# edervishaj/GANMF

Measured on AMD Instinct MI355X. Metric: GANMF training steps/sec, higher is better.
Workload: dtype f32

## Files before the change

ganmf_amd/csrc/gemm_bf16s.hpp:

```cpp
#pragma once
#include "gemm_f32.hpp"

namespace ganmf {

template <int R, int BK, bool KM>
struct SplitStage {
  static constexpr int NW = R * BK / 8;
  static constexpr int NI = NW / 256;
  static constexpr int PLANE = R * BK / 2;
  static constexpr int CH = BK / 8;
  static constexpr int RQ = R / 4;
  static constexpr int KROW = R / 2;
  static_assert(R == 64 || R == 128, "K-major chunk swizzle is laid out for 64- and 128-row operand tiles");
  __device__ static inline int swzk(int k) { return R == 64 ? ((k & 3) >> 1) << 2 : (k & 3) << 2; }
  static_assert(NW % 256 == 0 && NI >= 1, "tile too small for 256 threads");
  static_assert(BK == 32 || BK == 64, "BK must be 32 or 64");

  __device__ static inline int swz(int row) { return BK == 32 ? (row >> 2) & 3 : (row >> 1) & 7; }

  const float* zp;
  const float* ptr[NI];
  int aux[NI];
  int dst[NI];
  int dst1[NI];

  __device__ inline void init(const float* __restrict__ base, int ld, int r0, int rlimit, int kbeg,
                              const float* zero, int tid) {
    zp = zero + (tid & 255) * 8;
#pragma unroll
    for (int j = 0; j < NI; ++j) {
      const int w = j * 256 + tid;
      if constexpr (!KM) {
        const int row = w / CH, c8 = w % CH;
        const bool ok = (r0 + row) < rlimit;
        ptr[j] = ok ? base + (size_t)(r0 + row) * ld + kbeg + 8 * c8 : zp;
        aux[j] = ok ? BK : 0;
        dst[j] = row * (BK / 2) + 4 * (c8 ^ swz(row));
      } else {
        const int kp = w / RQ, rq = w % RQ;
        const bool ok = (r0 + 4 * rq) < ld;
        ptr[j] = base + (size_t)(kbeg + 2 * kp) * ld + r0 + 4 * rq;
        aux[j] = ok ? 2 * kp : -1;
        dst[j] = (2 * kp) * KROW + 4 * ((rq >> 1) ^ swzk(2 * kp)) + 2 * (rq & 1);
        dst1[j] = (2 * kp + 1) * KROW + 4 * ((rq >> 1) ^ swzk(2 * kp + 1)) + 2 * (rq & 1);
      }
    }
  }

  __device__ inline void load(float4 (&v)[NI][2], int ld, int kleft) {
#pragma unroll
    for (int j = 0; j < NI; ++j) {
      if constexpr (!KM) {
        const float* s = ptr[j];
        v[j][0] = *reinterpret_cast<const float4*>(s);
        v[j][1] = *reinterpret_cast<const float4*>(s + 4);
        ptr[j] += aux[j];
      } else {
        const float* s0 = (aux[j] >= 0 && aux[j] < kleft) ? ptr[j] : zp;
        const float* s1 = (aux[j] >= 0 && aux[j] + 1 < kleft) ? ptr[j] + ld : zp;
        v[j][0] = *reinterpret_cast<const float4*>(s0);
        v[j][1] = *reinterpret_cast<const float4*>(s1);
        ptr[j] += (size_t)BK * ld;
      }
    }
  }

  bool diag_nosplit = false;
  template <int NPIECE, bool F16 = false>
  __device__ inline void store(unsigned* __restrict__ planes, const float4 (&v)[NI][2], float scale = 1.f) const {
#pragma unroll
    for (int j = 0; j < NI; ++j) {
      const float4 a = v[j][0], b = v[j][1];
      u32x4 pc[3];
      auto one = [&](float x0, float x1, auto qq) {
        constexpr int q = decltype(qq)::value;
        if constexpr (NPIECE == 3) {
          unsigned h, m, l;
#ifdef GANMF_PERSIST_DIAG_BUILD
          if (diag_nosplit) { h = cvt_pk_bf16(x0, x1); m = h; l = h; } else
#endif
          split_bf16x3(x0, x1, h, m, l);
          pc[0][q] = h; pc[1][q] = m; pc[2][q] = l;
        } else if constexpr (F16) {
          pc[0][q] = cvt_pk_f16(x0 * scale, x1 * scale);
        } else {
          pc[0][q] = cvt_pk_bf16(x0, x1);
        }
      };
      one(a.x, a.y, std::integral_constant<int, 0>{}); one(a.z, a.w, std::integral_constant<int, 1>{});
      one(b.x, b.y, std::integral_constant<int, 2>{}); one(b.z, b.w, std::integral_constant<int, 3>{});
#pragma unroll
      for (int q = 0; q < NPIECE; ++q) {
        if constexpr (KM) {
          typedef unsigned u32x2 __attribute__((ext_vector_type(2)));
          *reinterpret_cast<u32x2*>(planes + q * PLANE + dst[j]) = u32x2{pc[q][0], pc[q][1]};
          *reinterpret_cast<u32x2*>(planes + q * PLANE + dst1[j]) = u32x2{pc[q][2], pc[q][3]};
        } else {
          *reinterpret_cast<u32x4*>(planes + q * PLANE + dst[j]) = pc[q];
        }
      }
    }
  }

  __device__ static inline u32x4 frag(const unsigned* __restrict__ plane, int rb, int c, int i, int h) {
    if constexpr (!KM) {
      return *reinterpret_cast<const u32x4*>(plane + (rb + i) * (BK / 2) + 4 * ((2 * c + h) ^ swz(i)));
    } else {
      const int l16 = i & 15, gi = i >> 4, qq = l16 >> 2, pp = l16 & 3;
      const unsigned base = (unsigned)(size_t)(__attribute__((address_space(3))) const unsigned*)plane;
      const unsigned addr = base + (unsigned)((16 * c + 8 * h + qq) * (KROW * 4) + ((((rb >> 3) + 2 * gi + (pp >> 1)) ^ swzk(qq)) << 4) + ((pp & 1) << 3));
#if defined(__HIP_DEVICE_COMPILE__)
      typedef __attribute__((address_space(3))) s16x4* lds_s16x4_p;
      const s16x4 lo = __builtin_amdgcn_ds_read_tr16_b64_v4i16((lds_s16x4_p)addr);
      const s16x4 hi = __builtin_amdgcn_ds_read_tr16_b64_v4i16((lds_s16x4_p)(addr + 4 * (KROW * 4)));
      return __builtin_bit_cast(u32x4, __builtin_shufflevector(lo, hi, 0, 1, 2, 3, 4, 5, 6, 7));
#else
      (void)addr;
      return u32x4{0u, 0u, 0u, 0u};
#endif
    }
  }
};

typedef _Float16 f16x8 __attribute__((ext_vector_type(8)));

template <int BM, int BN, int BK, int NPIECE>
struct Bf16sLds {
  static constexpr int OPER = NPIECE * (BM * BK / 2 + BN * BK / 2);
  static constexpr int DW = OPER > BM * BN ? OPER : BM * BN;
};

template <int BM, int BN, int BK, bool AKM, bool BKM, int NPIECE, bool F16 = false, bool GRAM = false, bool ROWSQ = false>
__device__ __forceinline__ void gemm_bf16s_body(const GemmP& p, const int bid, const int nblk, float* __restrict__ smem) {
  static_assert(!F16 || NPIECE == 1, "fp16 pieces only in the single-piece (mixed precision) mode");
  const float sa = (F16 && p.a_scale != 0.f) ? p.a_scale : 1.f, sb = (F16 && p.b_scale != 0.f) ? p.b_scale : 1.f;
  using SA = SplitStage<BM, BK, AKM>;
  using SB = SplitStage<BN, BK, BKM>;
  constexpr int WM = BM / 2, WN = BN / 2;
  constexpr int TM = WM / 32, TN = WN / 32;
  constexpr int NC = BK / 16;
  static_assert(NPIECE == 1 || NPIECE == 3, "pieces per operand");
  static_assert(BM % 32 == 0 && BN % 32 == 0, "row XOR of the K-major layout needs 32-row blocks");
  static_assert(Bf16sLds<BM, BN, BK, NPIECE>::OPER == NPIECE * (SA::PLANE + SB::PLANE), "LDS budget");
  unsigned* const planes_a = reinterpret_cast<unsigned*>(smem);
  unsigned* const planes_b = planes_a + NPIECE * SA::PLANE;

  const int tid = threadIdx.x;
  const int lane = tid & 63;
  const int wave = __builtin_amdgcn_readfirstlane(tid >> 6);
  const int wr = wave >> 1, wc = wave & 1;
  const int li = lane & 31, lh = lane >> 5;

  int tm, tn, sp = 0, bz = 0;
  if constexpr (GRAM) gram_tile_coords(p, bid, nblk, tm, tn);
  else tile_coords(p, bid, nblk, tm, tn, sp, bz);
  const int m0 = tm * BM, n0 = tn * BN;
  const int kbeg = sp * p.k_per_split;
  const int kend = min(p.K, kbeg + p.k_per_split);
  const int nt = (kend - kbeg + BK - 1) / BK;
#ifdef GANMF_PERSIST_DIAG_BUILD
#define GANMF_S_STAMP(i) do { if (p.stamps && tid == 0) p.stamps[(size_t)bid * 64 + (i)] = __builtin_amdgcn_s_memrealtime(); } while (0)
#else
#define GANMF_S_STAMP(i) do { } while (0)
#endif
  GANMF_S_STAMP(0);

  f32x16 acc[TM][TN];
#pragma unroll
  for (int a = 0; a < TM; ++a)
#pragma unroll
    for (int b = 0; b < TN; ++b)
#pragma unroll
      for (int r = 0; r < 16; ++r) acc[a][b][r] = 0.f;

  SA la;
  SB lb;
  la.init(p.A + (size_t)bz * p.a_batch_stride, p.lda, m0, p.M, kbeg, p.zero_page, tid);
  lb.init(p.B, p.ldb, n0, p.N, kbeg, p.zero_page, tid);
#ifdef GANMF_PERSIST_DIAG_BUILD
  la.diag_nosplit = lb.diag_nosplit = (p.diag & 2) != 0;
#endif

  float4 ra[SA::NI][2], rb[SB::NI][2];
  int kleft = kend - kbeg;
  la.load(ra, p.lda, kleft);
  lb.load(rb, p.ldb, kleft);
  kleft -= BK;
  la.template store<NPIECE, F16>(planes_a, ra, sa);
  lb.template store<NPIECE, F16>(planes_b, rb, sb);
  __syncthreads();

  u32x4 pa[2][TM][NPIECE], pb[2][TN][NPIECE];
  auto load_frags = [&](int set, int c) {
#pragma unroll
    for (int a = 0; a < TM; ++a)
#pragma unroll
      for (int q = 0; q < NPIECE; ++q) pa[set][a][q] = SA::frag(planes_a + q * SA::PLANE, wr * WM + a * 32, c, li, lh);
#pragma unroll
    for (int b = 0; b < TN; ++b)
#pragma unroll
      for (int q = 0; q < NPIECE; ++q) pb[set][b][q] = SB::frag(planes_b + q * SB::PLANE, wc * WN + b * 32, c, li, lh);
  };
  f32x16 accl[NPIECE == 3 ? TM : 1][NPIECE == 3 ? TN : 1];
  if constexpr (NPIECE == 3) {
#pragma unroll
    for (int a = 0; a < TM; ++a)
#pragma unroll
      for (int b = 0; b < TN; ++b)
#pragma unroll
        for (int r = 0; r < 16; ++r) accl[a][b][r] = 0.f;
  }
  auto mfmas = [&](int set) {
    constexpr int NT = NPIECE == 3 ? 6 : 1;
    constexpr int ta[6] = {1, 0, 2, 1, 0, 0}, tb[6] = {1, 2, 0, 0, 1, 0};
#pragma unroll
    for (int t6 = 0; t6 < NT; ++t6)
#pragma unroll
      for (int a = 0; a < TM; ++a)
#pragma unroll
        for (int b = 0; b < TN; ++b) {
          const int ia = NT == 6 ? ta[t6] : 0, ib = NT == 6 ? tb[t6] : 0;
          if (NT == 6 && t6 < 5)
            accl[a][b] = __builtin_amdgcn_mfma_f32_32x32x16_bf16(__builtin_bit_cast(bf16x8, pa[set][a][ia]),
                                                                 __builtin_bit_cast(bf16x8, pb[set][b][ib]), accl[a][b], 0, 0, 0);
          else if constexpr (F16)
            acc[a][b] = __builtin_amdgcn_mfma_f32_32x32x16_f16(__builtin_bit_cast(f16x8, pa[set][a][ia]),
                                                               __builtin_bit_cast(f16x8, pb[set][b][ib]), acc[a][b], 0, 0, 0);
          else
            acc[a][b] = __builtin_amdgcn_mfma_f32_32x32x16_bf16(__builtin_bit_cast(bf16x8, pa[set][a][ia]),
                                                                __builtin_bit_cast(bf16x8, pb[set][b][ib]), acc[a][b], 0, 0, 0);
        }
  };

  for (int it = 0; it < nt; ++it) {
    const bool more = it + 1 < nt;
    if (more) {
#ifdef GANMF_PERSIST_DIAG_BUILD
      if (!(p.diag & 16))
#endif
      {
      la.load(ra, p.lda, kleft);
      lb.load(rb, p.ldb, kleft);
      }
      kleft -= BK;
    }
    if (it < 12) GANMF_S_STAMP(1 + 5 * it);
    load_frags(0, 0);
#pragma unroll
    for (int c = 0; c < NC; ++c) {
      if (c + 1 < NC) load_frags((c + 1) & 1, c + 1);
#ifdef GANMF_PERSIST_DIAG_BUILD
      if (p.diag & 4) { if (c == 0) mfmas(0); continue; }
#endif
      mfmas(c & 1);
    }
    if (it < 12) GANMF_S_STAMP(2 + 5 * it);
    __syncthreads();
    if (it < 12) GANMF_S_STAMP(3 + 5 * it);
    if (more) {
      la.template store<NPIECE, F16>(planes_a, ra, sa);
      lb.template store<NPIECE, F16>(planes_b, rb, sb);
      if (it < 12) GANMF_S_STAMP(4 + 5 * it);
      __syncthreads();
      if (it < 12) GANMF_S_STAMP(5 + 5 * it);
    }
  }
  GANMF_S_STAMP(62);
  if constexpr (NPIECE == 3) {
#pragma unroll
    for (int a = 0; a < TM; ++a)
#pragma unroll
      for (int b = 0; b < TN; ++b) acc[a][b] += accl[a][b];
  }
  if constexpr (F16) {
    if (sa != 1.f || sb != 1.f) {
      const float un = 1.f / (sa * sb);
#pragma unroll
      for (int a = 0; a < TM; ++a)
#pragma unroll
        for (int b = 0; b < TN; ++b) acc[a][b] *= un;
    }
  }
  if constexpr (GRAM) {
    static_assert(NPIECE == 3 && !F16 && !AKM && !BKM, "the symmetric product is an NT product in the exact three-way split");
    gram_epilogue<BM, BN, TM, TN>(p, acc, smem, TileCoord{tm, tn, sp, bz, m0, n0});
  } else if constexpr (ROWSQ) {
    static_assert(NPIECE == 3 && !F16, "the per-row residual sums are formed in the exact three-way split");
    rowsq_epilogue<BM, BN, TM, TN>(p, acc, smem, TileCoord{tm, tn, sp, bz, m0, n0});
  } else
  gemm_epilogue<BM, BN, TM, TN, 1, AKM && BKM>(p, acc, smem, TileCoord{tm, tn, sp, bz, m0, n0});
#ifdef GANMF_PERSIST_DIAG_BUILD
  if (p.stamps) { asm volatile("s_waitcnt vmcnt(0)" ::: "memory"); __syncthreads(); }
#endif
  GANMF_S_STAMP(63);
}

template <int BM, int BN, int BK, bool AKM, bool BKM, int NPIECE, bool F16 = false>
__global__ __launch_bounds__(256, 2) void gemm_bf16s_mfma(const GemmP p) {
  __shared__ __attribute__((aligned(16))) float smem[Bf16sLds<BM, BN, BK, NPIECE>::DW];
  gemm_bf16s_body<BM, BN, BK, AKM, BKM, NPIECE, F16>(p, (int)blockIdx.x, (int)gridDim.x, smem);
}

template <int BM, int BN, int BK, int NPIECE, bool F16 = false>
inline hipError_t gemm_bf16s_launch(hipStream_t st, const GemmP& p, bool akm, bool bkm) {
  const int grid = p.tiles_m * p.tiles_n * p.nsplit * p.nbatch;
  if (grid <= 0) return hipSuccess;
  if (!akm && !bkm) GANMF_LAUNCH((gemm_bf16s_mfma<BM, BN, BK, false, false, NPIECE, F16>), dim3(grid), dim3(256), 0, st, p);
  else if (!akm && bkm) GANMF_LAUNCH((gemm_bf16s_mfma<BM, BN, BK, false, true, NPIECE, F16>), dim3(grid), dim3(256), 0, st, p);
  else if (akm && bkm) GANMF_LAUNCH((gemm_bf16s_mfma<BM, BN, BK, true, true, NPIECE, F16>), dim3(grid), dim3(256), 0, st, p);
  else return hipErrorInvalidValue;
  return hipGetLastError();
}

template <int NPIECE, bool F16>
inline hipError_t gemm_bf16k_launch(hipStream_t st, const GemmP& p, bool akm, bool bkm);

inline hipError_t gemm_planes_launch(hipStream_t st, const GemmP& p, bool bkm);

inline hipError_t gemm_dispatch_staged(hipStream_t st, const GemmP& p, bool akm, bool bkm, const GemmPlan& pl) {
  if (pl.tile == 64 && pl.kg == 4) {
#ifdef GANMF_PERSIST_DIAG_BUILD
    if (pl.mode == MFMA_BF16X3 && p.a_planes && p.b_planes && !akm && !p.a_gather) return gemm_planes_launch(st, p, bkm);
#endif
    if (pl.mode == MFMA_BF16X3) return gemm_bf16k_launch<3, false>(st, p, akm, bkm);
    if (pl.mode == MFMA_F16) return gemm_bf16k_launch<1, true>(st, p, akm, bkm);
    if (pl.mode == MFMA_BF16) return gemm_bf16k_launch<1, false>(st, p, akm, bkm);
  }
  if (pl.mode == MFMA_F16)
    return pl.tile == 128 ? gemm_bf16s_launch<128, 128, 32, 1, true>(st, p, akm, bkm) : gemm_bf16s_launch<64, 64, 64, 1, true>(st, p, akm, bkm);
  if (pl.mode == MFMA_BF16X3 && pl.tile == 64 && pl.bk == 32) return gemm_bf16s_launch<64, 64, 32, 3>(st, p, akm, bkm);
  if (pl.mode == MFMA_BF16X3)
    return pl.tile == 128 ? gemm_bf16s_launch<128, 128, 32, 3>(st, p, akm, bkm) : gemm_bf16s_launch<64, 64, 64, 3>(st, p, akm, bkm);
  return pl.tile == 128 ? gemm_bf16s_launch<128, 128, 32, 1>(st, p, akm, bkm) : gemm_bf16s_launch<64, 64, 64, 1>(st, p, akm, bkm);
}

}
```

ganmf_amd/csrc/gemm_f32.hpp:

```cpp
#pragma once
#include <hip/hip_runtime.h>
#include <hip/hip_ext.h>

#include <algorithm>
#include <cstdio>
#include <cstdlib>
#include <vector>
#include <cmath>
#include <type_traits>

#include "adam_touch.hpp"

namespace ganmf {

struct LaunchProf { hipEvent_t start = nullptr, stop = nullptr; int count = 0; };
inline LaunchProf& launch_prof() { static thread_local LaunchProf lp; return lp; }
inline hipEvent_t& launch_stop_event() { static thread_local hipEvent_t ev = nullptr; return ev; }
inline long long& launch_count() { static thread_local long long n = 0; return n; }

template <class F, class... Args>
inline void launch_kernel(F kernel, const dim3& grid, const dim3& block, unsigned shmem, hipStream_t st, Args... args) {
  LaunchProf& lp = launch_prof();
  hipEvent_t& stop = launch_stop_event();
  ++launch_count();
  if (lp.start && lp.count++ == 0) hipExtLaunchKernelGGL(kernel, grid, block, shmem, st, lp.start, lp.stop, 0, args...);
  else if (stop) { hipExtLaunchKernelGGL(kernel, grid, block, shmem, st, nullptr, stop, 0, args...); stop = nullptr; }
  else hipLaunchKernelGGL(kernel, grid, block, shmem, st, args...);
}
#define GANMF_LAUNCH(...) ::ganmf::launch_kernel(__VA_ARGS__)

typedef float f32x16 __attribute__((ext_vector_type(16)));
typedef float f32x2 __attribute__((ext_vector_type(2)));
typedef unsigned u32x4 __attribute__((ext_vector_type(4)));
typedef __bf16 bf16x8 __attribute__((ext_vector_type(8)));

enum MfmaMode : int { MFMA_AUTO = -1, MFMA_F32 = 0, MFMA_BF16 = 1, MFMA_F16 = 2, MFMA_BF16X3 = 3 };

typedef __bf16 bf16x2 __attribute__((ext_vector_type(2)));

__device__ inline unsigned cvt_pk_bf16(float x0, float x1) {
  unsigned r;
  asm("v_cvt_pk_bf16_f32 %0, %1, %2" : "=v"(r) : "v"(x0), "v"(x1));
  return r;
}

__device__ inline unsigned cvt_pk_bf16_tok(float x0, float x1, int tok) {
  unsigned r;
  asm("v_cvt_pk_bf16_f32 %0, %1, %2 ; behind wait token %3" : "=v"(r) : "v"(x0), "v"(x1), "s"(tok));
  return r;
}
__device__ inline void split_bf16x3_tok(float x0, float x1, unsigned& hi, unsigned& mid, unsigned& lo, int tok) {
  hi = cvt_pk_bf16_tok(x0, x1, tok);
  float r0 = x0 - __uint_as_float(hi << 16), r1 = x1 - __uint_as_float(hi & 0xffff0000u);
  mid = cvt_pk_bf16(r0, r1);
  r0 -= __uint_as_float(mid << 16);
  r1 -= __uint_as_float(mid & 0xffff0000u);
  lo = cvt_pk_bf16(r0, r1);
}

__device__ inline unsigned cvt_pk_f16(float x0, float x1) {
  unsigned r;
  x0 = __builtin_amdgcn_fmed3f(x0, -65504.f, 65504.f);
  x1 = __builtin_amdgcn_fmed3f(x1, -65504.f, 65504.f);
  asm("v_cvt_pk_f16_f32 %0, %1, %2" : "=v"(r) : "v"(x0), "v"(x1));
  return r;
}

__device__ inline void split_bf16x3(float x0, float x1, unsigned& hi, unsigned& mid, unsigned& lo) {
  hi = cvt_pk_bf16(x0, x1);
  float r0 = x0 - __uint_as_float(hi << 16), r1 = x1 - __uint_as_float(hi & 0xffff0000u);
  mid = cvt_pk_bf16(r0, r1);
  r0 -= __uint_as_float(mid << 16);
  r1 -= __uint_as_float(mid & 0xffff0000u);
  lo = cvt_pk_bf16(r0, r1);
}

template <int I, int N, class F>
__device__ inline void static_for(F&& f) {
  if constexpr (I < N) {
    f(std::integral_constant<int, I>{});
    static_for<I + 1, N>(f);
  }
}

constexpr int LD_ALIGN = 64;

enum GemmEpi : int {
  EPI_STORE = 0,
  EPI_SUB_AUX_SQ = 1,
  EPI_SUB_SCALED_AUX = 2,
  EPI_ROWSCALE = 3,
  EPI_G_DE = 4,
  EPI_ACT = 5,
  EPI_MUL_ACTGRAD = 6,
  EPI_ADAM = 7,
  EPI_GRAM_STATS = 8,
};

constexpr float ADAM_B1 = 0.9f, ADAM_B2 = 0.999f, ADAM_EPS = 1e-8f;

enum ActKind : int { ACT_LINEAR = 0, ACT_TANH = 1, ACT_RELU = 2, ACT_SIGMOID = 3 };

__device__ inline float act_apply(int act, float z) {
  switch (act) {
    case ACT_TANH: return tanhf(z);
    case ACT_RELU: return fmaxf(z, 0.f);
    case ACT_SIGMOID: return 1.f / (1.f + expf(-z));
    default: return z;
  }
}
__device__ inline float act_grad_out(int act, float a) {
  switch (act) {
    case ACT_TANH: return 1.f - a * a;
    case ACT_RELU: return a > 0.f ? 1.f : 0.f;
    case ACT_SIGMOID: return a * (1.f - a);
    default: return 1.f;
  }
}

struct EpiD {
  int kind;
  const float* aux;
  int ldaux;
  long long aux_batch_stride;
  const float* rowscale;
  float c;
  const float* er;
  const float* ef;
  float cfm;
  float* sq_partials;
  int sq_stride;
  int sq_m_half;
  int act;
  const float* r1_u;
  const float* r1_w;
  int r1_ld;
  float* adam_theta;
  float* adam_theta_out;
  float* adam_m;
  float* adam_v;
  const float* adam_alpha;
  float adam_reg;
  const long long* csr_indptr;
  const int* csr_indices;
  const float* csr_data;
  const int* csr_rows;
  const float* sp_rows;
  int sp_ld, sp_bias_row, sp_bias_parts;
  unsigned short* planes;
  long long plane_stride;
  double* gram_partials;
};

__device__ inline float4 csr_quad(const EpiD& e, int m, int col) {
  const int r = e.csr_rows[m];
  long long lo = e.csr_indptr[r];
  const long long en = e.csr_indptr[r + 1];
  long long hi = en;
  while (lo < hi) {
    const long long mid = (lo + hi) >> 1;
    if (e.csr_indices[mid] < col) lo = mid + 1; else hi = mid;
  }
  float4 x = make_float4(0.f, 0.f, 0.f, 0.f);
  for (long long j = lo; j < en; ++j) {
    const int c = e.csr_indices[j] - col;
    if (c > 3) break;
    const float v = e.csr_data[j];
    if (c == 0) x.x = v; else if (c == 1) x.y = v; else if (c == 2) x.z = v; else x.w = v;
  }
  return x;
}

__device__ inline float4 sparse_rows_quad(const EpiD& e, int row, int col) {
  if (row > e.sp_bias_row) return make_float4(0.f, 0.f, 0.f, 0.f);
  float4 s = *reinterpret_cast<const float4*>(e.sp_rows + (size_t)row * e.sp_ld + col);
  if (row == e.sp_bias_row)
    for (int q = 1; q < e.sp_bias_parts; ++q) {
      const float4 d = *reinterpret_cast<const float4*>(e.sp_rows + (size_t)(row + q) * e.sp_ld + col);
      s.x += d.x; s.y += d.y; s.z += d.z; s.w += d.w;
    }
  return s;
}

__device__ __forceinline__ float adam_step(float x, float ma, float v) {
#ifdef GANMF_ADAM_IEEE
  return x - ma / (sqrtf(v) + ADAM_EPS);
#else
  return __builtin_fmaf(-ma, __builtin_amdgcn_rcpf(__builtin_amdgcn_sqrtf(v) + ADAM_EPS), x);
#endif
}

__device__ inline void adam_update(float g, float alpha, float reg, float& th, float& m, float& v, float& sq) {
  const float x = th;
  sq += x * x;
  const float gr = g + reg * x;
  m += (gr - m) * (1.f - ADAM_B1);
  v += (gr * gr - v) * (1.f - ADAM_B2);
  th = adam_step(x, m * alpha, v);
}

__device__ inline float epi_apply(const EpiD& e, float v, int row, int col, int ldc, const float* __restrict__ aux,
                                  float& sq) {
  switch (e.kind) {
    case EPI_SUB_AUX_SQ:
      if (aux) v -= aux[(size_t)row * e.ldaux + col];
      sq += v * v;
      break;
    case EPI_SUB_SCALED_AUX:
      v -= e.c * aux[(size_t)row * e.ldaux + col];
      break;
    case EPI_ROWSCALE:
      v *= e.rowscale[row];
      break;
    case EPI_G_DE: {
      const float d = e.ef[(size_t)row * ldc + col] - e.er[(size_t)row * ldc + col];
      v = e.c * v + e.cfm * d;
      sq += d * d;
      break;
    }
    case EPI_ACT:
      if (e.r1_u) v += e.r1_u[(size_t)row * e.r1_ld] * e.r1_w[col];
      v = act_apply(e.act, v);
      break;
    case EPI_MUL_ACTGRAD:
      v *= act_grad_out(e.act, aux[(size_t)row * e.ldaux + col]);
      break;
    default: break;
  }
  return v;
}

struct GemmP {
  const float* A;
  const float* B;
  float* C;
  int lda, ldb, ldc;
  int M, N, K;
  const float* zero_page;
  int nsplit;
  int k_per_split;
  long long c_split_stride;
  int nbatch;
  long long a_batch_stride, c_batch_stride;
  EpiD epi;
  int tiles_m, tiles_n;
  unsigned* counters;
  float* Cf;
  long long cf_batch_stride;
  int c_pad_writable;
  const int* a_gather;
  int a_gather_batch;
  float a_scale, b_scale;
  int xb_m, xb_n, xb_band;
  int diag;
  unsigned long long* stamps;
  const unsigned short* a_planes;
  const unsigned short* b_planes;
  long long a_pstride, b_pstride;
  int n_fastest;
  int adam_touch;
};

#define GANMF_WAIT_VMCNT(N) asm volatile("s_waitcnt vmcnt(%0)" ::"n"(N) : "memory")

template <int BM, int BN, int NTHR>
struct AdamTouchRegs {
  static constexpr int NR = (adam_touch_slots(BM, BN) + NTHR - 1) / NTHR;
  float v[NR];
};

template <int BM, int BN, int NTHR>
__device__ __forceinline__ void adam_touch_issue(const GemmP& p, int m0, int n0, int tid, AdamTouchRegs<BM, BN, NTHR>& k) {
#pragma unroll
  for (int j = 0; j < AdamTouchRegs<BM, BN, NTHR>::NR; ++j) {
    k.v[j] = 0.f;
    const AdamTouch t = adam_touch_slot(BM, BN, j * NTHR + tid, m0, n0, p.M, p.N, p.ldc);
    if (t.arr >= 0) {
      const float* __restrict__ b = t.arr == 0 ? p.epi.adam_theta : t.arr == 1 ? p.epi.adam_m : p.epi.adam_v;
      k.v[j] = b[t.off];
    }
  }
}

template <int BM, int BN, int NTHR>
__device__ __forceinline__ void adam_touch_keep(const AdamTouchRegs<BM, BN, NTHR>& k) {
#pragma unroll
  for (int j = 0; j < AdamTouchRegs<BM, BN, NTHR>::NR; ++j) asm volatile("" ::"v"(k.v[j]));
}

template <int R, int BK, bool KM, int NTHR = 256>
struct Stage {
  static constexpr int F4 = R * BK / 4;
  static constexpr int NP = F4 / NTHR;
  static constexpr int SZ = R * BK;
  static constexpr int S = BK / 4;
  static constexpr int RC4 = R / 4;
  static_assert(F4 % NTHR == 0 && NP >= 1, "tile too small for the workgroup");
  static_assert(BK == 32 || BK == 64, "BK must be 32 or 64");

  __device__ static inline int swz(int row) { return (row / (64 / BK)) & (S - 1); }

  const float* zp;
  const float* ptr[NP];
  int aux[NP];

  __device__ inline void init(const float* __restrict__ base, int ld, int r0, int rlimit, int kbeg,
                              const float* zero, int tid, const int* __restrict__ gather = nullptr) {
    zero += (tid & 255) * 4;
    zp = zero;
#pragma unroll
    for (int j = 0; j < NP; ++j) {
      const int pos = j * NTHR + tid;
      if constexpr (!KM) {
        const int row = pos / S, slot = pos % S;
        const int c4 = slot ^ swz(row);
        const bool ok = (r0 + row) < rlimit;
        const int src_row = (ok && gather) ? gather[r0 + row] : r0 + row;
        ptr[j] = ok ? base + (size_t)src_row * ld + kbeg + 4 * c4 : zero;
        aux[j] = ok ? BK : 0;
      } else {
        const int krow = pos / RC4, c4 = pos % RC4;
        const bool ok = (r0 + 4 * c4) < ld;
        ptr[j] = base + (size_t)(kbeg + krow) * ld + r0 + 4 * c4;
        aux[j] = ok ? krow : -1;
      }
    }
  }

  template <int J>
  __device__ inline void issue_piece(float* s, int ld, int kleft, int wave) {
    const float* src;
    if constexpr (!KM) {
      src = kleft > 0 ? ptr[J] : zp;
      ptr[J] += aux[J];
    } else {
      src = (aux[J] >= 0 && aux[J] < kleft) ? ptr[J] : zp;
      ptr[J] += (size_t)BK * ld;
    }
    __builtin_amdgcn_global_load_lds((const __attribute__((address_space(1))) void*)src,
                                     (__attribute__((address_space(3))) void*)(s + (J * NTHR + wave * 64) * 4),
                                     16, 0, 0);
  }
  template <int J>
  __device__ inline void issue_piece_asm(float* s, int ld, int kleft, int wave) {
    const float* src;
    if constexpr (!KM) {
      src = kleft > 0 ? ptr[J] : zp;
      ptr[J] += aux[J];
    } else {
      src = (aux[J] >= 0 && aux[J] < kleft) ? ptr[J] : zp;
      ptr[J] += (size_t)BK * ld;
    }
    const unsigned dst = __builtin_amdgcn_readfirstlane(
        (unsigned)(size_t)(__attribute__((address_space(3))) void*)(s + (J * NTHR + wave * 64) * 4));
    unsigned keep;
    asm volatile("s_mov_b32 %0, m0\n\ts_mov_b32 m0, %2\n\ts_nop 0\n\tglobal_load_lds_dwordx4 %1, off\n\ts_mov_b32 m0, %0"
                 : "=&s"(keep) : "v"(src), "s"(dst) : "memory");
  }
  template <int J0, int J1>
  __device__ inline void issue_range_asm(float* s, int ld, int kleft, int wave) {
    if constexpr (J0 < J1) {
      issue_piece_asm<J0>(s, ld, kleft, wave);
      issue_range_asm<J0 + 1, J1>(s, ld, kleft, wave);
    }
  }
  template <int J0, int J1>
  __device__ inline void issue_range(float* s, int ld, int kleft, int wave) {
    if constexpr (J0 < J1) {
      issue_piece<J0>(s, ld, kleft, wave);
      issue_range<J0 + 1, J1>(s, ld, kleft, wave);
    }
  }
  __device__ inline void issue(float* s, int ld, int kleft, int wave) {
    issue_range<0, NP>(s, ld, kleft, wave);
  }

  __device__ static inline float4 frag(const float* __restrict__ s, int rb, int c, int i, int h) {
    if constexpr (!KM) {
      return *reinterpret_cast<const float4*>(s + (rb + i) * BK + 4 * ((2 * c + h) ^ swz(i)));
    } else {
      const float* q = s + (c * 8 + 4 * h) * R + rb + i;
      return make_float4(q[0], q[R], q[2 * R], q[3 * R]);
    }
  }
};

__device__ inline void tile_coords(const GemmP& p, int bid, int nblk, int& tm, int& tn, int& sp, int& bz) {
  tile_order(TileGrid{p.tiles_m, p.tiles_n, p.nsplit, p.xb_m, p.xb_n, p.xb_band, p.n_fastest}, bid, nblk, tm, tn, sp, bz);
}

#ifndef GANMF_ADAM_HOIST
#define GANMF_ADAM_HOIST 1
#endif

struct TileCoord { int tm, tn, sp, bz, m0, n0; };

__device__ inline void gram_tile_coords(const GemmP& p, int bid, int nblk, int& tm, int& tn);
template <int BM, int BN, int TM, int TN>
__device__ inline void gram_epilogue(const GemmP& p, const f32x16 (&acc)[TM][TN], float* smem, const TileCoord& tc_);
template <int BM, int BN, int TM, int TN>
__device__ inline void rowsq_epilogue(const GemmP& p, const f32x16 (&acc)[TM][TN], float* smem, const TileCoord& tc_);

template <int BM, int BN, int TM, int TN, int KG = 1, bool ADAM_OK = true, int NIMG = KG, bool STAGED = false>
__device__ inline void gemm_epilogue(const GemmP& p, const f32x16 (&acc)[TM][TN], float* smem, const TileCoord& tc_) {
  constexpr int WM = BM / 2, WN = BN / 2;
  constexpr int NTHR = 256 * KG;
  const int tid = threadIdx.x, lane = tid & 63;
  const int wave = __builtin_amdgcn_readfirstlane(tid >> 6);
  const int kg = wave >> 2;
  const int wr = (wave >> 1) & 1, wc = wave & 1;
  const int li = lane & 31, lh = lane >> 5;
  const int tm = tc_.tm, tn = tc_.tn, sp = tc_.sp, bz = tc_.bz, m0 = tc_.m0, n0 = tc_.n0;
  float* __restrict__ ct = smem + kg * (BM * BN);
// ... 278 lines not shown
  la.init(p.A + (size_t)bz * p.a_batch_stride, p.lda, m0, p.M, kbeg, p.zero_page, tid,
          (AKM || !p.a_gather) ? nullptr : p.a_gather + (size_t)bz * p.a_gather_batch);
  lb.init(p.B, p.ldb, n0, p.N, kbeg, p.zero_page, tid);

  constexpr int NC = BK / 8 / KG;
  static_assert((BK / 8) % KG == 0 && NC >= 2 && NC % 2 == 0, "chunks per K group");
  float4 fa[2][TM], fb[2][TN];
  auto load_frags = [&](int set, const float* __restrict__ tile, int cl) {
    const int c = cl * KG + kg;
#pragma unroll
    for (int a = 0; a < TM; ++a) fa[set][a] = SA::frag(tile, wr * WM + a * 32, c, li, lh);
#pragma unroll
    for (int b = 0; b < TN; ++b) fb[set][b] = SB::frag(tile + SA::SZ, wc * WN + b * 32, c, li, lh);
  };
  auto mfmas = [&](int set) {
#pragma unroll
    for (int a = 0; a < TM; ++a)
#pragma unroll
      for (int b = 0; b < TN; ++b) {
        acc[a][b] = __builtin_amdgcn_mfma_f32_32x32x2f32(fa[set][a].x, fb[set][b].x, acc[a][b], 0, 0, 0);
        acc[a][b] = __builtin_amdgcn_mfma_f32_32x32x2f32(fa[set][a].y, fb[set][b].y, acc[a][b], 0, 0, 0);
        acc[a][b] = __builtin_amdgcn_mfma_f32_32x32x2f32(fa[set][a].z, fb[set][b].z, acc[a][b], 0, 0, 0);
        acc[a][b] = __builtin_amdgcn_mfma_f32_32x32x2f32(fa[set][a].w, fb[set][b].w, acc[a][b], 0, 0, 0);
      }
  };

  int kleft = kend - kbeg;
  constexpr bool TOUCH_OK = AKM && BKM && !GRAM;
  AdamTouchRegs<BM, BN, NTHR> touched{};
  const bool touch = TOUCH_OK && p.adam_touch && p.nsplit == 1 && p.epi.kind == EPI_ADAM;
  if constexpr (TOUCH_OK) {
    if (touch) adam_touch_issue<BM, BN, NTHR>(p, m0, n0, tid, touched);
  }
#pragma unroll
  for (int s = 0; s < NS; ++s) {
    if (kleft > 0) {
      la.issue(smem + s * BUF, p.lda, kleft, wave);
      lb.issue(smem + s * BUF + SA::SZ, p.ldb, kleft, wave);
    }
    kleft -= BK;
  }
  if (nt >= NS) GANMF_WAIT_VMCNT((NS - 1) * LOADS);
  else GANMF_WAIT_VMCNT(0);
  __builtin_amdgcn_s_barrier();
  GANMF_GEMM_STAMP(1);
  load_frags(0, smem, 0);

  constexpr int PPC = (LOADS + NC - 1) / NC;
  int slot = 0;
  int pend_slot = 0;
  int pend_kleft = 0;
  auto refill_chunk = [&](auto cc) {
    constexpr int c = decltype(cc)::value;
    if (pend_kleft > 0) {
      float* base = smem + pend_slot * BUF;
      constexpr int q0 = c * PPC < LOADS ? c * PPC : LOADS, q1 = (c + 1) * PPC < LOADS ? (c + 1) * PPC : LOADS;
      constexpr int a0 = q0 < SA::NP ? q0 : SA::NP, a1 = q1 < SA::NP ? q1 : SA::NP;
      constexpr int b0 = q0 > SA::NP ? q0 - SA::NP : 0, b1 = q1 > SA::NP ? q1 - SA::NP : 0;
      la.template issue_range<a0, a1>(base, p.lda, pend_kleft, wave);
      lb.template issue_range<b0, b1>(base + SA::SZ, p.ldb, pend_kleft, wave);
    }
  };
  auto tile = [&](auto tail_tag) {
    constexpr bool TAIL = decltype(tail_tag)::value;
    const float* __restrict__ cur = smem + slot * BUF;
    const int nslot = (slot + 1 == NS) ? 0 : slot + 1;
    static_for<0, NC>([&](auto cc) {
      constexpr int c = decltype(cc)::value;
      if constexpr (c + 1 < NC) {
        load_frags((c + 1) & 1, cur, c + 1);
        refill_chunk(cc);
        __builtin_amdgcn_sched_barrier(0);
      } else {
        refill_chunk(cc);
        asm volatile("s_waitcnt lgkmcnt(0)" ::: "memory");
        if constexpr (TAIL) GANMF_WAIT_VMCNT(0);
        else GANMF_WAIT_VMCNT((NS - 2) * LOADS);
        __builtin_amdgcn_s_barrier();
        pend_slot = slot;
        pend_kleft = kleft;
        kleft -= BK;
        load_frags(0, smem + nslot * BUF, 0);
        __builtin_amdgcn_sched_barrier(0);
      }
      mfmas(c & 1);
    });
    slot = nslot;
  };
  int it = 0;
  for (; it + NS - 1 < nt; ++it) tile(std::false_type{});
  for (; it < nt; ++it) tile(std::true_type{});
  GANMF_WAIT_VMCNT(0);
  asm volatile("s_waitcnt lgkmcnt(0)" ::: "memory");
  __builtin_amdgcn_s_barrier();
  if constexpr (TOUCH_OK) {
    if (touch) adam_touch_keep<BM, BN, NTHR>(touched);
  }

  GANMF_GEMM_STAMP(2);
  static_assert(KG * BM * BN <= NS * BUF, "the ring must hold the KG staged partial tiles");
  if constexpr (GRAM) {
    static_assert(KG == 1 && !AKM && !BKM, "the symmetric product is an NT product on one K group");
    gram_epilogue<BM, BN, TM, TN>(p, acc, smem, TileCoord{tm, tn, sp, bz, m0, n0});
  } else
  gemm_epilogue<BM, BN, TM, TN, KG, AKM && BKM>(p, acc, smem, TileCoord{tm, tn, sp, bz, m0, n0});
#ifdef GANMF_PERSIST_DIAG_BUILD
  if (p.stamps) { asm volatile("s_waitcnt vmcnt(0)" ::: "memory"); __builtin_amdgcn_s_barrier(); }
#endif
  GANMF_GEMM_STAMP(3);
}

template <int BM, int BN, int BK, int NS, bool AKM, bool BKM, int KG = 1>
__global__ __launch_bounds__(256 * KG) void gemm_f32_mfma(const GemmP p) {
  __shared__ __attribute__((aligned(16))) float smem[NS * (BM + BN) * BK];
  gemm_f32_body<BM, BN, BK, NS, AKM, BKM, KG>(p, (int)blockIdx.x, (int)gridDim.x, smem);
}

typedef unsigned short bf16raw;
typedef short s16x4 __attribute__((ext_vector_type(4)));
typedef short s16x8 __attribute__((ext_vector_type(8)));

struct PlaneRef {
  bf16raw* p;
  long long pstride;
};

__device__ inline void planes_store4(const PlaneRef& pl, size_t off, float x, float y, float z, float w) {
  unsigned h0, m0, l0, h1, m1, l1;
  split_bf16x3(x, y, h0, m0, l0);
  split_bf16x3(z, w, h1, m1, l1);
  *reinterpret_cast<uint2*>(pl.p + off) = make_uint2(h0, h1);
  *reinterpret_cast<uint2*>(pl.p + pl.pstride + off) = make_uint2(m0, m1);
  *reinterpret_cast<uint2*>(pl.p + 2 * pl.pstride + off) = make_uint2(l0, l1);
}
__device__ inline void planes_store1(const PlaneRef& pl, size_t off, float x) {
  unsigned h, m, l;
  split_bf16x3(x, 0.f, h, m, l);
  pl.p[off] = (bf16raw)(h & 0xffffu);
  pl.p[pl.pstride + off] = (bf16raw)(m & 0xffffu);
  pl.p[2 * pl.pstride + off] = (bf16raw)(l & 0xffffu);
}


struct RedP {
  const float* part;
  long long split_stride;
  int nsplit;
  float* out;
  int ld;
  int M, N;
  long long batch_stride;
  EpiD epi;
  int sc1 = 0;
};

__host__ __device__ inline int reduce_groups(long long total4, int nsplit) {
  return (nsplit >= 64 && total4 <= 8192) ? 16 : 1;
}

template <int NT = 256>
__device__ __forceinline__ void splitk_reduce_body(const RedP& p, const int bx, const int nbx, const int bz, float* __restrict__ red) {
  const int n4 = (p.N + 3) >> 2;
  const long long total = (long long)p.M * n4;
  const float* __restrict__ part = p.part + (size_t)bz * p.batch_stride;
  float* __restrict__ out = p.out + (size_t)bz * p.batch_stride;
  const EpiD& e = p.epi;
  const bool csr0 = e.csr_indptr != nullptr && bz == 0 && e.kind == EPI_SUB_AUX_SQ;
  const float* __restrict__ aux = (e.aux && !csr0) ? e.aux + (size_t)bz * e.aux_batch_stride : nullptr;
  float sq = 0.f;
  auto finish = [&](float4 s, int m, int c, size_t off) {
    if (csr0) {
      const float4 x = csr_quad(e, m, c);
      s.x -= x.x; s.y -= x.y; s.z -= x.z; s.w -= x.w;
    }
    float o[4] = {s.x, s.y, s.z, s.w};
    if (c + 3 < p.N) {
#pragma unroll
      for (int j = 0; j < 4; ++j) o[j] = epi_apply(e, o[j], m, c + j, p.ld, aux, sq);
      if (p.sc1) {
        typedef unsigned u32x4s __attribute__((ext_vector_type(4)));
        const __amdgpu_buffer_rsrc_t rs = __builtin_amdgcn_make_buffer_rsrc((void*)out, (short)0, 0x7fffffff, 0x00020000);
        u32x4s bits;
        bits[0] = __float_as_uint(o[0]); bits[1] = __float_as_uint(o[1]); bits[2] = __float_as_uint(o[2]); bits[3] = __float_as_uint(o[3]);
        __builtin_amdgcn_raw_buffer_store_b128(bits, rs, (int)(off * sizeof(float)), 0, 16 );
      } else
      *reinterpret_cast<float4*>(out + off) = make_float4(o[0], o[1], o[2], o[3]);
      if (e.planes) planes_store4(PlaneRef{e.planes, e.plane_stride}, off, o[0], o[1], o[2], o[3]);
    } else {
      for (int j = 0; j < 4 && c + j < p.N; ++j) {
        const float r = epi_apply(e, o[j], m, c + j, p.ld, aux, sq);
        if (p.sc1) {
          const __amdgpu_buffer_rsrc_t rs = __builtin_amdgcn_make_buffer_rsrc((void*)out, (short)0, 0x7fffffff, 0x00020000);
          __builtin_amdgcn_raw_buffer_store_b32(__float_as_uint(r), rs, (int)((off + j) * sizeof(float)), 0, 16);
        } else
        out[off + j] = r;
        if (e.planes) planes_store1(PlaneRef{e.planes, e.plane_stride}, off + j, r);
      }
    }
  };
  const int G = reduce_groups(total, p.nsplit);
  if (G > 1) {
    float4* const meet = reinterpret_cast<float4*>(red + 4);
    const int epb = NT / G, g = threadIdx.x / epb, el = threadIdx.x % epb;
    for (long long base = (long long)bx * epb; base < total; base += (long long)nbx * epb) {
      const long long idx = base + el;
      const bool live = idx < total;
      const int m = live ? (int)(idx / n4) : 0, c = live ? (int)(idx % n4) * 4 : 0;
      const size_t off = (size_t)m * p.ld + c;
      float4 s = make_float4(0.f, 0.f, 0.f, 0.f);
      if (live) {
#pragma unroll 8
        for (int k = g; k < p.nsplit; k += G) {
          const float4 q = *reinterpret_cast<const float4*>(part + (size_t)k * p.split_stride + off);
          s.x += q.x; s.y += q.y; s.z += q.z; s.w += q.w;
        }
      }
      meet[threadIdx.x] = s;
      __syncthreads();
      if (g == 0 && live) {
        for (int q = 1; q < G; ++q) {
          const float4 t = meet[q * epb + el];
          s.x += t.x; s.y += t.y; s.z += t.z; s.w += t.w;
        }
        finish(s, m, c, off);
      }
      __syncthreads();
    }
  } else {
    for (long long idx = (long long)bx * NT + threadIdx.x; idx < total; idx += (long long)nbx * NT) {
      const int m = (int)(idx / n4), c = (int)(idx % n4) * 4;
      const size_t off = (size_t)m * p.ld + c;
      float4 s = *reinterpret_cast<const float4*>(part + off);
#pragma unroll 8
      for (int k = 1; k < p.nsplit; ++k) {
        const float4 q = *reinterpret_cast<const float4*>(part + (size_t)k * p.split_stride + off);
        s.x += q.x; s.y += q.y; s.z += q.z; s.w += q.w;
      }
      finish(s, m, c, off);
    }
  }
  if (e.sq_partials) {
#pragma unroll
    for (int o = 32; o > 0; o >>= 1) sq += __shfl_xor(sq, o);
    if ((threadIdx.x & 63) == 0) red[threadIdx.x >> 6] = sq;
    __syncthreads();
    if (threadIdx.x == 0) {
      float t = (red[0] + red[1]) + (red[2] + red[3]);
#pragma unroll
      for (int w = 4; w < NT / 64; w += 4) t += (red[w] + red[w + 1]) + (red[w + 2] + red[w + 3]);
      e.sq_partials[(size_t)bz * e.sq_stride + bx] = t;
    }
  }
}

__global__ __launch_bounds__(256) void splitk_reduce_kernel(const RedP p) {
  __shared__ __attribute__((aligned(16))) float red[4 + 4 * 256];
  splitk_reduce_body(p, (int)blockIdx.x, (int)gridDim.x, (int)blockIdx.y, red);
}

constexpr int GEMM_K_ALIGN = 64;
constexpr int GEMM_CUS = 256;
constexpr int GEMM_RED_GRID = 512;

struct GemmPlan {
  int tile = 128, ring = 2, nsplit = 1, kps = 0;
  int mode = MFMA_F32;
  int tiles_m = 0, tiles_n = 0;
  int persist = 0;
  int bk = 0;
  int kg = 1;
  int sq_count = 0;
  int tile_order = 0;
  int skinny = 0;
  int skinny_n = 0;
  int wide32 = 0;
  double est_us = 0;
};

struct GemmTune {
  int tile = 0, ring = 0, nsplit = 0;
  int mode = MFMA_AUTO;
  int persist = -1;
  int bk = 0;
  int kg = 0;
  int tile_order = 0;
};

inline void split_plan(int K, int want, int& nsplit, int& kps) {
  int chunks = (K + GEMM_K_ALIGN - 1) / GEMM_K_ALIGN;
  if (want < 1) want = 1;
  if (want > chunks) want = chunks;
  int cps = (chunks + want - 1) / want;
  kps = cps * GEMM_K_ALIGN;
  nsplit = (chunks + cps - 1) / cps;
}

struct TileShape { int code, bm, bn, bk; double cyc_tile, fixed; };
constexpr TileShape kTileShapes[2] = {
    {128, 128, 128, 32, 4800.0, 9000.0},
    {64, 64, 64, 64, 2900.0, 6000.0},
};

inline GemmPlan gemm_plan(int M, int N, int K, int nbatch, bool wants_sq, const GemmTune& tune, bool no_split = false) {
  GemmPlan best;
  best.est_us = 1e30;
  const double gflop = 2.0 * M * (double)N * K * nbatch * 1e-9;
  for (const TileShape& ts : kTileShapes) {
    const int tile = ts.code;
    if (tune.tile && tune.tile != tile) continue;
    if (!tune.tile && tile == 128 && (M <= 64 || N <= 64)) continue;
    const int tm = (M + ts.bm - 1) / ts.bm, tn = (N + ts.bn - 1) / ts.bn;
    const long long T = (long long)tm * tn * nbatch;
    const int bk = ts.bk;
    const double cyc_tile = ts.cyc_tile;
    const int max_split = no_split ? 1 : std::max(1, (K + GEMM_K_ALIGN - 1) / GEMM_K_ALIGN);
    for (int want = 1; want <= max_split; want = want < 8 ? want + 1 : want + (want + 3) / 4) {
      if (tune.nsplit) want = std::min(tune.nsplit, max_split);
      int ns, kps;
      split_plan(K, want, ns, kps);
      const long long wgs = T * ns;
      const double k_tiles = std::ceil((double)std::min(kps, K) / bk);
      const double per_wg = ts.fixed + k_tiles * cyc_tile;
      const double rounds = std::ceil((double)wgs / GEMM_CUS);
      double us = rounds * per_wg / 2100.0;
      if (ns > 1) us += 1.5 + (double)(ns + 1) * M * N * nbatch * 4.0 / 3.0e6;
      if (us < best.est_us) {
        best.est_us = us; best.tile = tile; best.nsplit = ns; best.kps = kps; best.tiles_m = tm; best.tiles_n = tn;
      }
      if (tune.nsplit) break;
    }
  }
  const long long wgs = (long long)best.tiles_m * best.tiles_n * nbatch * best.nsplit;
  best.ring = tune.ring ? tune.ring : (wgs > GEMM_CUS ? 2 : 3);
  if (best.nsplit == 1) best.kps = ((K + GEMM_K_ALIGN - 1) / GEMM_K_ALIGN) * GEMM_K_ALIGN;
  const bool many = wgs >= 2 * GEMM_CUS || (best.tile == 128 && 2 * wgs >= 3 * GEMM_CUS);
  best.mode = tune.mode != MFMA_AUTO ? tune.mode : (many || gflop >= 6.0 ? MFMA_BF16X3 : MFMA_F32);
  best.bk = tune.bk;
  best.tile_order = tune.tile_order;
  best.kg = (best.tile == 64 && best.mode == MFMA_F32 && best.ring <= 3) ? (tune.kg ? tune.kg : (best.ring == 3 ? 4 : 1)) : 1;
  if (best.kg == 4 && best.ring != 3) best.kg = 2;
#ifndef GANMF_PERSIST_DIAG_BUILD
  if (best.tile == 64 && best.mode == MFMA_F32) {
    if (best.kg >= 2 && best.ring >= 3) { best.kg = 4; best.ring = 3; }
    else { best.kg = 1; best.ring = 2; }
  }
#endif
  best.sq_count = wants_sq ? best.tiles_m * best.tiles_n : 0;
  return best;
}

inline size_t gemm_slab_elems(const GemmPlan& pl, int M, int ldc, int nbatch) {
  return pl.nsplit > 1 ? (size_t)pl.nsplit * nbatch * M * ldc : 0;
}

template <int BM, int BN, int BK, int NS, int KG = 1>
inline hipError_t gemm_launch_t(hipStream_t st, const GemmP& p, bool akm, bool bkm) {
  const int grid = p.tiles_m * p.tiles_n * p.nsplit * p.nbatch;
  if (grid <= 0) return hipSuccess;
  if (!akm && !bkm) GANMF_LAUNCH((gemm_f32_mfma<BM, BN, BK, NS, false, false, KG>), dim3(grid), dim3(256 * KG), 0, st, p);
  else if (!akm && bkm) GANMF_LAUNCH((gemm_f32_mfma<BM, BN, BK, NS, false, true, KG>), dim3(grid), dim3(256 * KG), 0, st, p);
  else if (akm && bkm) GANMF_LAUNCH((gemm_f32_mfma<BM, BN, BK, NS, true, true, KG>), dim3(grid), dim3(256 * KG), 0, st, p);
  else return hipErrorInvalidValue;
  return hipGetLastError();
}

struct GemmPlan;
inline hipError_t gemm_dispatch(hipStream_t st, const GemmP& p, bool akm, bool bkm, const GemmPlan& pl);

inline hipError_t gemm_run(hipStream_t st, GemmP p, bool akm, bool bkm, const GemmPlan& pl, float* slab,
                           size_t slab_elems, unsigned* counters = nullptr, size_t n_counters = 0, int red_blocks = GEMM_RED_GRID) {
  if (p.nbatch < 1) p.nbatch = 1;
  if (!p.zero_page || (p.lda % LD_ALIGN) || (p.ldb % LD_ALIGN)) return hipErrorInvalidValue;
  p.tiles_m = pl.tiles_m; p.tiles_n = pl.tiles_n;
  p.nsplit = pl.nsplit; p.k_per_split = pl.kps;
  p.epi.sq_stride = pl.sq_count;
  p.counters = nullptr;
  const bool in_launch = pl.nsplit > 1 && counters && (size_t)pl.tiles_m * pl.tiles_n * p.nbatch <= n_counters;
  RedP r{};
  if (pl.nsplit > 1) {
    if (gemm_slab_elems(pl, p.M, p.ldc, p.nbatch) > slab_elems) return hipErrorOutOfMemory;
    r.part = slab; r.nsplit = pl.nsplit; r.out = p.C; r.ld = p.ldc; r.M = p.M; r.N = p.N;
    r.batch_stride = p.c_batch_stride; r.epi = p.epi;
    r.split_stride = (long long)p.nbatch * p.M * p.ldc;
    if (p.nbatch > 1 && p.c_batch_stride != (long long)p.M * p.ldc) return hipErrorInvalidValue;
    if (in_launch) { p.counters = counters; p.Cf = p.C; p.cf_batch_stride = p.c_batch_stride; }
    else if (p.epi.sq_partials) { p.epi.sq_stride = red_blocks; r.epi.sq_stride = red_blocks; }
    p.C = slab; p.c_split_stride = r.split_stride; p.c_batch_stride = (long long)p.M * p.ldc;
  }
  hipError_t e;
  e = gemm_dispatch(st, p, akm, bkm, pl);
  if (e != hipSuccess || pl.nsplit == 1 || in_launch) return e;
  GANMF_LAUNCH(splitk_reduce_kernel, dim3(red_blocks, p.nbatch), dim3(256), 0, st, r);
  return hipGetLastError();
}

inline hipError_t gemm_dispatch_staged(hipStream_t st, const GemmP& p, bool akm, bool bkm, const GemmPlan& pl);

inline hipError_t gemm_dispatch_persist(hipStream_t st, const GemmP& p, bool akm, bool bkm, const GemmPlan& pl);

inline void choose_tile_order(GemmP& p, const GemmPlan& pl) {
  p.xb_m = p.xb_n = p.xb_band = 0;
  if (pl.tile_order == 0 || pl.nsplit != 1 || p.nbatch != 1) return;
  const long long tiles = (long long)pl.tiles_m * pl.tiles_n;
  if (pl.tile_order == 1 && tiles < 3LL * GEMM_CUS) return;
  const double tile_bytes = 4.0 * pl.tile * std::max(p.K, 1);
  const int band = (int)std::max(1.0, std::min(1.5e6 / tile_bytes, 1e6));
  double best = 1e300;
  for (int xm = 1; xm <= 8; xm *= 2) {
    const int xn = 8 / xm;
    double fetch = 0;
// ... 85 lines not shown
```

ganmf_amd/csrc/gemm_multi.hpp:

```cpp
#pragma once
#include "gemm_bf16s.hpp"
#include "gemm_bf16k.hpp"
#ifdef GANMF_PERSIST_DIAG_BUILD
#include "gemm_planes.hpp"
#endif
#include "gemm_f32.hpp"
#include "kernels.hpp"
#include "gemm_skinny.hpp"
#include "gemm_bf16w.hpp"

namespace ganmf {

template <int KG, bool X3 = false>
__global__ __launch_bounds__(256 * KG) void front_kernel(const GemmP g, const DensP d) {
  __shared__ __attribute__((aligned(16))) float smem[3 * (64 + 64) * 64];
  static_assert(!X3 || KG == 4, "the split-bf16 form has four K groups");
  const int ng = g.tiles_m * g.tiles_n * g.nsplit * g.nbatch;
  if ((int)blockIdx.x < ng) {
    if constexpr (X3) gemm_bf16k_body<false, false>(g, (int)blockIdx.x, ng, smem);
    else gemm_f32_body<64, 64, 64, 3, false, false, KG>(g, (int)blockIdx.x, ng, smem);
  } else densify_row_body(d, (int)blockIdx.x - ng);
}
template <bool F16>
__global__ __launch_bounds__(1024) void front_lp_kernel(const GemmP g, const DensP d) {
  __shared__ __attribute__((aligned(16))) float smem[bf16k_smem_dw<1>()];
  const int ng = g.tiles_m * g.tiles_n * g.nsplit * g.nbatch;
  if ((int)blockIdx.x < ng) gemm_bf16k_body<false, false, 1, F16>(g, (int)blockIdx.x, ng, smem);
  else densify_row_body(d, (int)blockIdx.x - ng);
}

template <int KG, bool X3 = false>
__global__ __launch_bounds__(256 * KG) void de_dcoef_kernel(const GemmP g, const DCoefP d, const int nd) {
  __shared__ __attribute__((aligned(16))) float smem[3 * (64 + 64) * 64];
  static_assert(!X3 || KG == 4, "the split-bf16 form has four K groups");
  const int ng = g.tiles_m * g.tiles_n * g.nsplit * g.nbatch;
  if (nd == 0) {
    d_coef_body(d, (int)blockIdx.x, ng, smem);
    __syncthreads();
    if constexpr (X3) gemm_bf16k_body<false, false>(g, (int)blockIdx.x, ng, smem);
    else gemm_f32_body<64, 64, 64, 3, false, false, KG>(g, (int)blockIdx.x, ng, smem);
    return;
  }
  if ((int)blockIdx.x < ng) {
    if constexpr (X3) gemm_bf16k_body<false, false>(g, (int)blockIdx.x, ng, smem);
    else gemm_f32_body<64, 64, 64, 3, false, false, KG>(g, (int)blockIdx.x, ng, smem);
  } else d_coef_body(d, (int)blockIdx.x - ng, nd, smem);
}

template <int KG, int NS>
__global__ __launch_bounds__(256 * KG) __attribute__((amdgpu_num_sgpr(80))) void pair_kernel(const GemmP g0, const GemmP g1) {
  __shared__ __attribute__((aligned(16))) float smem[NS * (64 + 64) * 64];
  const int n0 = g0.tiles_m * g0.tiles_n * g0.nsplit * g0.nbatch;
  const int n1 = g1.tiles_m * g1.tiles_n * g1.nsplit * g1.nbatch;
  if ((int)blockIdx.x < n0) gemm_f32_body<64, 64, 64, NS, false, true, KG>(g0, (int)blockIdx.x, n0, smem);
  else gemm_f32_body<64, 64, 64, NS, true, true, KG>(g1, (int)blockIdx.x - n0, n1, smem);
}

template <bool F16>
__global__ __launch_bounds__(1024) __attribute__((amdgpu_num_sgpr(80))) void pair_lp_kernel(const GemmP g0, const GemmP g1) {
  __shared__ __attribute__((aligned(16))) float smem[bf16k_smem_dw<1>()];
  const int n0 = g0.tiles_m * g0.tiles_n * g0.nsplit * g0.nbatch;
  const int n1 = g1.tiles_m * g1.tiles_n * g1.nsplit * g1.nbatch;
  if ((int)blockIdx.x < n0) gemm_bf16k_body<false, true, 1, F16>(g0, (int)blockIdx.x, n0, smem);
  else gemm_bf16k_body<true, true, 1, F16>(g1, (int)blockIdx.x - n0, n1, smem);
}

__global__ __launch_bounds__(256, 2) void gemm_bf16s_red(const GemmP g, const RedP r, const int nred) {
  __shared__ __attribute__((aligned(16))) float smem[Bf16sLds<64, 64, 32, 3>::DW];
  const int ng = g.tiles_m * g.tiles_n * g.nsplit * g.nbatch;
  if ((int)blockIdx.x < ng) gemm_bf16s_body<64, 64, 32, true, true, 3>(g, (int)blockIdx.x, ng, smem);
  else splitk_reduce_body(r, (int)blockIdx.x - ng, nred, 0, smem);
}

template <int BK, int NPIECE, bool F16>
__global__ __launch_bounds__(256, 2) void gemm_bf16s_colsum(const GemmP g, const ColSumP q, const int ncs) {
  __shared__ __attribute__((aligned(16))) float smem[Bf16sLds<64, 64, BK, NPIECE>::DW];
  static_assert(Bf16sLds<64, 64, BK, NPIECE>::DW >= 2 * CS_GROUPS * CS_COLS, "the column sums' two LDS images");
  const int ng = g.tiles_m * g.tiles_n * g.nsplit * g.nbatch;
  if ((int)blockIdx.x < ng) gemm_bf16s_body<64, 64, BK, true, true, NPIECE, F16>(g, (int)blockIdx.x, ng, smem);
  else dis_colsum_body(q, (int)blockIdx.x - ng, smem);
}

__global__ __launch_bounds__(256, 2) void wgrad_pair_kernel(const GemmP g0, const GemmP g1) {
  __shared__ __attribute__((aligned(16))) float smem[Bf16sLds<64, 64, 32, 3>::DW];
  const int n0 = g0.tiles_m * g0.tiles_n * g0.nsplit * g0.nbatch;
  const int n1 = g1.tiles_m * g1.tiles_n * g1.nsplit * g1.nbatch;
  if ((int)blockIdx.x < n0) gemm_bf16s_body<64, 64, 32, true, true, 3>(g0, (int)blockIdx.x, n0, smem);
  else gemm_bf16s_body<64, 64, 32, true, true, 3>(g1, (int)blockIdx.x - n0, n1, smem);
}

__global__ __launch_bounds__(256, 2) void wgrad_seam_kernel(const GemmP g0, const GemmP g1, const RedP r, const int nred, unsigned long long* cnt,
                                                            const unsigned long long target) {
  __shared__ __attribute__((aligned(16))) float smem[Bf16sLds<64, 64, 32, 3>::DW];
  static_assert(Bf16sLds<64, 64, 32, 3>::DW >= 4 + 4 * 256, "splitk_reduce_body's LDS");
  const int n0 = g0.tiles_m * g0.tiles_n * g0.nsplit * g0.nbatch;
  const int n1 = g1.tiles_m * g1.tiles_n * g1.nsplit * g1.nbatch;
  const int b = (int)blockIdx.x;
  if (b < nred) {
    splitk_reduce_body(r, b, nred, 0, smem);
    asm volatile("s_waitcnt vmcnt(0)" ::: "memory");
    __syncthreads();
    if (threadIdx.x == 0) __hip_atomic_fetch_add(cnt, 1ull, __ATOMIC_RELAXED, __HIP_MEMORY_SCOPE_AGENT);
    return;
  }
  if (b < nred + n0) { gemm_bf16s_body<64, 64, 32, true, true, 3>(g0, b - nred, n0, smem); return; }
  if (threadIdx.x == 0) {
    unsigned spins = 0;
    while (__hip_atomic_load(cnt, __ATOMIC_RELAXED, __HIP_MEMORY_SCOPE_AGENT) < target) {
      __builtin_amdgcn_s_sleep(4);
      if (++spins > (1u << 22)) { __hip_atomic_store(cnt + 1, 1ull, __ATOMIC_RELAXED, __HIP_MEMORY_SCOPE_AGENT); break; }
    }
    __builtin_amdgcn_fence(__ATOMIC_ACQUIRE, "agent");
    asm volatile("s_waitcnt vmcnt(0)" ::: "memory");
  }
  __syncthreads();
  gemm_bf16s_body<64, 64, 32, true, true, 3>(g1, b - nred - n0, n1, smem);
}

inline bool plan_is_f32_64_kg(const GemmPlan& pl, int kg) {
  return pl.mode == MFMA_F32 && pl.tile == 64 && pl.ring == 3 && pl.kg == kg && !pl.persist;
}
inline bool plan_is_lp_64(const GemmPlan& pl) {
  return (pl.mode == MFMA_F16 || pl.mode == MFMA_BF16) && pl.tile == 64 && pl.ring == 3 && pl.bk != 32 && !pl.persist;
}

inline void fill_plan(GemmP& p, const GemmPlan& pl) {
  if (p.nbatch < 1) p.nbatch = 1;
  p.tiles_m = pl.tiles_m; p.tiles_n = pl.tiles_n;
  p.nsplit = pl.nsplit; p.k_per_split = pl.kps;
  p.epi.sq_stride = pl.sq_count;
  p.counters = nullptr;
}

}
```

ganmf_amd/csrc/kernels.hpp:

```cpp
#pragma once
#include <hip/hip_runtime.h>

#include "gemm_f32.hpp"

namespace ganmf {

enum Scal : int {
  S_B1P_D = 0, S_B2P_D = 1, S_B1P_G = 2, S_B2P_G = 3,
  S_ALPHA_D = 4, S_ALPHA_G = 5,
  S_ALPHA_D_ALT = 6,
  S_SUM_REAL = 8, S_SUM_FAKE = 9, S_SUM_FM = 10,
  S_B1P_G_SAVED = 12, S_B2P_G_SAVED = 13,
  S_COUNT = 16,
  S_TAB = 16
};


__device__ inline float wave_sum(float v) {
#pragma unroll
  for (int o = 32; o > 0; o >>= 1) v += __shfl_xor(v, o);
  return v;
}

__device__ inline float block_sum_256(float v, float* red4) {
  v = wave_sum(v);
  if ((threadIdx.x & 63) == 0) red4[threadIdx.x >> 6] = v;
  __syncthreads();
  return (red4[0] + red4[1]) + (red4[2] + red4[3]);
}

__device__ __forceinline__ void open_steps_body(float* __restrict__ scal, int which, int first_slot, int count, float lr);

struct DensP {
  const long long* indptr;
  const int* indices;
  const float* data;
  const int* rows;
  int nb, ncols;
  float* X;
  int ldx;
  const float* Uemb;
  int ldk;
  float* Ub;
  float* scal;
  int which, alpha_idx;
  float lr;
  int uid_col, row_offset;
  int nseg;
  int stage_b;
  int open_d_slot, open_d_count, open_g_slot, open_g_count;
  float lr_d, lr_g;
};

__device__ __forceinline__ void densify_row_body(const DensP& d, const int bid) {
  const int nseg = d.nseg > 1 ? d.nseg : 1;
  const int b = bid / nseg, seg = bid % nseg;
  const bool staged = d.stage_b > 0;
  if (staged && bid == 0 && threadIdx.x == 0) {
    if (d.open_d_count > 0) open_steps_body(d.scal, 0, d.open_d_slot, d.open_d_count, d.lr_d);
    if (d.open_g_count > 0) {
      d.scal[S_B1P_G_SAVED] = d.scal[S_B1P_G]; d.scal[S_B2P_G_SAVED] = d.scal[S_B2P_G];
      open_steps_body(d.scal, 1, d.open_g_slot, d.open_g_count, d.lr_g);
    }
  }
  if (!staged && d.alpha_idx >= 0 && bid == 0 && threadIdx.x == 0) {
    const int o = d.which ? S_B1P_G : S_B1P_D;
    const float b1p = d.scal[o], b2p = d.scal[o + 1];
    d.scal[d.alpha_idx] = d.lr * sqrtf(1.f - b2p) / (1.f - b1p);
    d.scal[o] = b1p * ADAM_B1;
    d.scal[o + 1] = b2p * ADAM_B2;
  }
  const int r = d.rows[b];
  const size_t xrow = staged ? (size_t)b + (size_t)(b / d.stage_b) * d.stage_b : (size_t)b;
  const size_t frow = staged ? xrow + d.stage_b : (size_t)d.nb + b;
  const int segw = ((d.ldx / 4 + nseg - 1) / nseg) * 4;
  const int c0 = seg * segw, c1 = min(d.ldx, c0 + segw);
  float* x = d.X + xrow * d.ldx;
  float4* xr = reinterpret_cast<float4*>(x + c0);
  for (int c = threadIdx.x; c < (c1 - c0) / 4; c += blockDim.x) xr[c] = make_float4(0.f, 0.f, 0.f, 0.f);
  if (seg == 0 && d.Ub) {
    const float4* us = reinterpret_cast<const float4*>(d.Uemb + (size_t)r * d.ldk);
    float4* ud = reinterpret_cast<float4*>(d.Ub + (size_t)b * d.ldk);
    for (int c = threadIdx.x; c < d.ldk / 4; c += blockDim.x) ud[c] = us[c];
  }
  __syncthreads();
  const long long s = d.indptr[r], e = d.indptr[r + 1];
  for (long long j = s + threadIdx.x; j < e; j += blockDim.x) {
    const int col = d.indices[j];
    if (col >= c0 && col < c1) x[col] = d.data[j];
  }
  if (threadIdx.x == 0) {
    if (d.ncols >= c0 && d.ncols < c1) x[d.ncols] = 1.0f;
    if (seg == 0) d.X[frow * d.ldx + d.ncols] = 1.0f;
    if (d.uid_col >= 0) {
      if (d.uid_col >= c0 && d.uid_col < c1) x[d.uid_col] = (float)(d.row_offset + r);
      if (seg == 0) d.X[frow * d.ldx + d.uid_col] = (float)(d.row_offset + r);
    }
  }
}

__global__ __launch_bounds__(256) void densify_rows_kernel(const DensP d) { densify_row_body(d, (int)blockIdx.x); }

__device__ __forceinline__ void csr_rowsum_body(const int* __restrict__ indices, const float* __restrict__ data, const long long s,
                                                const long long en, const float* __restrict__ We, const int lde, const int ncols,
                                                const int e, float* __restrict__ Erow, float4* __restrict__ part) {
  const int tid = threadIdx.x;
  const int c4n = (e + 3) / 4;
  const float* bias = We + (size_t)ncols * lde;
  for (int c0 = 0; c0 < c4n; c0 += 256) {
    const int width = min(256, c4n - c0);
    const int G = 256 / width, g = tid / width, c = c0 + tid % width;
    float4 acc = make_float4(0.f, 0.f, 0.f, 0.f);
    if (g < G) {
#pragma unroll 8
      for (long long j = s + g; j < en; j += G) {
        const float w = data[j];
        const float4 a = *reinterpret_cast<const float4*>(We + (size_t)indices[j] * lde + 4 * c);
        acc.x += w * a.x; acc.y += w * a.y; acc.z += w * a.z; acc.w += w * a.w;
      }
    }
    part[tid] = acc;
    __syncthreads();
    if (tid < width) {
      float4 t = *reinterpret_cast<const float4*>(bias + 4 * c);
      for (int q = 0; q < G; ++q) {
        const float4 a = part[q * width + tid];
        t.x += a.x; t.y += a.y; t.z += a.z; t.w += a.w;
      }
      float* dst = Erow + 4 * c;
      if (4 * c + 3 < e) *reinterpret_cast<float4*>(dst) = t;
      else {
        dst[0] = t.x;
        if (4 * c + 1 < e) dst[1] = t.y;
        if (4 * c + 2 < e) dst[2] = t.z;
      }
    }
    __syncthreads();
  }
}

__global__ __launch_bounds__(256) void sparse_front_kernel(const long long* __restrict__ indptr,
                                                           const int* __restrict__ indices,
                                                           const float* __restrict__ data,
                                                           const int* __restrict__ rows, int nb, int ncols,
                                                           float* __restrict__ XF, int ldx,
                                                           const float* __restrict__ Uemb, int ldk,
                                                           float* __restrict__ Ub, float* __restrict__ scal, int which,
                                                           int alpha_idx, float lr, const float* __restrict__ We, int lde,
                                                           int e, float* __restrict__ E) {
  __shared__ float4 part[256];
  const int b = blockIdx.x, tid = threadIdx.x;
  if (alpha_idx >= 0 && b == 0 && tid == 0) {
    const int o = which ? S_B1P_G : S_B1P_D;
    const float b1p = scal[o], b2p = scal[o + 1];
    scal[alpha_idx] = lr * sqrtf(1.f - b2p) / (1.f - b1p);
    scal[o] = b1p * ADAM_B1;
    scal[o + 1] = b2p * ADAM_B2;
  }
  const int r = rows[b];
  const float4* us = reinterpret_cast<const float4*>(Uemb + (size_t)r * ldk);
  if (Ub) {
    float4* ud = reinterpret_cast<float4*>(Ub + (size_t)b * ldk);
    for (int c = tid; c < ldk / 4; c += 256) ud[c] = us[c];
  }
  if (tid == 0) XF[(size_t)(nb + b) * ldx + ncols] = 1.0f;
  csr_rowsum_body(indices, data, indptr[r], indptr[r + 1], We, lde, ncols, e, E + (size_t)b * lde, part);
}

constexpr int CSC_BIAS_PARTS = 16;
__global__ __launch_bounds__(256) void csc_rows_kernel(const long long* __restrict__ colptr, const int* __restrict__ rowidx,
                                                       const float* __restrict__ val, const int* __restrict__ pos, int start,
                                                       int nb, int ncols, const float* __restrict__ dEr, int ld, int e,
                                                       float* __restrict__ S) {
  __shared__ float4 part[256];
  const int j = blockIdx.x, tid = threadIdx.x;
  const int c4n = (e + 3) / 4;
  const bool bias = j >= ncols;
  const long long a = bias ? 0 : colptr[j], z = bias ? 0 : colptr[j + 1];
  for (int c0 = 0; c0 < c4n; c0 += 256) {
    const int width = min(256, c4n - c0);
    const int G = 256 / width, g = tid / width, c = c0 + tid % width;
    float4 acc = make_float4(0.f, 0.f, 0.f, 0.f);
    if (g < G) {
      if (!bias) {
#pragma unroll 4
        for (long long i = a + g; i < z; i += G) {
          const int b = pos[rowidx[i]] - start;
          const bool in = b >= 0 && b < nb;
          const float w = in ? val[i] : 0.f;
          const float4 d = *reinterpret_cast<const float4*>(dEr + (size_t)(in ? b : 0) * ld + 4 * c);
          acc.x += w * d.x; acc.y += w * d.y; acc.z += w * d.z; acc.w += w * d.w;
        }
      } else {
#pragma unroll 4
        for (int b = (j - ncols) + g * CSC_BIAS_PARTS; b < nb; b += G * CSC_BIAS_PARTS) {
          const float4 d = *reinterpret_cast<const float4*>(dEr + (size_t)b * ld + 4 * c);
          acc.x += d.x; acc.y += d.y; acc.z += d.z; acc.w += d.w;
        }
      }
    }
    part[tid] = acc;
    __syncthreads();
    if (tid < width) {
      float4 t = part[tid];
      for (int q = 1; q < G; ++q) {
        const float4 u = part[q * width + tid];
        t.x += u.x; t.y += u.y; t.z += u.z; t.w += u.w;
      }
      *reinterpret_cast<float4*>(S + (size_t)j * ld + 4 * c) = t;
    }
    __syncthreads();
  }
}

__global__ void open_step_kernel(float* __restrict__ scal, int which, int alpha_idx, float lr) {
  if (blockIdx.x == 0 && threadIdx.x == 0) {
    const int o = which ? S_B1P_G : S_B1P_D;
    const float b1p = scal[o], b2p = scal[o + 1];
    scal[alpha_idx] = lr * sqrtf(1.f - b2p) / (1.f - b1p);
    scal[o] = b1p * ADAM_B1;
    scal[o + 1] = b2p * ADAM_B2;
  }
}

__device__ __forceinline__ void open_steps_body(float* __restrict__ scal, int which, int first_slot, int count, float lr) {
  const int o = which ? S_B1P_G : S_B1P_D;
  float b1p = scal[o], b2p = scal[o + 1];
  for (int i = 0; i < count; ++i) {
    scal[first_slot + i] = lr * sqrtf(1.f - b2p) / (1.f - b1p);
    b1p = b1p * ADAM_B1;
    b2p = b2p * ADAM_B2;
  }
  scal[o] = b1p;
  scal[o + 1] = b2p;
}
__global__ void restore_g_powers_kernel(float* __restrict__ scal) {
  if (blockIdx.x == 0 && threadIdx.x == 0) { scal[S_B1P_G] = scal[S_B1P_G_SAVED]; scal[S_B2P_G] = scal[S_B2P_G_SAVED]; }
}
__global__ void open_steps_kernel(float* __restrict__ scal, int which, int first_slot, int count, float lr) {
  if (blockIdx.x == 0 && threadIdx.x == 0) open_steps_body(scal, which, first_slot, count, lr);
}

__global__ __launch_bounds__(256) void gather_rows_kernel(const float* __restrict__ src, int ld,
                                                          const int* __restrict__ rows, int nrows,
                                                          float* __restrict__ dst) {
  const int c4 = ld / 4;
  const long long total = (long long)nrows * c4;
  for (long long i = (long long)blockIdx.x * blockDim.x + threadIdx.x; i < total;
       i += (long long)gridDim.x * blockDim.x) {
    const int b = (int)(i / c4), c = (int)(i % c4);
    reinterpret_cast<float4*>(dst + (size_t)b * ld)[c] =
        reinterpret_cast<const float4*>(src + (size_t)rows[b] * ld)[c];
  }
}

struct MultiRedEntry { const float* p; int n; int dst; int accumulate; };
constexpr int MULTIRED_MAX = 8;
struct MultiRed { MultiRedEntry e[MULTIRED_MAX]; int count; float* out; };

__global__ __launch_bounds__(256) void multi_reduce_kernel(const MultiRed mr) {
  __shared__ float red[4];
  for (int z = 0; z < mr.count; ++z) {
    const MultiRedEntry e = mr.e[z];
    if (e.dst != (int)blockIdx.x) continue;
    float s = 0.f;
    for (int i = threadIdx.x; i < e.n; i += 256) s += e.p[i];
    const float t = block_sum_256(s, red);
    if (threadIdx.x == 0) mr.out[e.dst] = e.accumulate ? mr.out[e.dst] + t : t;
    __syncthreads();
  }
}

__global__ __launch_bounds__(256) void finish_parts_kernel(const float* __restrict__ arena, int cap, int mode,
                                                           float* __restrict__ parts) {
  __shared__ float red[4];
  const float* a = arena + (size_t)blockIdx.x * 4 * cap;
  float tot[4];
  for (int sgm = 0; sgm < 4; ++sgm) {
    float s = 0.f;
    for (int i = threadIdx.x; i < cap; i += 256) s += a[(size_t)sgm * cap + i];
    tot[sgm] = block_sum_256(s, red);
    __syncthreads();
  }
  if (threadIdx.x == 0) {
    float* p = parts + (size_t)blockIdx.x * 4;
    if (mode == 0) p[2] = tot[2] + tot[3];
    else { p[0] = tot[0]; p[1] = tot[1]; p[2] = tot[2]; p[3] = tot[3]; }
  }
}

__global__ __launch_bounds__(256) void finish_dis_parts_kernel(const float* __restrict__ arena, long long stride, int cap,
                                                               int nseg, int mode, float* __restrict__ parts) {
  __shared__ float red[4];
  const float* a = arena + (size_t)blockIdx.x * stride;
  float out[4] = {0.f, 0.f, 0.f, 0.f};
  for (int sgm = 0; sgm < nseg; ++sgm) {
    if (mode == 0 && (sgm == 2 || sgm == 3)) continue;
    if (mode == 1 && sgm >= 4) break;
    float s = 0.f;
    for (int i = threadIdx.x; i < cap; i += 256) s += a[(size_t)sgm * cap + i];
    const float t = block_sum_256(s, red);
    __syncthreads();
    if (mode == 1 || sgm < 2) out[sgm] = t;
    else out[2] += t;
  }
  if (threadIdx.x == 0) {
    float* p = parts + (size_t)blockIdx.x * 4;
    p[0] = out[0]; p[1] = out[1]; p[2] = out[2];
    if (mode == 1) p[3] = out[3];
  }
}

__global__ void col_copy_kernel(float* __restrict__ parts, float* __restrict__ vec, long long n, int col, int to_vec) {
  for (long long i = (long long)blockIdx.x * blockDim.x + threadIdx.x; i < n; i += (long long)gridDim.x * blockDim.x) {
    if (to_vec) vec[i] = parts[4 * i + col];
    else parts[4 * i + col] = vec[i];
  }
}

struct DCoefP {
  float* scal;
  const float* partials;
  int np, pstride, presummed;
  float m;
  int b_local;
  float inv_bn;
  const float* E;
  float* Es;
  int lde;
  float* rs;
  float* loss_parts;
};

__device__ __forceinline__ void d_coef_body(const DCoefP& p, const int bx, const int nbx, float* __restrict__ red) {
  float* sums = red + 4;
  if (!p.presummed) {
    for (int z = 0; z < 2; ++z) {
      float s = 0.f;
      if (threadIdx.x < 256)
        for (int i = threadIdx.x; i < p.np; i += 256) s += p.partials[(size_t)z * p.pstride + i];
      s = wave_sum(s);
      if (threadIdx.x < 256 && (threadIdx.x & 63) == 0) red[threadIdx.x >> 6] = s;
      __syncthreads();
      if (threadIdx.x == 0) sums[z] = (red[0] + red[1]) + (red[2] + red[3]);
      __syncthreads();
    }
  } else {
    if (threadIdx.x == 0) { sums[0] = p.scal[S_SUM_REAL]; sums[1] = p.scal[S_SUM_FAKE]; }
    __syncthreads();
  }
  const float Lr = sums[0] * p.inv_bn, Lf = sums[1] * p.inv_bn;
  const float h = p.m * Lr - Lf;
  const bool on = h > 0.f;
  const float cr = (on ? 1.f + p.m : 1.f) * (2.f * p.inv_bn);
  const float cf = (on ? -1.f : 0.f) * (2.f * p.inv_bn);
  const int c4 = p.lde / 4;
  const long long total = (long long)2 * p.b_local * c4;
  for (long long i = (long long)bx * blockDim.x + threadIdx.x; i < total; i += (long long)nbx * blockDim.x) {
    const int r = (int)(i / c4);
    const float sc = r < p.b_local ? cr : cf;
    float4 v = reinterpret_cast<const float4*>(p.E)[i];
    v.x *= sc; v.y *= sc; v.z *= sc; v.w *= sc;
    reinterpret_cast<float4*>(p.Es)[i] = v;
  }
  if (bx == 0) {
    for (int r = threadIdx.x; r < 2 * p.b_local; r += blockDim.x) p.rs[r] = r < p.b_local ? cr : cf;
    if (threadIdx.x == 0) {
      p.loss_parts[0] = Lr + fmaxf(0.f, h);
      p.loss_parts[1] = on ? 1.f : 0.f;
    }
  }
}

__global__ __launch_bounds__(256) void d_coef_kernel(const DCoefP p) {
  __shared__ float red[6];
  d_coef_body(p, (int)blockIdx.x, (int)gridDim.x, red);
}

__global__ __launch_bounds__(256) void adam_dense_kernel(float* __restrict__ th, float* __restrict__ mo,
                                                         float* __restrict__ vo, const float* __restrict__ g,
                                                         long long n4, const float* __restrict__ scal,
                                                         int alpha_idx, float reg, float* __restrict__ sq_partials) {
  __shared__ float red[4];
  const float alpha = scal[alpha_idx];
  float sq = 0.f;
  for (long long i = (long long)blockIdx.x * blockDim.x + threadIdx.x; i < n4;
       i += (long long)gridDim.x * blockDim.x) {
    float4 t = reinterpret_cast<float4*>(th)[i];
    float4 m = reinterpret_cast<float4*>(mo)[i];
    float4 v = reinterpret_cast<float4*>(vo)[i];
    const float4 gg = reinterpret_cast<const float4*>(g)[i];
    float* tp = &t.x; float* mp = &m.x; float* vp = &v.x; const float* gp = &gg.x;
#pragma unroll
    for (int j = 0; j < 4; ++j) {
      const float x = tp[j];
      sq += x * x;
      const float gr = gp[j] + reg * x;
      mp[j] += (gr - mp[j]) * (1.f - ADAM_B1);
      vp[j] += (gr * gr - vp[j]) * (1.f - ADAM_B2);
      tp[j] = adam_step(x, mp[j] * alpha, vp[j]);
    }
    reinterpret_cast<float4*>(th)[i] = t;
    reinterpret_cast<float4*>(mo)[i] = m;
    reinterpret_cast<float4*>(vo)[i] = v;
  }
  if (sq_partials) {
    const float s = block_sum_256(sq, red);
    if (threadIdx.x == 0) sq_partials[blockIdx.x] = s;
  }
}

__device__ __forceinline__ void adam_row_elem(float g, float reg, float alpha, float& th, float& m, float& v, float& sq) {
  const float x = th;
  sq += x * x;
  const float gr = g + reg * x;
  m = m * ADAM_B1 + gr * (1.f - ADAM_B1);
  v = v * ADAM_B2 + (gr * gr) * (1.f - ADAM_B2);
  th = adam_step(x, alpha * m, v);
}

__global__ __launch_bounds__(256) void adam_rows_kernel(float* __restrict__ th, float* __restrict__ mo,
                                                        float* __restrict__ vo, const float* __restrict__ gb,
                                                        int gsplit, long long gstride,
                                                        const int* __restrict__ pos, int start, int nb,
                                                        int nrows, int ld, const float* __restrict__ scal,
                                                        int alpha_idx, float reg, float* __restrict__ sq_partials) {
  __shared__ float red[4];
  const float alpha = scal[alpha_idx];
  const int c4 = ld / 4;
  const long long total = (long long)nrows * c4;
  float sq = 0.f;
  for (long long i = (long long)blockIdx.x * blockDim.x + threadIdx.x; i < total;
       i += (long long)gridDim.x * blockDim.x) {
    const int r = (int)(i / c4), c = (int)(i % c4);
    const int slot = pos[r] - start;
    float4 gg = make_float4(0.f, 0.f, 0.f, 0.f);
    if (slot >= 0 && slot < nb) {
      const float* gp0 = gb + (size_t)slot * ld + 4 * c;
      gg = *reinterpret_cast<const float4*>(gp0);
#pragma unroll 8
      for (int sp = 1; sp < gsplit; ++sp) {
        const float4 q = *reinterpret_cast<const float4*>(gp0 + (size_t)sp * gstride);
        gg.x += q.x; gg.y += q.y; gg.z += q.z; gg.w += q.w;
      }
    }
    float4 t = reinterpret_cast<float4*>(th)[i];
    float4 m = reinterpret_cast<float4*>(mo)[i];
    float4 v = reinterpret_cast<float4*>(vo)[i];
    float* tp = &t.x; float* mp = &m.x; float* vp = &v.x; const float* gp = &gg.x;
#pragma unroll
    for (int j = 0; j < 4; ++j) adam_row_elem(gp[j], reg, alpha, tp[j], mp[j], vp[j], sq);
    reinterpret_cast<float4*>(th)[i] = t;
    reinterpret_cast<float4*>(mo)[i] = m;
    reinterpret_cast<float4*>(vo)[i] = v;
  }
  if (sq_partials) {
    const float s = block_sum_256(sq, red);
    if (threadIdx.x == 0) sq_partials[blockIdx.x] = s;
  }
}

struct LazyStep {
  const float* g;
  long long gstride;
  int nsplit, start, nb;
};

__global__ __launch_bounds__(256) void adam_rows_advance_kernel(const float* __restrict__ th, const float* __restrict__ mo,
                                                                const float* __restrict__ vo, const int* __restrict__ perm,
                                                                const int* __restrict__ pos_step, int n, int ld,
                                                                const float* __restrict__ scal, int tab, float reg,
                                                                float* __restrict__ out) {
  const int c4 = ld / 4;
  const long long total = (long long)n * c4;
  for (long long i = (long long)blockIdx.x * blockDim.x + threadIdx.x; i < total; i += (long long)gridDim.x * blockDim.x) {
    const int a = (int)(i / c4), c = (int)(i % c4);
    const size_t src = (size_t)perm[a] * c4 + c;
    const int s = pos_step[a];
    float4 t = reinterpret_cast<const float4*>(th)[src];
    float4 m = reinterpret_cast<const float4*>(mo)[src];
    float4 v = reinterpret_cast<const float4*>(vo)[src];
    float* tp = &t.x; float* mp = &m.x; float* vp = &v.x;
    float sq = 0.f;
    for (int tt = 0; tt < s; ++tt) {
      const float alpha = scal[tab + tt];
#pragma unroll
      for (int j = 0; j < 4; ++j) adam_row_elem(0.f, reg, alpha, tp[j], mp[j], vp[j], sq);
    }
    reinterpret_cast<float4*>(out)[i] = t;
  }
}

__global__ __launch_bounds__(256) void adam_rows_flush_kernel(float* __restrict__ th, float* __restrict__ mo, float* __restrict__ vo,
                                                              const int* __restrict__ pos, const int* __restrict__ pos_step,
                                                              const LazyStep* __restrict__ steps, int T, int nrows, int ld,
                                                              const float* __restrict__ scal, int tab, float reg) {
  const int c4 = ld / 4;
  const long long total = (long long)nrows * c4;
  for (long long i = (long long)blockIdx.x * blockDim.x + threadIdx.x; i < total; i += (long long)gridDim.x * blockDim.x) {
    const int r = (int)(i / c4), c = (int)(i % c4);
    const int a = pos[r];
    const int s = a >= 0 ? pos_step[a] : -1;
    float4 gg = make_float4(0.f, 0.f, 0.f, 0.f);
    if (s >= 0) {
      const LazyStep st = steps[s];
      const float* gp0 = st.g + (size_t)(a - st.start) * ld + 4 * c;
      gg = *reinterpret_cast<const float4*>(gp0);
#pragma unroll 8
      for (int sp = 1; sp < st.nsplit; ++sp) {
        const float4 q = *reinterpret_cast<const float4*>(gp0 + (size_t)sp * st.gstride);
        gg.x += q.x; gg.y += q.y; gg.z += q.z; gg.w += q.w;
      }
    }
    float4 t = reinterpret_cast<float4*>(th)[i];
    float4 m = reinterpret_cast<float4*>(mo)[i];
    float4 v = reinterpret_cast<float4*>(vo)[i];
    float* tp = &t.x; float* mp = &m.x; float* vp = &v.x; const float* gp = &gg.x;
    float sq = 0.f;
    for (int tt = 0; tt < T; ++tt) {
      const float alpha = scal[tab + tt];
      const bool mine = tt == s;
#pragma unroll
      for (int j = 0; j < 4; ++j) adam_row_elem(mine ? gp[j] : 0.f, reg, alpha, tp[j], mp[j], vp[j], sq);
    }
    reinterpret_cast<float4*>(th)[i] = t;
    reinterpret_cast<float4*>(mo)[i] = m;
    reinterpret_cast<float4*>(vo)[i] = v;
  }
// ... 646 lines not shown
```

ganmf_amd/csrc/lib/abi_core.inc:

```

int ganmf_abi_version(void) { return GANMF_ABI_VERSION; }
const char* ganmf_last_error(void) { return g_err.c_str(); }

static uint32_t g_crc_tab[8][256];
static std::once_flag g_crc_once;
static void crc_init() {
  for (uint32_t i = 0; i < 256; ++i) {
    uint32_t c = i;
    for (int k = 0; k < 8; ++k) c = (c & 1) ? (c >> 1) ^ 0x82F63B78u : c >> 1;
    g_crc_tab[0][i] = c;
  }
  for (uint32_t i = 0; i < 256; ++i)
    for (int t = 1; t < 8; ++t) g_crc_tab[t][i] = (g_crc_tab[t - 1][i] >> 8) ^ g_crc_tab[0][g_crc_tab[t - 1][i] & 0xff];
}
uint32_t ganmf_crc32c(uint32_t crc, const void* data, uint64_t n) {
  std::call_once(g_crc_once, crc_init);
  const uint8_t* p = static_cast<const uint8_t*>(data);
  uint32_t c = ~crc;
  while (n >= 8) {
    uint64_t w;
    memcpy(&w, p, 8);
    w ^= c;
    c = g_crc_tab[7][w & 0xff] ^ g_crc_tab[6][(w >> 8) & 0xff] ^ g_crc_tab[5][(w >> 16) & 0xff] ^
        g_crc_tab[4][(w >> 24) & 0xff] ^ g_crc_tab[3][(w >> 32) & 0xff] ^ g_crc_tab[2][(w >> 40) & 0xff] ^
        g_crc_tab[1][(w >> 48) & 0xff] ^ g_crc_tab[0][(w >> 56) & 0xff];
    p += 8; n -= 8;
  }
  while (n--) c = (c >> 8) ^ g_crc_tab[0][(c ^ *p++) & 0xff];
  return ~c;
}

int ganmf_device_count(void) {
  int n = 0;
  if (hipGetDeviceCount(&n) != hipSuccess) return 0;
  return n;
}

static int create_impl(const ganmf_cfg* cfg, ganmf_handle* h);

int ganmf_create(const ganmf_cfg* cfg, ganmf_handle** out) {
  if (!cfg || !out) return fail(-1, "ganmf_create: null argument");
  if (cfg->abi_version != GANMF_ABI_VERSION) return fail(-1, "ganmf_create: ABI version %d != %d", cfg->abi_version, GANMF_ABI_VERSION);
  if (cfg->model != GANMF_MODEL_GANMF && cfg->model != GANMF_MODEL_DISGANMF && cfg->model != GANMF_MODEL_MF && cfg->model != GANMF_MODEL_ITEMSIM) return fail(-1, "ganmf_create: unknown model %d", cfg->model);
  if (cfg->model == GANMF_MODEL_DISGANMF && (cfg->d_layers < 1 || cfg->d_layers > 16 || cfg->d_act < 0 || cfg->d_act > 3))
    return fail(-1, "ganmf_create: DisGANMF needs 1 <= d_layers <= 16 and a known activation");
  if (cfg->num_users < 1 || cfg->num_items < 1 || cfg->num_factors < 1 || cfg->emb_dim < 1 || cfg->batch_size < 1)
    return fail(-1, "ganmf_create: non-positive dimension");
  if (cfg->num_users > (1LL << 30) || cfg->num_items > (1LL << 30)) return fail(-1, "ganmf_create: dimension too large");
  int ndev = 0;
  HIP_TRY(hipGetDeviceCount(&ndev));
  if (ndev < 1) return fail(-2, "ganmf_create: no HIP device (the HIP path is the only path; there is no CPU fallback)");
  if (cfg->device < 0 || cfg->device >= ndev) return fail(-1, "ganmf_create: device %d out of range [0,%d)", cfg->device, ndev);
  HIP_TRY(hipSetDevice(cfg->device));
  ganmf_handle* h = new ganmf_handle();
  const int rc = create_impl(cfg, h);
  if (rc != 0) {
    const std::string msg = g_err;
    ganmf_destroy(h);
    (void)hipGetLastError();
    g_err = msg;
    *out = nullptr;
    return rc;
  }
  *out = h;
  return 0;
}

static int create_impl(const ganmf_cfg* cfg, ganmf_handle* h) {
  h->cfg = *cfg;
  h->dev = cfg->device;
  h->U = (int)cfg->num_users; h->N = (int)cfg->num_items; h->k = cfg->num_factors; h->e = cfg->emb_dim;
  h->B = (int)std::min<int64_t>(cfg->batch_size, cfg->num_users);
  h->ldN = round_up(h->N + 2, LD_ALIGN); h->ldk = round_up(h->k + 1, LD_ALIGN); h->lde = round_up(h->e + 1, LD_ALIGN);
  h->tune.tile = tune_env_int("tile", 0);
  if (h->tune.tile != 0 && h->tune.tile != 64 && h->tune.tile != 128) h->tune.tile = 0;
  h->tune.ring = tune_env_int("ring", 0);
  if (h->tune.ring != 0 && h->tune.ring != 2 && h->tune.ring != 3 && h->tune.ring != 4) h->tune.ring = 0;
  h->tune.nsplit = std::max(0, tune_env_int("nsplit", 0));
  h->tune.mode = env_mfma_mode((cfg->flags & GANMF_FLAG_MFMA_F16) ? MFMA_F16 : (cfg->flags & GANMF_FLAG_MFMA_BF16) ? MFMA_BF16 : (cfg->flags & GANMF_FLAG_MFMA_F32) ? MFMA_F32 : MFMA_DEFAULT);
  h->tune.persist = tune_env_int("persist", -1);
  if (h->tune.persist > 1) h->tune.persist = experiment_int("GANMF_PERSIST_WAVES", 1);
  h->tune.kg = tune_env_int("kg", 0);
  h->tune.tile_order = tune_env_int("tile_order", 0);
  h->pass_stage = tune_env_int("pass_stage", 1) != 0;
  h->skinny = tune_env_int("skinny", 1) != 0;
  h->skinny_n = h->skinny && tune_env_int("skinny_n", 1) != 0;
  h->lazy_rows = tune_env_int("lazy_rows", 1) != 0;
#ifdef GANMF_ASM_PREFETCH_UNTESTED
  constexpr int kAsmPrefetchDefault = 0;
#else
  constexpr int kAsmPrefetchDefault = 1;
#endif
  h->bf16w = tune_env_int("bf16w", kAsmPrefetchDefault);
  h->wgrad_xb = std::max(0, tune_env_int("wgrad_xb", 16));
  h->wd_lane = std::max(0, tune_env_int("wd_lane", 0));
  h->g_rows_staged = std::max(0, std::min(2, tune_env_int("g_rows_staged", 1)));
  h->pair_kg = tune_env_int("pair_kg", 4) == 1 ? 1 : 4;
  h->wgrad_seam = tune_env_int("wgrad_seam", 0);
  h->adam_touch = tune_env_int("adam_touch", 1) != 0 ? 1 : 0;
  h->gram_arith = tune_env_int("gram", 1) == 0 ? 0 : 1;
  HIP_TRY(hipMalloc((void**)&h->seam_cnt, 2 * sizeof(unsigned long long)));
  HIP_TRY(hipMemset(h->seam_cnt, 0, 2 * sizeof(unsigned long long)));
  if (h->tune.kg != 0 && h->tune.kg != 1 && h->tune.kg != 2 && h->tune.kg != 4) h->tune.kg = 0;
  h->debug_plan = env_int("GANMF_DEBUG_PLAN", 0) != 0;
  h->fused_mode = experiment_int("GANMF_FUSED_X3", 1) ? MFMA_BF16X3 : MFMA_F32;
  h->fused_tile = experiment_int("GANMF_FUSED_TILE", 64) == 128 ? 128 : 64;
  h->fused_bk = experiment_int("GANMF_FUSED_BK", 32);
  HIP_TRY(hipStreamCreateWithFlags(&h->st, hipStreamNonBlocking));
  HIP_TRY(hipStreamCreateWithFlags(&h->st2, hipStreamNonBlocking));
  const bool lane_fence = env_int("GANMF_LANE_EVENT_FENCE", cfg->world_size > 1 ? 1 : 0) != 0;
  const unsigned lane_flags = lane_fence ? hipEventDisableTiming : (hipEventDisableTiming | hipEventDisableSystemFence);
  HIP_TRY(hipEventCreateWithFlags(&h->ev_fork, lane_flags));
  HIP_TRY(hipEventCreateWithFlags(&h->ev_join, lane_flags));
  HIP_TRY(hipEventCreateWithFlags(&h->ev_mid, lane_flags));
  HIP_TRY(hipEventCreateWithFlags(&h->ev_we, lane_flags));
  HIP_TRY(hipEventCreateWithFlags(&h->ev_wd, lane_flags));
  h->fuse_adam = experiment_int("GANMF_FUSE_ADAM", 1) != 0;
  const int multi_env = env_int("GANMF_MULTI", 127);
  h->multi = multi_env & 31;
  h->defer_gub = (multi_env & 32) != 0;
  h->dis_fuse_hidden = (multi_env & 64) != 0;
  h->x3kg = env_int("GANMF_X3KG", kAsmPrefetchDefault ? 7 : 0);
  h->dcoef_spread = experiment_int("GANMF_DCOEF_SPREAD", 1) != 0;
  h->pair_ring = experiment_int("GANMF_PAIR_RING", 2) == 3 ? 3 : 2;
  h->inkernel_reduce = experiment_int("GANMF_INKERNEL_REDUCE", 0) != 0;
  h->inlaunch_max = experiment_int("GANMF_INLAUNCH_MAX", 4);
  h->inlaunch_tags = experiment_int("GANMF_INLAUNCH_TAGS", 0);
  h->force_coll = env_int("GANMF_FORCE_COLLECTIVES", 0) != 0;
  h->score_presplit = env_int("GANMF_SCORE_PRESPLIT", 1) != 0;
  h->fork_attach = experiment_int("GANMF_FORK_ATTACH", 1) != 0;
  h->adam_nfast = experiment_int("GANMF_ADAM_NFAST", 3);
  h->red_elems = experiment_int("GANMF_RED_ELEMS", 0);
  h->merge_decode = experiment_int("GANMF_MERGE_DECODE", 1) != 0;
  TRY(dalloc((float**)&h->counters, COUNTER_CAP));
  TRY(dalloc((float**)&h->counters2, COUNTER_CAP));
  const int U = h->U, N = h->N, k = h->k, e = h->e, B = h->B;
  const bool dis = cfg->model == GANMF_MODEL_DISGANMF;
  const bool sim = cfg->model == GANMF_MODEL_ITEMSIM;
  const bool mf = cfg->model == GANMF_MODEL_MF || sim;
  const int world = std::max(1, (int)cfg->world_size);
  if (!sim) {
    TRY(alloc_tensor(h->Ue, U, k, false, 1));
    TRY(alloc_tensor(h->V, N, k, true, world));
    TRY(dalloc(&h->V_alt, h->V.cap));
  }
  if (mf) {
  } else if (!dis) {
    TRY(alloc_tensor(h->We, N + 1, e, false, world));
    TRY(alloc_tensor(h->Wd, e + 1, N, false, world, h->ldN));
    h->gD_elems = h->We.cap + h->Wd.cap;
    TRY(dalloc(&h->gD, h->gD_elems));
    h->We.g = h->gD;
    h->Wd.g = h->We.g + h->We.cap;
  } else {
    h->L = cfg->d_layers; h->act = cfg->d_act;
    h->Wl.resize(h->L);
    h->dis_fused.assign(h->L, 0);
    h->dis_regn.assign(h->L, ADAM_GRID);
    h->gD_elems = 0;
    for (int l = 0; l < h->L; ++l) {
      TRY(alloc_tensor(h->Wl[l], l == 0 ? N + 2 : e + 1, e, false, world));
      h->gD_elems += h->Wl[l].cap;
    }
    TRY(alloc_tensor(h->Wo, 1, e + 1, false, world));
    h->gD_elems += h->Wo.cap;
    TRY(dalloc(&h->gD, h->gD_elems));
    float* gp = h->gD;
    for (int l = 0; l < h->L; ++l) { h->Wl[l].g = gp; gp += h->Wl[l].cap; }
    h->Wo.g = gp;
  }
  TRY(dalloc(&h->zero_page, 2048 + 64));
  TRY(dalloc((float**)&h->perm, (size_t)3 * U));
  h->pos = h->perm + U;
  h->pos_step = h->perm + 2 * (size_t)U;
  if (!mf) {
    TRY(dalloc(&h->XF, (size_t)2 * B * h->ldN));
    h->XF_own = h->XF;
    TRY(dalloc(&h->Ub, (size_t)B * h->ldk));
    h->Ub_own = h->Ub;
    TRY(dalloc(&h->dF, (size_t)B * h->ldN));
    TRY(dalloc(&h->gUb, (size_t)B * h->ldk));
    h->gUb_own = h->gUb;
    std::vector<float> ones((size_t)2 * B, 1.0f);
    HIP_TRY(hipMemcpy2D(h->XF + N, (size_t)h->ldN * 4, ones.data(), 4, 4, (size_t)2 * B, hipMemcpyHostToDevice));
    if (!dis) {
      TRY(dalloc(&h->E, (size_t)2 * B * h->lde));
      TRY(dalloc(&h->Es, (size_t)2 * B * h->lde));
      TRY(dalloc(&h->Dl, (size_t)2 * B * h->ldN));
      TRY(dalloc(&h->dE, (size_t)2 * B * h->lde));
      HIP_TRY(hipMemcpy2D(h->E + e, (size_t)h->lde * 4, ones.data(), 4, 4, (size_t)2 * B, hipMemcpyHostToDevice));
#ifdef GANMF_PERSIST_DIAG_BUILD
      h->wgrad_stream = env_int("GANMF_WGRAD_STREAM", 0) != 0;
#endif
      if (h->wgrad_stream) {
        h->ps_N = (long long)2 * B * h->ldN; h->ps_e = (long long)2 * B * h->lde;
        TRY(dalloc((float**)&h->pl_XF, (size_t)(3 * h->ps_N + 1) / 2));
        TRY(dalloc((float**)&h->pl_Dl, (size_t)(3 * h->ps_N + 1) / 2));
        TRY(dalloc((float**)&h->pl_Es, (size_t)(3 * h->ps_e + 1) / 2));
        TRY(dalloc((float**)&h->pl_dE, (size_t)(3 * h->ps_e + 1) / 2));
        TRY(dalloc(&h->wgs_dump, 2048 + 64));
      }
    } else {
      h->Al.resize(h->L, nullptr);
      for (int l = 0; l < h->L; ++l) {
        TRY(dalloc(&h->Al[l], (size_t)2 * B * h->lde));
        HIP_TRY(hipMemcpy2D(h->Al[l] + e, (size_t)h->lde * 4, ones.data(), 4, 4, (size_t)2 * B, hipMemcpyHostToDevice));
      }
      TRY(dalloc(&h->dz0, (size_t)2 * B * h->lde));
      TRY(dalloc(&h->dz1, (size_t)2 * B * h->lde));
      TRY(dalloc(&h->dlogit, (size_t)2 * B));
    }
  }
  TRY(dalloc(&h->rs, (size_t)2 * B));
  h->tab_cap = (int)(U / std::max(B, 1)) + 2;
  TRY(dalloc(&h->scal, (size_t)S_TAB + 4 * (size_t)h->tab_cap));
  TRY(dalloc(&h->sqp, (size_t)2 * std::max(GEMM_RED_GRID, ((B + 63) / 64) * ((N + 63) / 64)) + 16));
  {
    auto t64 = [](int a, int b) { return ((a + 63) / 64) * ((b + 63) / 64); };
    h->reg_cap = std::max({ADAM_GRID, (int)GEMM_RED_GRID, t64(N + 2, e), t64(e + 1, N), t64(N, k), t64(B, N), t64(B, e)});
    h->reg_cap = round_up(h->reg_cap + (e + 63) / 64, 64);
    h->dis_cap = round_up(std::max({h->reg_cap, B, dis_dz_top_blocks(e) + 1}), 64);
  }
  const float pw[4] = {ADAM_B1, ADAM_B2, ADAM_B1, ADAM_B2};
  HIP_TRY(hipMemcpy(h->scal, pw, sizeof pw, hipMemcpyHostToDevice));
  HIP_TRY(hipDeviceSynchronize());
  return 0;
}

int ganmf_destroy(ganmf_handle* h) {
  if (!h) return 0;
  hipSetDevice(h->dev);
  if (h->st) hipStreamSynchronize(h->st);
  if (h->has_comm && !h->local && !h->comm_aborted) ncclCommDestroy(h->comm);
  if (h->local) {
    std::lock_guard<std::mutex> lk(h->local->mu);
    h->local->failed = true;
    h->local->cv.notify_all();
  }
  free_tensor(h->We, false); free_tensor(h->Wd, false); hipFree(h->zero_page); hipFree(h->Es); hipFree(h->seam_cnt);
  for (auto& t : h->Wl) free_tensor(t, false);
  free_tensor(h->Wo, false);
  for (float* a : h->Al) hipFree(a);
  hipFree(h->dz0); hipFree(h->dz1); hipFree(h->dlogit);
  free_tensor(h->Ue, false); free_tensor(h->V, true); hipFree(h->V_alt);
  hipFree(h->gD); hipFree(h->indptr); hipFree(h->indices); hipFree(h->data); hipFree(h->perm);
  hipFree(h->csc_colptr); hipFree(h->csc_rowidx); hipFree(h->csc_val); hipFree(h->sp_rows);
  if (h->stage_i) hipHostFree(h->stage_i);
  if (h->stage_f) hipHostFree(h->stage_f);
  hipFree(h->test_indptr); hipFree(h->test_indices); hipFree(h->test_gain); hipFree(h->eval_buf);
  hipFree(h->cand_indptr); hipFree(h->cand_indices);
  hipFree(h->test_rating); hipFree(h->eval_w); hipFree(h->eval_rmse); hipFree(h->eval_counts); hipFree(h->eval_grp);
  hipFree(h->XF_own); hipFree(h->XF_pass); hipFree(h->Ub_pass); hipFree(h->Ub_own); hipFree(h->Ub_sched); hipFree(h->lazy_tab);
  for (auto& ch : h->lazy_chunks) hipFree(ch.first);
  if (h->lazy_stage) hipHostFree(h->lazy_stage);
  h->lazy_chunks.clear();
  hipFree(h->E); hipFree(h->Dl); hipFree(h->dE); hipFree(h->dF); hipFree(h->gUb_own);
  hipFree(h->slab); hipFree(h->rs); hipFree(h->scal); hipFree(h->sqp);
  hipFree(h->seen_indptr); hipFree(h->seen_indices); hipFree(h->item_mask); hipFree(h->topk_items); hipFree(h->topk_vals); hipFree(h->sc_ids);
  hipFree(h->colbuf); hipFree(h->parts_all); hipFree(h->sc_rows); hipFree(h->sc_out); hipFree(h->sc_pa); hipFree(h->sc_pb);
  hipFree(h->sim_mat); hipFree(h->sim_pool); hipFree(h->sim_part); hipFree(h->sim_zero);
  hipFree(h->rank_mask); hipFree(h->div_mat);
  for (AlsSide& s : h->als) { hipFree(s.indptr); hipFree(s.indices); hipFree(s.conf); }
  hipFree(h->als_G); hipFree(h->als_bad);
  hipFree(h->knn_indptr); hipFree(h->knn_nbr); hipFree(h->knn_val); hipFree(h->knn_dense);
  hipFree(h->svd_P[0]); hipFree(h->svd_P[1]); hipFree(h->svd_G); hipFree(h->svd_X); hipFree(h->svd_Wl);
  hipFree(h->svd_lam); hipFree(h->svd_flag);
  hipFree(h->dr_ids); hipFree(h->dr_X); hipFree(h->dr_Ub); hipFree(h->dr_E); hipFree(h->dr_A); hipFree(h->dr_part); hipFree(h->dr_val);
  for (auto& r : h->recs) { hipEventDestroy(r.a); hipEventDestroy(r.b); }
  if (h->st2) hipStreamSynchronize(h->st2);
  if (h->ev_fork) hipEventDestroy(h->ev_fork);
  if (h->ev_join) hipEventDestroy(h->ev_join);
  if (h->ev_mid) hipEventDestroy(h->ev_mid);
  if (h->ev_t0) hipEventDestroy(h->ev_t0);
  if (h->ev_t1) hipEventDestroy(h->ev_t1);
  if (h->ev_we) hipEventDestroy(h->ev_we);
  if (h->ev_wd) hipEventDestroy(h->ev_wd);
  if (h->st2) hipStreamDestroy(h->st2);
  if (h->st) hipStreamDestroy(h->st);
  hipFree(h->slab2); hipFree(h->counters); hipFree(h->counters2);
  hipFree(h->pl_XF); hipFree(h->pl_Dl); hipFree(h->pl_Es); hipFree(h->pl_dE); hipFree(h->wgs_dump); hipFree(h->wgs_table);
  delete h;
  return 0;
}

int ganmf_comm_unique_id(uint8_t out128[128]) {
  static_assert(sizeof(ncclUniqueId) == 128, "ncclUniqueId is expected to be 128 bytes");
  ncclUniqueId id;
  NCCL_TRY(ncclGetUniqueId(&id));
  memcpy(out128, &id, 128);
  return 0;
}

int ganmf_comm_init_local(ganmf_handle* h, int32_t group_id) {
  if (!h) return fail(-1, "null handle");
  if (h->has_comm) return fail(-1, "ganmf_comm_init_local: handle already has a communicator");
  const int world = h->cfg.world_size, rank = h->cfg.rank;
  if (world < 1 || world > LOCAL_MAX_WORLD || rank < 0 || rank >= world)
    return fail(-1, "ganmf_comm_init_local: world_size %d / rank %d out of range (max %d)", world, rank, LOCAL_MAX_WORLD);
  std::lock_guard<std::mutex> lk(g_local_mu);
  std::shared_ptr<LocalGroup>& slot = g_local_groups[group_id];
  if (!slot || slot->joined == slot->world || slot->failed) {
    slot = std::make_shared<LocalGroup>();
    slot->world = world; slot->dev = h->dev;
  }
  if (slot->world != world || slot->dev != h->dev)
    return fail(-1, "ganmf_comm_init_local: group %d is for world_size %d on device %d", group_id, slot->world, slot->dev);
  ++slot->joined;
  h->local = slot;
  h->has_comm = true;
  return 0;
}

int ganmf_comm_init(ganmf_handle* h, const uint8_t id128[128]) {
  if (!h) return fail(-1, "null handle");
  HIP_TRY(hipSetDevice(h->dev));
  ncclUniqueId id;
  memcpy(&id, id128, 128);
  NCCL_TRY(ncclCommInitRank(&h->comm, h->cfg.world_size, id, h->cfg.rank));
  h->has_comm = true;
  return 0;
}

int ganmf_comm_info(ganmf_handle* h, int32_t* world_size, int32_t* rank) {
  if (!h || !world_size || !rank) return fail(-1, "ganmf_comm_info: null argument");
  *world_size = 0; *rank = -1;
  if (!h->has_comm) return 0;
  if (h->local) { *world_size = h->local->world; *rank = h->cfg.rank; return 0; }
  int n = 0, r = -1;
  std::lock_guard<std::mutex> comm_lk(h->comm_mu);
  if (h->comm_aborted.load(std::memory_order_acquire)) return fail(-3, "ganmf_comm_info: communicator aborted (ganmf_comm_abort)");
  NCCL_TRY(ncclCommCount(h->comm, &n));
  NCCL_TRY(ncclCommUserRank(h->comm, &r));
  *world_size = n; *rank = r;
  return 0;
}

int ganmf_comm_abort(ganmf_handle* h) {
  if (!h) return fail(-1, "ganmf_comm_abort: null handle");
  if (!h->has_comm) return 0;
  if (h->local) {
    std::lock_guard<std::mutex> lk(h->local->mu);
    h->local->failed = true;
    h->local->cv.notify_all();
    return 0;
  }
  if (!h->comm_aborted.exchange(true, std::memory_order_acq_rel)) {
    std::lock_guard<std::mutex> comm_lk(h->comm_mu);
    NCCL_TRY(ncclCommAbort(h->comm));
  }
  return 0;
}

int ganmf_set_urm_csr(ganmf_handle* h, const int64_t* indptr, const int32_t* indices, const float* data,
                      int64_t n_rows, int64_t n_cols) {
  if (!h || !indptr || ((!indices || !data) && indptr[n_rows] > 0)) return fail(-1, "ganmf_set_urm_csr: null argument");
  if (n_rows != h->U || n_cols != h->N) return fail(-1, "ganmf_set_urm_csr: shape %lldx%lld != handle %dx%d", (long long)n_rows, (long long)n_cols, h->U, h->N);
  int64_t nnz = indptr[n_rows];
  if (indptr[0] != 0 || nnz < 0) return fail(-1, "ganmf_set_urm_csr: bad indptr");
  for (int64_t r = 0; r < n_rows; ++r)
    if (indptr[r + 1] < indptr[r]) return fail(-1, "ganmf_set_urm_csr: indptr not monotone at row %lld", (long long)r);
  for (int64_t j = 0; j < nnz; ++j)
    if (indices[j] < 0 || indices[j] >= n_cols) return fail(-1, "ganmf_set_urm_csr: column index %d out of range at %lld", indices[j], (long long)j);
  std::vector<int64_t> c_indptr;
  std::vector<int> c_indices;
  std::vector<float> c_data;
  bool canonical = true;
  for (int64_t r = 0; r < n_rows && canonical; ++r)
    for (int64_t j = indptr[r] + 1; j < indptr[r + 1]; ++j)
      if (indices[j] <= indices[j - 1]) { canonical = false; break; }
  if (!canonical) {
    c_indptr.assign((size_t)n_rows + 1, 0);
    c_indices.reserve((size_t)nnz);
    c_data.reserve((size_t)nnz);
    std::vector<int64_t> order;
    for (int64_t r = 0; r < n_rows; ++r) {
      order.resize((size_t)(indptr[r + 1] - indptr[r]));
      for (size_t i = 0; i < order.size(); ++i) order[i] = indptr[r] + (int64_t)i;
      std::stable_sort(order.begin(), order.end(), [&](int64_t a, int64_t b) { return indices[a] < indices[b]; });
      for (size_t i = 0; i < order.size(); ++i) {
        const int64_t j = order[i];
        if (i > 0 && indices[j] == c_indices.back()) c_data.back() += data[j];
        else { c_indices.push_back(indices[j]); c_data.push_back(data[j]); }
      }
      c_indptr[(size_t)r + 1] = (int64_t)c_indices.size();
    }
    indptr = c_indptr.data();
    indices = c_indices.data();
    data = c_data.data();
    nnz = (int64_t)c_indices.size();
  }
  HIP_TRY(hipSetDevice(h->dev));
  if (h->indptr) { hipFree(h->indptr); hipFree(h->indices); hipFree(h->data); h->indptr = nullptr; }
  HIP_TRY(hipMalloc((void**)&h->indptr, (n_rows + 1) * sizeof(long long)));
  HIP_TRY(hipMalloc((void**)&h->indices, std::max<int64_t>(nnz, 1) * sizeof(int)));
  HIP_TRY(hipMalloc((void**)&h->data, std::max<int64_t>(nnz, 1) * sizeof(float)));
  HIP_TRY(hipMemcpy(h->indptr, indptr, (n_rows + 1) * sizeof(long long), hipMemcpyHostToDevice));
  if (nnz) {
    HIP_TRY(hipMemcpy(h->indices, indices, nnz * sizeof(int), hipMemcpyHostToDevice));
    HIP_TRY(hipMemcpy(h->data, data, nnz * sizeof(float), hipMemcpyHostToDevice));
  }
  h->nnz = nnz;
  h->has_urm = true;
  const double density = (double)nnz / ((double)n_rows * (double)n_cols);
  const int force = env_int("GANMF_SPARSE", -1);
  h->sparse_g = h->cfg.model == GANMF_MODEL_GANMF && (force >= 0 ? force != 0 : density < 0.005);
  const int force_d = env_int("GANMF_SPARSE_D", -1);
  const double flops_saved = 4.0 * (double)h->B * (double)h->N * (double)h->e;
  h->sparse_d = h->cfg.model == GANMF_MODEL_GANMF && force != 0 &&
                (force_d >= 0 ? force_d != 0 : (density < 0.005 && flops_saved >= 2.0e9));
  if (h->debug_plan)
    fprintf(stderr, "[ganmf urm] set_urm_csr %lldx%lld nnz=%lld%s density %.5f -> sparse_g %d sparse_d %d\n", (long long)n_rows,
            (long long)n_cols, (long long)nnz, canonical ? "" : " (made canonical)", density, (int)h->sparse_g, (int)h->sparse_d);
  hipFree(h->csc_colptr); hipFree(h->csc_rowidx); hipFree(h->csc_val);
  h->csc_colptr = nullptr; h->csc_rowidx = nullptr; h->csc_val = nullptr;
  if (h->sparse_d) {
    std::vector<long long> colptr((size_t)n_cols + 1, 0);
    for (int64_t j = 0; j < nnz; ++j) ++colptr[(size_t)indices[j] + 1];
    for (int64_t c = 0; c < n_cols; ++c) colptr[c + 1] += colptr[c];
    std::vector<long long> fill(colptr.begin(), colptr.end() - 1);
    std::vector<int> rowidx((size_t)std::max<int64_t>(nnz, 1));
    std::vector<float> val((size_t)std::max<int64_t>(nnz, 1));
    for (int64_t r = 0; r < n_rows; ++r)
      for (int64_t j = indptr[r]; j < indptr[r + 1]; ++j) {
        const long long at = fill[indices[j]]++;
        rowidx[at] = (int)r; val[at] = data[j];
      }
    HIP_TRY(hipMalloc((void**)&h->csc_colptr, (size_t)(n_cols + 1) * sizeof(long long)));
    HIP_TRY(hipMalloc((void**)&h->csc_rowidx, rowidx.size() * sizeof(int)));
    HIP_TRY(hipMalloc((void**)&h->csc_val, val.size() * sizeof(float)));
    HIP_TRY(hipMemcpy(h->csc_colptr, colptr.data(), (size_t)(n_cols + 1) * sizeof(long long), hipMemcpyHostToDevice));
    HIP_TRY(hipMemcpy(h->csc_rowidx, rowidx.data(), rowidx.size() * sizeof(int), hipMemcpyHostToDevice));
    HIP_TRY(hipMemcpy(h->csc_val, val.data(), val.size() * sizeof(float), hipMemcpyHostToDevice));
    if (!h->sp_rows) TRY(dalloc(&h->sp_rows, (size_t)(h->N + CSC_BIAS_PARTS) * h->lde));
  }
  return 0;
}

int ganmf_tensor_shape(ganmf_handle* h, int tensor_id, int64_t* rows, int64_t* cols) {
  View v;
  if (h) TRY(needs_tensors(h, "ganmf_tensor_shape"));
  if (!h || !find_view(h, tensor_id, &v)) return fail(-1, "unknown tensor id %d", tensor_id);
  if (rows) *rows = v.rows;
  if (cols) *cols = v.cols;
  return 0;
}

static int copy_view(ganmf_handle* h, int tensor_id, int slot, float* host, int64_t n, bool to_device, const char* who) {
  View v;
  if (h) TRY(needs_tensors(h, who));
  if (!h || !host || !find_view(h, tensor_id, &v)) return fail(-1, "%s: unknown tensor id %d", who, tensor_id);
  if (n != (int64_t)v.rows * v.cols) return fail(-1, "%s: tensor %d has %lld elements, got %lld", who, tensor_id, (long long)v.rows * v.cols, (long long)n);
  if ((slot == GANMF_SLOT_ADAM_M || slot == GANMF_SLOT_ADAM_V) && h->has_comm && h->cfg.world_size > 1 && tensor_id != GANMF_T_USER_EMB)
    return fail(-1, "%s: the Adam moments of replicated tensor %d are sharded over the %d ranks of a data-parallel run "
                    "(each rank holds its slice only); only user_embeddings' moments are whole on their rank", who, tensor_id, h->cfg.world_size);
  HIP_TRY(hipSetDevice(h->dev));
  HIP_TRY(hipStreamSynchronize(h->st));
  for (int i = 0; i < v.nseg; ++i) {
    const Seg& sg = v.seg[i];
    float* d = slot_ptr(sg.t, slot);
    if (!d) return fail(-1, "%s: bad slot %d", who, slot);
    d += (size_t)sg.row0 * sg.t->ld + sg.col0;
    float* hp = host + (size_t)sg.host_row0 * v.cols;
    const size_t hpitch = (size_t)sg.cols * 4, dpitch = (size_t)sg.t->ld * 4;
    if (to_device) HIP_TRY(hipMemcpy2D(d, dpitch, hp, hpitch, (size_t)sg.cols * 4, sg.rows, hipMemcpyHostToDevice));
    else HIP_TRY(hipMemcpy2D(hp, hpitch, d, dpitch, (size_t)sg.cols * 4, sg.rows, hipMemcpyDeviceToHost));
  }
  return 0;
}

int ganmf_set_tensor(ganmf_handle* h, int tensor_id, int slot, const float* host, int64_t n) {
  if (h) ++h->param_version;
  return copy_view(h, tensor_id, slot, const_cast<float*>(host), n, true, "ganmf_set_tensor");
}

int ganmf_get_tensor(ganmf_handle* h, int tensor_id, int slot, float* host, int64_t n) {
  return copy_view(h, tensor_id, slot, host, n, false, "ganmf_get_tensor");
}

int ganmf_get_adam_powers(ganmf_handle* h, float out4[4]) {
  if (!h) return fail(-1, "null handle");
  HIP_TRY(hipSetDevice(h->dev));
  HIP_TRY(hipStreamSynchronize(h->st));
  HIP_TRY(hipMemcpy(out4, h->scal, 4 * sizeof(float), hipMemcpyDeviceToHost));
  return 0;
}

int ganmf_set_adam_powers(ganmf_handle* h, const float in4[4]) {
  if (!h) return fail(-1, "null handle");
  HIP_TRY(hipSetDevice(h->dev));
  HIP_TRY(hipStreamSynchronize(h->st));
  HIP_TRY(hipMemcpy(h->scal, in4, 4 * sizeof(float), hipMemcpyHostToDevice));
  return 0;
}
```

ganmf_amd/csrc/lib/handle.inc:

```

constexpr int LOCAL_MAX_WORLD = 8;
struct LocalPtrs { float* p[LOCAL_MAX_WORLD]; };
enum LocalOp : int { LOCAL_ALLREDUCE = 0, LOCAL_REDUCE_SCATTER = 1, LOCAL_ALLGATHER = 2 };
__global__ void local_collective_kernel(LocalPtrs b, int world, size_t count, int op) {
  const size_t slice = count / (size_t)world;
  for (size_t i = (size_t)blockIdx.x * blockDim.x + threadIdx.x; i < count; i += (size_t)gridDim.x * blockDim.x) {
    if (op == LOCAL_ALLGATHER) {
      const float v = b.p[i / slice][i];
      for (int r = 0; r < world; ++r) b.p[r][i] = v;
      continue;
    }
    float s = b.p[0][i];
    for (int r = 1; r < world; ++r) s += b.p[r][i];
    if (op == LOCAL_ALLREDUCE) { for (int r = 0; r < world; ++r) b.p[r][i] = s; }
    else b.p[i / slice][i] = s;
  }
}
struct LocalGroup {
  std::mutex mu;
  std::condition_variable cv;
  int world = 0, dev = -1, arrived = 0, joined = 0;
  long long generation = 0;
  size_t count = 0;
  int op = 0;
// ... 45 lines not shown
  size_t stage_i_cap = 0, stage_f_cap = 0;
  float *XF = nullptr, *Ub = nullptr, *E = nullptr, *Es = nullptr, *Dl = nullptr, *dE = nullptr, *dF = nullptr, *gUb = nullptr;
  float* XF_own = nullptr;
  float* XF_pass = nullptr;
  size_t XF_pass_elems = 0;
  float* Ub_pass = nullptr;
  size_t Ub_pass_elems = 0;
  bool skinny = true;
  int bf16w = 1;
  bool skinny_n = true;
  bool pass_stage = true;
  bool pass_buffers_tried = false;
  bool x_staged = false;
  bool front_staged = false;
  int tab_cap = 0;
  bool lazy_rows = true;
  bool lazy_pass = false;
  int g_alpha = S_ALPHA_G;
  float* Ub_own = nullptr;
  float* gUb_own = nullptr;
  float* Ub_sched = nullptr;
  size_t Ub_sched_elems = 0;
  int* pos_step = nullptr;
  std::vector<std::pair<float*, size_t>> lazy_chunks;
  size_t lazy_chunk = 0, lazy_used = 0;
  std::vector<LazyStep> lazy_steps;
  int lazy_step = 0;
  LazyStep* lazy_stage = nullptr;
  size_t lazy_stage_cap = 0;
  LazyStep* lazy_tab = nullptr;
  size_t lazy_tab_cap = 0;
  float* zero_page = nullptr;
  float* slab = nullptr;
  size_t slab_elems = 0;
  float* slab2 = nullptr;
  size_t slab2_elems = 0;
  unsigned *counters = nullptr, *counters2 = nullptr;
  int x3kg = 7;
  bool inkernel_reduce = true;
  int inlaunch_tags = 0;
  int inlaunch_max = 4;
  float* rs = nullptr;
  float* scal = nullptr;
  float *sqp = nullptr;
  int sqp_stride = 0;
  int reg_cap = 0;
  int pair_ring = 2;
  bool dis_colsum_pending = false;
  ColSumP dis_colsum{};
  bool dis_uid_done = false;
  int dis_cap = 0;
  float* dis_slot = nullptr;
  std::vector<char> dis_fused;
  std::vector<int> dis_regn;
  bool defer_gub = true;
  int multi = 31;
  float* V_alt = nullptr;
  bool fuse_adam = true;
  bool dis_fuse_hidden = true;
  bool dcoef_spread = true;
  float* parts_all = nullptr;
  float *d_parts = nullptr, *g_parts = nullptr;
  float* colbuf = nullptr;
  float *d_arena = nullptr, *g_arena = nullptr;
  int64_t parts_cap = 0;
  long long* seen_indptr = nullptr;
  int* seen_indices = nullptr;
  int64_t seen_rows = 0, seen_cols = 0;
  unsigned char* item_mask = nullptr;
  size_t item_mask_cap = 0;
  int64_t item_mask_w = 0;
  bool mask_cold = false;
  std::vector<unsigned char> filter_host, ignore_host;
  int64_t ignore_w = 0;
  unsigned char* rank_mask = nullptr;
  size_t rank_mask_cap = 0;
  int* topk_items = nullptr;
  float* topk_vals = nullptr;
  size_t topk_cap = 0;
  float* div_mat = nullptr;
  int64_t div_w = 0;
  long long* test_indptr = nullptr;
  int* test_indices = nullptr;
  double* test_gain = nullptr;
  int64_t test_rows = 0, test_cols = 0;
  double* eval_buf = nullptr;
  size_t eval_cap = 0;
  int64_t test_nnz = 0;
  float* test_rating = nullptr;
  bool test_rating_ok = false;
  double* eval_w = nullptr;
  int64_t eval_w_width = 0;
  float* eval_rmse = nullptr;
  size_t eval_rmse_cap = 0;
  unsigned* eval_counts = nullptr;
  size_t eval_counts_cap = 0;
  int* eval_grp = nullptr;
  size_t eval_grp_cap = 0;
  long long* cand_indptr = nullptr;
  int* cand_indices = nullptr;
  std::vector<long long> cand_indptr_host;
  int64_t cand_rows = 0, cand_cols = 0;
  int* sc_ids = nullptr;
  size_t sc_ids_cap = 0;
  float *sc_rows = nullptr, *sc_out = nullptr;
  size_t sc_rows_cap = 0, sc_out_cap = 0;
  unsigned *sc_pa = nullptr, *sc_pb = nullptr;
  size_t sc_pa_cap = 0, sc_pb_cap = 0;
  const float* sc_pb_src = nullptr;
  long long sc_pb_version = -1, param_version = 0;
  int sc_pb_rows = 0;
  float *sim_mat = nullptr, *sim_pool = nullptr;
  double* sim_part = nullptr;
  int* sim_zero = nullptr;
  size_t sim_mat_cap = 0, sim_pool_cap = 0, sim_part_cap = 0, sim_zero_cap = 0;
  int* dr_ids = nullptr;
  float *dr_X = nullptr, *dr_Ub = nullptr, *dr_E = nullptr, *dr_A = nullptr;
  double *dr_part = nullptr, *dr_val = nullptr;
  size_t dr_ids_cap = 0, dr_X_cap = 0, dr_Ub_cap = 0, dr_E_cap = 0, dr_A_cap = 0, dr_part_cap = 0, dr_val_cap = 0;
  int64_t disc_block = 0;
  AlsSide als[2];
  float* als_G = nullptr;
  int* als_bad = nullptr;
  long long* knn_indptr = nullptr;
  int* knn_nbr = nullptr;
  float* knn_val = nullptr;
  int64_t knn_nnz = -1;
  float* knn_dense = nullptr;
  size_t knn_dense_cap = 0;
  float* svd_P[2] = {nullptr, nullptr};
  float *svd_G = nullptr, *svd_X = nullptr, *svd_Wl = nullptr, *svd_lam = nullptr;
  int* svd_flag = nullptr;
  int svd_ldl = 0;
  int gram_arith = 1;
  bool score_presplit = true;
  ncclComm_t comm = nullptr;
  bool has_comm = false;
  std::atomic<bool> comm_aborted{false};
  std::mutex comm_mu;
  std::shared_ptr<LocalGroup> local;
  int d_alpha = S_ALPHA_D;
  int side_pending = 0;
  bool merge_decode = true;
  int red_elems = 0;
  bf16raw *pl_XF = nullptr, *pl_Dl = nullptr, *pl_Es = nullptr, *pl_dE = nullptr;
  long long ps_N = 0, ps_e = 0;
  float* wgs_dump = nullptr;
  int* wgs_table = nullptr;
  int wgs_key[5] = {0, 0, 0, 0, 0}, wgs_rounds = 0;
  size_t wgs_table_cap = 0;
  bool wgrad_stream = false;
  int adam_nfast = 3;
  int wgrad_xb = 16;
  int wgrad_seam = 0;
  int adam_touch = 1;
  unsigned long long* seam_cnt = nullptr;
  unsigned long long seam_target = 0;
  int pair_kg = 4;
  bool gub_x3 = false;
  int g_rows_staged = 1;
  int wd_lane = 0;
  long long fork_armed_at = 0;
  bool fork_attach = true;
  bool force_coll = false;
  GemmTune tune;
  bool debug_plan = false;
  int fused_bk = 0;
  int fused_tile = 64;
  int fused_mode = MFMA_BF16X3;
  std::vector<long long> seen_plans;
  bool prof = false;
  std::vector<ProfRec> recs;
};
```

ganmf_amd/csrc/lib/step_ganmf.inc:

```
GemmPlan generator_plan(ganmf_handle* h, int nb, bool* front) {
  const int N = h->N, k = h->k;
  GemmP g{};
  g.A = h->Ub; g.lda = h->ldk; g.B = h->V.p; g.ldb = h->ldk;
  g.C = h->XF + (size_t)nb * h->ldN; g.ldc = h->ldN;
  g.M = nb; g.N = N; g.K = k; g.epi.kind = EPI_STORE; g.nbatch = 1;
  g.zero_page = h->zero_page;
  GemmPlan pl = gemm_plan(g.M, g.N, g.K, 1, false, h->tune, (h->multi & 1) != 0 && k <= 256);
  pl.persist = gemm_persist_eligible(g, false, false, pl, h->tune.persist) ? 1 : 0;
  *front = (h->multi & 1) && plan_is_f32_64_kg(pl, 4) && pl.nsplit == 1;
  if (!*front && (h->multi & 1) && (h->x3kg & 4) && low_precision(h) && plan_is_lp_64(pl) && pl.nsplit == 1) { pl.kg = 4; *front = true; }
  if (*front) return pl;
  return plan_gemm(h, T_GEMM_GEN, g, false, false, nullptr);
}

inline int lazy_tab_slot(const ganmf_handle* h, int p);
bool stage_pass_plan(ganmf_handle* h, int64_t nfull, GemmPlan* pl, bool* front) {
  if (!h->pass_stage || nfull < 4 || h->sparse_d || nfull > h->tab_cap) return false;
  *pl = generator_plan(h, h->B, front);
  if (!*front && (pl->persist || pl->nsplit != 1)) return false;
  const size_t need = (size_t)nfull * 2 * h->B * h->ldN;
  if (need > h->XF_pass_elems) {
    size_t free_b = 0, total_b = 0;
    if (hipMemGetInfo(&free_b, &total_b) != hipSuccess) return false;
    if ((need - h->XF_pass_elems) * sizeof(float) > free_b / 4) return false;
// ... 101 lines not shown
    fill_plan(g, pl);
    Scope s(h, T_GEMM_GEN, nfull * gemm_flops(g.M, g.N, g.K), gemm_bytes((double)nfull * g.M, g.N, g.K));
    HIP_TRY(gemm_dispatch(h->st, g, false, false, pl));
    return 0;
  }
  g.A = h->Ub_pass; g.a_batch_stride = (long long)B * h->ldk;
  return run_gemm(h, T_GEMM_GEN, T_RED_GEN, g, false, false, nullptr, 0, 0, nullptr, nullptr, nullptr, nullptr, &pl0);
}

int rows_and_generator(ganmf_handle* h, const int* rows_dev, int nb, int which, int aslot, int uid_col, int row_offset) {
  if (which == 0 && h->front_staged) return 0;
  const bool xs = which == 1 && h->x_staged && h->lazy_pass;
  const int N = h->N, k = h->k;
  const bool lazy = which == 1 && h->lazy_pass;
  DensP d{h->indptr, h->indices, h->data, rows_dev, nb, N, h->XF, h->ldN, h->Ue.p, h->ldk, lazy ? nullptr : h->Ub, h->scal, which,
          lazy ? -1 : aslot, which ? h->cfg.g_lr : h->cfg.d_lr, uid_col, row_offset};
  GemmP g{};
  g.A = h->Ub; g.lda = h->ldk; g.B = h->V.p; g.ldb = h->ldk;
  g.C = h->XF + (size_t)nb * h->ldN; g.ldc = h->ldN;
  g.M = nb; g.N = N; g.K = k; g.epi.kind = EPI_STORE; g.nbatch = 1;
  g.zero_page = h->zero_page;
  bool is_front = false;
  GemmPlan pl = generator_plan(h, nb, &is_front);
  if (is_front) {
    if (h->debug_plan) {
      const long long key = ((long long)T_GEMM_GEN << 48) ^ ((long long)g.M << 32) ^ ((long long)g.N << 16) ^ g.K;
      if (std::find(h->seen_plans.begin(), h->seen_plans.end(), key) == h->seen_plans.end()) {
        h->seen_plans.push_back(key);
        fprintf(stderr, "[ganmf plan] %-28s M=%d N=%d K=%d batch=1 -> tile 64 ring 3 kg 4 nsplit 1 (kps %d) mfma %s wgs %d est %.1f us (one launch with the %d CSR rows)\n",
                kTagName[T_GEMM_GEN], g.M, g.N, g.K, pl.kps, pl.mode == MFMA_F16 ? "f16" : pl.mode == MFMA_BF16 ? "bf16" : combined_x3(h) ? "bf16x3" : "f32",
                pl.tiles_m * pl.tiles_n, pl.est_us, nb);
      }
    }
    Scope s(h, T_FRONT, gemm_flops(g.M, g.N, g.K), gemm_bytes(g.M, g.N, g.K) + 4.0 * nb * (N + 2 * k));
    if (!lazy) { g.A = h->Ue.p; g.a_gather = rows_dev; }
    fill_plan(g, pl);
    const int nrow_blocks = xs ? 0 : nb;
    if (pl.mode == MFMA_F16) GANMF_LAUNCH(front_lp_kernel<true>, dim3(pl.tiles_m * pl.tiles_n + nrow_blocks), dim3(1024), 0, h->st, g, d);
    else if (pl.mode == MFMA_BF16) GANMF_LAUNCH(front_lp_kernel<false>, dim3(pl.tiles_m * pl.tiles_n + nrow_blocks), dim3(1024), 0, h->st, g, d);
    else if (combined_x3(h)) GANMF_LAUNCH((front_kernel<4, true>), dim3(pl.tiles_m * pl.tiles_n + nrow_blocks), dim3(1024), 0, h->st, g, d);
    else GANMF_LAUNCH(front_kernel<4>, dim3(pl.tiles_m * pl.tiles_n + nrow_blocks), dim3(1024), 0, h->st, g, d);
    HIP_TRY(hipGetLastError());
    return 0;
  }
  if (!xs) {
    Scope s(h, T_DENSIFY, 0, 4.0 * nb * (N + 2 * k));
    d.nseg = std::max(1, std::min(16, (h->ldN + 8191) / 8192));
    GANMF_LAUNCH(densify_rows_kernel, dim3(nb * d.nseg), dim3(256), 0, h->st, d);
    HIP_TRY(hipGetLastError());
  }
  return run_gemm(h, T_GEMM_GEN, T_RED_GEN, g, false, false);
}

int step_front(ganmf_handle* h, const int* rows_dev, int nb, int which) {
  const int N = h->N, k = h->k, e = h->e;
  const int aslot = which ? h->g_alpha : h->d_alpha;
  const bool lazy = which == 1 && h->lazy_pass;
  if ((which == 1 && h->sparse_g) || (which == 0 && h->sparse_d)) {
    TRY(dp_join(h, PEND_WE));
    {
      Scope s(h, T_DENSIFY, 0, 4.0 * nb * (2 * k + e) + 4.0 * (double)h->nnz / std::max(h->U, 1) * nb * e);
      GANMF_LAUNCH(sparse_front_kernel, dim3(nb), dim3(256), 0, h->st, h->indptr, h->indices, h->data, rows_dev, nb, N,
                         h->XF, h->ldN, h->Ue.p, h->ldk, lazy ? nullptr : h->Ub, h->scal, which, lazy ? -1 : aslot, which ? h->cfg.g_lr : h->cfg.d_lr, h->We.p, h->lde, e, h->E);
      HIP_TRY(hipGetLastError());
    }
    {
      GemmP g{};
      g.A = h->Ub; g.lda = h->ldk; g.B = h->V.p; g.ldb = h->ldk;
      g.C = h->XF + (size_t)nb * h->ldN; g.ldc = h->ldN;
      g.M = nb; g.N = N; g.K = k; g.epi.kind = EPI_STORE;
      TRY(run_gemm(h, T_GEMM_GEN, T_RED_GEN, g, false, false));
    }
    {
      TRY(dp_join(h, PEND_WE));
      GemmP g{};
      g.A = h->XF + (size_t)nb * h->ldN; g.lda = h->ldN; g.B = h->We.p; g.ldb = h->lde;
      g.C = h->E + (size_t)nb * h->lde; g.ldc = h->lde; g.M = nb; g.N = e; g.K = N + 1; g.epi.kind = EPI_STORE;
      TRY(run_gemm(h, T_GEMM_ENC, T_RED_ENC, g, false, true));
    }
    return 0;
  }
  TRY(rows_and_generator(h, rows_dev, nb, which, aslot, -1, 0));
  {
    TRY(dp_join(h, PEND_WE));
    GemmP g{};
    g.A = h->XF; g.lda = h->ldN; g.B = h->We.p; g.ldb = h->lde;
    g.C = h->E; g.ldc = h->lde; g.M = 2 * nb; g.N = e; g.K = N + 1; g.epi.kind = EPI_STORE;
    TRY(run_gemm(h, T_GEMM_ENC, T_RED_ENC, g, false, true));
  }
  return 0;
}

int d_step(ganmf_handle* h, const int* rows_dev, int nb, int b_global, float* parts, float* arena) {
  float* regWe = arena + 2 * (size_t)h->reg_cap;
  float* regWd = arena + 3 * (size_t)h->reg_cap;
  const int N = h->N, e = h->e;
  const bool dist = h->has_comm;
  if ((dist || h->wd_lane) && !h->front_staged) h->d_alpha = h->d_alpha == S_ALPHA_D ? S_ALPHA_D_ALT : S_ALPHA_D;
  const int aslot = h->d_alpha;
  const float inv_bn = 1.0f / ((float)b_global * (float)N);
  int sqn = 0;
  bool fused = false;
  int regn[2] = {ADAM_GRID, ADAM_GRID};
  if (nb > 0) {
    TRY(step_front(h, rows_dev, nb, 0));
    TRY(dp_join(h, PEND_WD));
    {
      GemmP g{};
      g.A = h->E; g.lda = h->lde; g.B = h->Wd.p; g.ldb = h->ldN;
      g.C = h->Dl; g.ldc = h->ldN; g.M = nb; g.N = N; g.K = e + 1;
      g.nbatch = 2; g.a_batch_stride = (long long)nb * h->lde; g.c_batch_stride = (long long)nb * h->ldN;
      g.epi.kind = EPI_SUB_AUX_SQ; g.epi.aux = h->XF; g.epi.ldaux = h->ldN;
      g.epi.aux_batch_stride = (long long)nb * h->ldN; g.epi.sq_partials = h->sqp;
      if (h->sparse_d) {
        g.epi.csr_indptr = h->indptr; g.epi.csr_indices = h->indices; g.epi.csr_data = h->data; g.epi.csr_rows = rows_dev;
      }
      bool merged = false;
      if (!h->sparse_d && nb % 64 == 0 && h->merge_decode) {
        const GemmPlan p1 = gemm_plan(2 * nb, g.N, g.K, 1, true, h->tune), p2 = gemm_plan(g.M, g.N, g.K, 2, true, h->tune);
        if (p1.tile == 64 && p2.tile == 64 && p1.nsplit == 1 && p2.nsplit == 1 && p1.mode == p2.mode && p1.kg == p2.kg && p1.ring == p2.ring) {
          GemmP q = g;
          q.M = 2 * nb; q.nbatch = 1; q.a_batch_stride = 0; q.c_batch_stride = 0; q.epi.aux_batch_stride = 0;
          q.epi.sq_m_half = nb / 64;
          int cnt = 0;
          TRY(run_gemm(h, T_GEMM_DEC, T_RED_DEC, q, false, true, &cnt, 4.0 * 2 * nb * N));
          sqn = p2.sq_count;
          merged = true;
        }
      }
      if (!merged)
      TRY(run_gemm(h, T_GEMM_DEC, T_RED_DEC, g, false, true, &sqn, 4.0 * 2 * nb * N));
    }
  } else {
    GANMF_LAUNCH(open_step_kernel, dim3(1), dim3(64), 0, h->st, h->scal, 0, aslot, h->cfg.d_lr);
    HIP_TRY(hipGetLastError());
  }
  if (dist) {
    MultiRed mr{};
    mr.count = 2; mr.out = h->scal;
    mr.e[0] = {h->sqp, sqn, S_SUM_REAL, 0};
    mr.e[1] = {h->sqp + sqn, sqn, S_SUM_FAKE, 0};
    {
      Scope s(h, T_MULTIRED, 0, 0);
      GANMF_LAUNCH(multi_reduce_kernel, dim3(S_SUM_FAKE + 1), dim3(256), 0, h->st, mr);
      HIP_TRY(hipGetLastError());
    }
    TRY(allreduce(h, h->scal + S_SUM_REAL, 2));
  }
  const DCoefP dc{h->scal, h->sqp, sqn, sqn, dist ? 1 : 0, h->cfg.m, nb, inv_bn, h->E, h->Es, h->lde, h->rs, parts};
  const long long dc_total = (long long)2 * nb * (h->lde / 4);
  bool dcoef_done = false;
  GemmP gde{};
  GemmPlan pde;
  if (nb > 0 && (h->multi & 4) && (h->multi & 8)) {
    gde.A = h->Dl; gde.lda = h->ldN; gde.B = h->Wd.p; gde.ldb = h->ldN;
    gde.C = h->dE; gde.ldc = h->lde; gde.M = 2 * nb; gde.N = e; gde.K = N; gde.nbatch = 1;
    gde.epi.kind = EPI_ROWSCALE; gde.epi.rowscale = h->rs; gde.zero_page = h->zero_page;
    pde = gemm_plan(gde.M, gde.N, gde.K, 1, false, h->tune);
    pde.persist = 0;
    GemmPlan pskn = pde;
    const bool de_stream = h->skinny_n && plan_skinny_n(pskn, gde, false);
    if (!de_stream && plan_is_f32_64_kg(pde, 4) && pde.nsplit > 1 && !(h->inkernel_reduce && pde.nsplit <= h->inlaunch_max)) {
      TRY(ensure_slab(h, gemm_slab_elems(pde, gde.M, gde.ldc, 1), 0));
      Scope s(h, T_DE_DCOEF, gemm_flops(gde.M, gde.N, gde.K), gemm_bytes(gde.M, gde.N, gde.K) + 8.0 * 2 * nb * e);
      GemmP q = gde;
      fill_plan(q, pde);
      q.C = h->slab; q.c_split_stride = (long long)gde.M * gde.ldc; q.c_batch_stride = (long long)gde.M * gde.ldc;
      const int ng = pde.tiles_m * pde.tiles_n * pde.nsplit;
      const int nd = h->dcoef_spread ? 0 : (int)std::max<long long>(1, std::min<long long>(32, (dc_total + 4095) / 4096));
      if (combined_x3(h)) GANMF_LAUNCH((de_dcoef_kernel<4, true>), dim3(ng + nd), dim3(1024), 0, h->st, q, dc, nd);
      else GANMF_LAUNCH(de_dcoef_kernel<4>, dim3(ng + nd), dim3(1024), 0, h->st, q, dc, nd);
      HIP_TRY(hipGetLastError());
      dcoef_done = true;
    }
  }
  if (!dcoef_done) {
    Scope s(h, T_DCOEF, 0, 8.0 * 2 * nb * e);
    const int grid = (int)std::max<long long>(1, std::min<long long>(128, (dc_total + 1023) / 1024));
    GANMF_LAUNCH(d_coef_kernel, dim3(grid), dim3(256), 0, h->st, dc);
    HIP_TRY(hipGetLastError());
  }
  if (nb > 0) {
    const bool regD = h->cfg.d_reg != 0.f;
    fused = h->fuse_adam && !dist;
    GemmTune ft;
    ft.tile = h->fused_tile; ft.ring = 2; ft.nsplit = 1;
    ft.mode = h->tune.mode != MFMA_AUTO ? h->tune.mode : h->fused_mode;
    ft.bk = h->fused_bk;
    const GemmTune* wg_tune = &ft;
    const int start = (int)(rows_dev - h->perm);
    auto sparse_gWe = [&](GemmP& g) {
      if (!h->sparse_d) return;
      g.A = h->XF + (size_t)nb * h->ldN; g.B = h->dE + (size_t)nb * h->lde; g.K = nb;
      g.epi.sp_rows = h->sp_rows; g.epi.sp_ld = h->lde; g.epi.sp_bias_row = N; g.epi.sp_bias_parts = CSC_BIAS_PARTS;
    };
    auto sparse_rows = [&]() -> int {
      if (!h->sparse_d) return 0;
      Scope s(h, T_DENSIFY, 0, 4.0 * ((double)h->nnz / std::max(h->U, 1) * nb * e + 2.0 * (N + CSC_BIAS_PARTS) * e));
      GANMF_LAUNCH(csc_rows_kernel, dim3(N + CSC_BIAS_PARTS), dim3(256), 0, h->st, h->csc_colptr, h->csc_rowidx, h->csc_val,
                   h->pos, start, nb, N, h->dE, h->lde, e, h->sp_rows);
      HIP_TRY(hipGetLastError());
      return 0;
    };
    RedP dE_red{};
    auto gemm_gWd = [&]() -> int {
      GemmP g{};
      g.A = h->Es; g.lda = h->lde; g.B = h->Dl; g.ldb = h->ldN;
      g.C = h->Wd.g; g.ldc = h->ldN; g.M = e + 1; g.N = N; g.K = 2 * nb; g.epi.kind = EPI_STORE;
      g.a_scale = grad_scale(h, b_global);
      if (fused) {
        g.epi.kind = EPI_ADAM; g.epi.adam_theta = h->Wd.p; g.epi.adam_m = h->Wd.m; g.epi.adam_v = h->Wd.v;
        g.epi.adam_alpha = h->scal + aslot; g.epi.adam_reg = h->cfg.d_reg;
        g.epi.sq_partials = regD ? regWd : nullptr;
      }
      return run_gemm(h, T_GEMM_GWD, T_RED_GWD, g, true, true, &regn[1], fused ? 24.0 * h->Wd.count() : 0, 0, wg_tune, nullptr,
                      nullptr, dE_red.part ? &dE_red : nullptr);
    };
    if (dcoef_done) {
      dE_red = RedP{};
      dE_red.part = h->slab; dE_red.nsplit = pde.nsplit; dE_red.out = gde.C; dE_red.ld = gde.ldc; dE_red.M = gde.M; dE_red.N = gde.N;
      dE_red.batch_stride = 0; dE_red.epi = gde.epi; dE_red.epi.sq_stride = GEMM_RED_GRID;
      dE_red.split_stride = (long long)gde.M * gde.ldc;
    } else {
      GemmP g{};
      g.A = h->Dl; g.lda = h->ldN; g.B = h->Wd.p; g.ldb = h->ldN;
      g.C = h->dE; g.ldc = h->lde; g.M = 2 * nb; g.N = e; g.K = N;
      g.epi.kind = EPI_ROWSCALE; g.epi.rowscale = h->rs;
      TRY(run_gemm(h, T_GEMM_DE, T_RED_DE, g, false, false, nullptr, 0, 0, nullptr, nullptr,
                   (!dist && (h->multi & 4)) ? &dE_red : nullptr));
    }
    bool wpair = false;
#ifdef GANMF_PERSIST_DIAG_BUILD
    if (!dist && fused && h->wgrad_stream && h->pl_XF && ft.mode == MFMA_BF16X3) {
      const int K2 = 2 * nb;
      PlaneJobs js{};
      auto job = [&](const float* src, bf16raw* dst, long long ps, int rows, int ld) {
        js.j[js.count++] = PlaneJob{src, PlaneRef{dst, ps}, (long long)rows * ld / 4};
      };
      if (h->sparse_d) job(h->XF + (size_t)nb * h->ldN, h->pl_XF + (size_t)nb * h->ldN, h->ps_N, nb, h->ldN);
      else job(h->XF, h->pl_XF, h->ps_N, K2, h->ldN);
      job(h->Dl, h->pl_Dl, h->ps_N, K2, h->ldN);
      job(h->Es, h->pl_Es, h->ps_e, K2, h->lde);
      RedPlanes rp{};
      RedP rr{};
      int nred = 0;
      long long n4 = 0;
      if (dE_red.part) {
        rr = dE_red; rp.pl = PlaneRef{h->pl_dE, h->ps_e}; rp.on = 1;
        nred = h->red_elems > 0 ? red_grid(h, dE_red.M, dE_red.N, dE_red.nsplit) : GEMM_RED_GRID;
        rr.epi.sq_stride = nred;
      } else job(h->dE, h->pl_dE, h->ps_e, K2, h->lde);
      for (int i = 0; i < js.count; ++i) n4 += js.j[i].n4;
      const int nsp = (int)std::max<long long>(1, std::min<long long>(1024, (n4 + 1023) / 1024));
      {
        Scope s(h, T_RED_DE, 0, (dE_red.part ? 4.0 * (dE_red.nsplit + 1) * dE_red.M * dE_red.N : 0.0) + 10.0 * 4.0 * (double)n4);
        GANMF_LAUNCH(presplit_red_kernel, dim3(nred + nsp), dim3(256), 0, h->st, rr, rp, nred, js);
        HIP_TRY(hipGetLastError());
      }
      TRY(sparse_rows());
      WgsP w{};
      w.zero_page = h->zero_page;
      w.dump = h->wgs_dump;
      WgsProd& w0 = w.g[0];
      w0.a_pl = h->pl_Es; w0.a_ps = h->ps_e; w0.lda = h->lde; w0.b_pl = h->pl_Dl; w0.b_ps = h->ps_N; w0.ldb = h->ldN; w0.ldc = h->ldN;
      w0.M = e + 1; w0.N = N; w0.K = K2;
      w0.epi.kind = EPI_ADAM; w0.epi.adam_theta = h->Wd.p; w0.epi.adam_m = h->Wd.m; w0.epi.adam_v = h->Wd.v;
      w0.epi.adam_alpha = h->scal + aslot; w0.epi.adam_reg = h->cfg.d_reg; w0.epi.sq_partials = regD ? regWd : nullptr;
      WgsProd& w1 = w.g[1];
      const size_t r1 = h->sparse_d ? (size_t)nb : 0;
      w1.a_pl = h->pl_XF + r1 * h->ldN; w1.a_ps = h->ps_N; w1.lda = h->ldN; w1.b_pl = h->pl_dE + r1 * h->lde; w1.b_ps = h->ps_e; w1.ldb = h->lde;
      w1.ldc = h->lde; w1.M = N + 1; w1.N = e; w1.K = h->sparse_d ? nb : K2;
      w1.epi.kind = EPI_ADAM; w1.epi.adam_theta = h->We.p; w1.epi.adam_m = h->We.m; w1.epi.adam_v = h->We.v;
      w1.epi.adam_alpha = h->scal + aslot; w1.epi.adam_reg = h->cfg.d_reg; w1.epi.sq_partials = regD ? regWe : nullptr;
      if (h->sparse_d) { w1.epi.sp_rows = h->sp_rows; w1.epi.sp_ld = h->lde; w1.epi.sp_bias_row = N; w1.epi.sp_bias_parts = CSC_BIAS_PARTS; }
      for (int i = 0; i < 2; ++i) { w.g[i].tiles_m = (w.g[i].M + WGS_BM - 1) / WGS_BM; w.g[i].tiles_n = (w.g[i].N + WGS_BN - 1) / WGS_BN; }
      w.tiles0 = w0.tiles_m * w0.tiles_n;
      w.tiles_total = w.tiles0 + w1.tiles_m * w1.tiles_n;
      regn[1] = w.tiles0; regn[0] = w.tiles_total - w.tiles0;
      const int grid = std::min(GEMM_CUS, round_up(w.tiles_total, 8));
      {
        const int key[5] = {w0.tiles_m, w0.tiles_n, w1.tiles_m, w1.tiles_n, grid};
        if (memcmp(key, h->wgs_key, sizeof key) != 0) {
          const int tms[2] = {w0.tiles_m, w1.tiles_m}, tns[2] = {w0.tiles_n, w1.tiles_n};
          std::vector<int> tab;
          const int rounds = wgs_build_schedule(tms, tns, 2, grid, tab);
          HIP_TRY(hipStreamSynchronize(h->st));
          if (tab.size() > h->wgs_table_cap) {
            hipFree(h->wgs_table); h->wgs_table = nullptr;
            HIP_TRY(hipMalloc((void**)&h->wgs_table, tab.size() * sizeof(int)));
            h->wgs_table_cap = tab.size();
          }
          HIP_TRY(hipMemcpy(h->wgs_table, tab.data(), tab.size() * sizeof(int), hipMemcpyHostToDevice));
          memcpy(h->wgs_key, key, sizeof key);
          h->wgs_rounds = rounds;
        }
        w.table = h->wgs_table; w.rounds = h->wgs_rounds;
      }
      w.diag = env_int("GANMF_WGS_DIAG", 0);
      static unsigned long long* wst = nullptr;
      static int wst_n = 0;
      const bool stamping = env_int("GANMF_WGS_STAMPS", 0) != 0 && wst_n < 40;
      if (stamping) {
        if (!wst) HIP_TRY(hipMalloc((void**)&wst, (size_t)GEMM_CUS * 64 * 8));
        HIP_TRY(hipMemsetAsync(wst, 0, (size_t)GEMM_CUS * 64 * 8, h->st));
        w.stamps = wst;
      }
      {
        Scope s(h, T_WPAIR, gemm_flops(w0.M, w0.N, w0.K) + gemm_flops(w1.M, w1.N, w1.K),
                6.0 * ((double)w0.K * (w0.M + w0.N) + (double)w1.K * (w1.M + w1.N)) + 24.0 * ((double)w0.M * w0.N + (double)w1.M * w1.N));
        GANMF_LAUNCH(wgrad_stream_kernel, dim3(grid), dim3(1024), 0, h->st, w);
        HIP_TRY(hipGetLastError());
      }
      if (stamping && ++wst_n == 40) {
        HIP_TRY(hipStreamSynchronize(h->st));
        std::vector<unsigned long long> hs((size_t)grid * 64);
        HIP_TRY(hipMemcpy(hs.data(), wst, hs.size() * 8, hipMemcpyDeviceToHost));
        unsigned long long t0 = ~0ull;
        for (int b = 0; b < grid; ++b) if (hs[(size_t)b * 64]) t0 = std::min(t0, hs[(size_t)b * 64]);
        auto med = [&](int role, int i) {
          std::vector<double> v;
          for (int b = 0; b < grid; ++b) { const unsigned long long x = hs[((size_t)b * 2 + role) * 32 + i]; if (x) v.push_back((double)(x - t0) * 0.01); }
          if (v.empty()) return -1.0;
          std::sort(v.begin(), v.end());
          return v[v.size() / 2];
        };
        fprintf(stderr, "[wgs stamps] diag %d, %d workgroups, medians in us after the first GEMM-wave entry\n", w.diag, grid);
        for (int role = 0; role < 2; ++role) {
          fprintf(stderr, "  %s: start %.2f |", role ? "Adam" : "GEMM", med(role, 0));
          for (int r = 0; r < 6; ++r) fprintf(stderr, " r%d: work done %.2f, past Y %.2f, past X %.2f |", r, med(role, 1 + 3 * r), med(role, 2 + 3 * r), med(role, 3 + 3 * r));
          fprintf(stderr, "\n   detail:");
          for (int i = 19; i < 32; ++i) fprintf(stderr, " %.2f", med(role, i));
          fprintf(stderr, "\n");
        }
      }
      wpair = true;
    }
#endif
    if (!wpair && !dist && fused && (h->multi & 16) && dE_red.part) {
      GemmP g0{}, g1{};
      g0.A = h->Es; g0.lda = h->lde; g0.B = h->Dl; g0.ldb = h->ldN;
      g0.C = h->Wd.g; g0.ldc = h->ldN; g0.M = e + 1; g0.N = N; g0.K = 2 * nb; g0.nbatch = 1; g0.zero_page = h->zero_page;
      g0.a_scale = grad_scale(h, b_global);
      g0.epi.kind = EPI_ADAM; g0.epi.adam_theta = h->Wd.p; g0.epi.adam_m = h->Wd.m; g0.epi.adam_v = h->Wd.v;
      g0.epi.adam_alpha = h->scal + aslot; g0.epi.adam_reg = h->cfg.d_reg; g0.epi.sq_partials = regD ? regWd : nullptr;
      g1.A = h->XF; g1.lda = h->ldN; g1.B = h->dE; g1.ldb = h->lde;
      g1.C = h->We.g; g1.ldc = h->lde; g1.M = N + 1; g1.N = e; g1.K = 2 * nb; g1.nbatch = 1; g1.zero_page = h->zero_page;
      g1.b_scale = grad_scale(h, b_global);
      g1.epi.kind = EPI_ADAM; g1.epi.adam_theta = h->We.p; g1.epi.adam_m = h->We.m; g1.epi.adam_v = h->We.v;
      g1.epi.adam_alpha = h->scal + aslot; g1.epi.adam_reg = h->cfg.d_reg; g1.epi.sq_partials = regD ? regWe : nullptr;
      sparse_gWe(g1);
      GemmPlan p0 = gemm_plan(g0.M, g0.N, g0.K, 1, regD, ft, true), p1 = gemm_plan(g1.M, g1.N, g1.K, 1, regD, ft, true);
      auto staged = [](const GemmPlan& pl) { return pl.mode == MFMA_BF16X3 && pl.tile == 64 && pl.bk == 32 && pl.nsplit == 1; };
      const bool seam = h->wgrad_seam && !h->wd_lane && !h->sparse_d;
      if (staged(p0) && staged(p1)) {
        if (!seam) {
          Scope s(h, T_RED_DE, 0, 4.0 * (dE_red.nsplit + 1) * dE_red.M * dE_red.N);
          GANMF_LAUNCH(splitk_reduce_kernel, dim3(h->red_elems > 0 ? red_grid(h, dE_red.M, dE_red.N, dE_red.nsplit) : GEMM_RED_GRID, 1), dim3(256), 0, h->st, dE_red);
          HIP_TRY(hipGetLastError());
        }
        TRY(sparse_rows());
        fill_plan(g0, p0);
        fill_plan(g1, p1);
        g0.n_fastest = g1.n_fastest = (h->adam_nfast & 1);
        if (h->wgrad_xb > 0) { g0.n_fastest = 0; g0.xb_m = 1; g0.xb_n = 8; g0.xb_band = h->wgrad_xb; }
#ifdef GANMF_PERSIST_DIAG_BUILD
        if (env_int("GANMF_WGRAD_DIAG", 0) & 1) { g0.K = 0; g1.K = 0; g0.k_per_split = g1.k_per_split = 0; }
        g0.diag = g1.diag = env_int("GANMF_WGRAD_DIAG", 0);
#endif
        regn[1] = p0.sq_count; regn[0] = p1.sq_count;
        const int n0 = p0.tiles_m * p0.tiles_n, n1 = p1.tiles_m * p1.tiles_n;
#ifdef GANMF_PERSIST_DIAG_BUILD
        static unsigned long long* wst = nullptr;
        static int wst_printed = 0;
        const bool stamping = env_int("GANMF_WGRAD_STAMPS", 0) != 0 && wst_printed < 3;
        if (stamping) {
          if (!wst) HIP_TRY(hipMalloc((void**)&wst, (size_t)(n0 + n1) * 64 * 8));
          HIP_TRY(hipMemsetAsync(wst, 0, (size_t)(n0 + n1) * 64 * 8, h->st));
          g0.stamps = wst; g1.stamps = wst + (size_t)n0 * 64;
        }
#endif
        if (h->wd_lane) {
          GemmP none{};
          const bool armed = h->wd_lane == 1 && fork_arm(h);
          if (h->wd_lane != 1) TRY(lane_fork(h));
          {
            Scope s1(h, T_GEMM_GWE, gemm_flops(g1.M, g1.N, g1.K), 4.0 * (double)g1.K * (g1.M + g1.N) + 24.0 * (double)g1.M * g1.N);
            GANMF_LAUNCH(wgrad_pair_kernel, dim3(n1), dim3(256), 0, h->st, none, g1);
            HIP_TRY(hipGetLastError());
          }
          if (h->wd_lane == 1) TRY(fork_wait(h, armed));
          {
            Scope s0(h, T_GEMM_GWD, gemm_flops(g0.M, g0.N, g0.K), 4.0 * (double)g0.K * (g0.M + g0.N) + 24.0 * (double)g0.M * g0.N, h->st2);
            GANMF_LAUNCH(wgrad_pair_kernel, dim3(n0), dim3(256), 0, h->st2, g0, none);
            HIP_TRY(hipGetLastError());
          }
          TRY(dp_mark(h, PEND_WD));
        } else if (seam) {
          const int nred = h->red_elems > 0 ? red_grid(h, dE_red.M, dE_red.N, dE_red.nsplit) : GEMM_RED_GRID;
          RedP rr = dE_red;
          rr.sc1 = 1;
          h->seam_target += (unsigned long long)nred;
          Scope s(h, T_WPAIR, gemm_flops(g0.M, g0.N, g0.K) + gemm_flops(g1.M, g1.N, g1.K),
                  4.0 * ((double)g0.K * (g0.M + g0.N) + (double)g1.K * (g1.M + g1.N)) + 24.0 * ((double)g0.M * g0.N + (double)g1.M * g1.N) +
                      4.0 * (dE_red.nsplit + 1) * dE_red.M * dE_red.N);
          GANMF_LAUNCH(wgrad_seam_kernel, dim3(nred + n0 + n1), dim3(256), 0, h->st, g0, g1, rr, nred, h->seam_cnt, h->seam_target);
          HIP_TRY(hipGetLastError());
        } else {
          Scope s(h, T_WPAIR, gemm_flops(g0.M, g0.N, g0.K) + gemm_flops(g1.M, g1.N, g1.K),
                  4.0 * ((double)g0.K * (g0.M + g0.N) + (double)g1.K * (g1.M + g1.N)) + 24.0 * ((double)g0.M * g0.N + (double)g1.M * g1.N));
          GANMF_LAUNCH(wgrad_pair_kernel, dim3(n0 + n1), dim3(256), 0, h->st, g0, g1);
          HIP_TRY(hipGetLastError());
        }
#ifdef GANMF_PERSIST_DIAG_BUILD
        if (stamping && ++wst_printed >= 2) {
          HIP_TRY(hipStreamSynchronize(h->st));
          const int nw = n0 + n1;
          std::vector<unsigned long long> hs((size_t)nw * 64);
          HIP_TRY(hipMemcpy(hs.data(), wst, hs.size() * 8, hipMemcpyDeviceToHost));
          unsigned long long t0 = ~0ull, t1 = 0;
          for (int b = 0; b < nw; ++b) { t0 = std::min(t0, hs[(size_t)b * 64]); t1 = std::max(t1, hs[(size_t)b * 64 + 63]); }
          auto med = [&](auto f) { std::vector<double> v(nw); for (int b = 0; b < nw; ++b) v[b] = f(b) * 0.01; std::sort(v.begin(), v.end()); return std::make_pair(v[nw / 2], v[(size_t)(nw * 0.9)]); };
          auto pr = [&](const char* name, std::pair<double, double> m) { fprintf(stderr, "  %-44s median %6.2f  p90 %6.2f us\n", name, m.first, m.second); };
          fprintf(stderr, "[wgrad stamps] %d + %d workgroups, first entry -> last exit %.2f us\n", n0, n1, (t1 - t0) * 0.01);
          pr("entry after the first entry", med([&](int b) { return (double)(hs[(size_t)b * 64] - t0); }));
          pr("entry -> first K-tile's loads issued", med([&](int b) { return (double)(hs[(size_t)b * 64 + 1] - hs[(size_t)b * 64]); }));
          pr("K loop (8 K-tiles)", med([&](int b) { return (double)(hs[(size_t)b * 64 + 62] - hs[(size_t)b * 64 + 1]); }));
          pr("epilogue (Adam streams) + store drain", med([&](int b) { return (double)(hs[(size_t)b * 64 + 63] - hs[(size_t)b * 64 + 62]); }));
          for (int it = 0; it < 8; ++it) {
            const int o = 1 + 5 * it;
            fprintf(stderr, "  K-tile %d:", it);
            auto m1 = med([&](int b) { return (double)(hs[(size_t)b * 64 + o + 1] - hs[(size_t)b * 64 + o]); });
            auto m2 = med([&](int b) { return (double)(hs[(size_t)b * 64 + o + 2] - hs[(size_t)b * 64 + o + 1]); });
            fprintf(stderr, " fragments + MFMA issue %5.2f (p90 %5.2f)  barrier %5.2f (%5.2f)", m1.first, m1.second, m2.first, m2.second);
            if (it < 7) {
              auto m3 = med([&](int b) { return (double)(hs[(size_t)b * 64 + o + 3] - hs[(size_t)b * 64 + o + 2]); });
              auto m4 = med([&](int b) { return (double)(hs[(size_t)b * 64 + o + 4] - hs[(size_t)b * 64 + o + 3]); });
              auto m5 = med([&](int b) { return (double)(hs[(size_t)b * 64 + o + 5] - hs[(size_t)b * 64 + o + 4]); });
              fprintf(stderr, "  wait for loads + split + plane stores %5.2f (%5.2f)  barrier %5.2f (%5.2f)  next loads issued %5.2f", m3.first, m3.second, m4.first, m4.second, m5.first);
            }
            fprintf(stderr, " us\n");
          }
        }
#endif
        wpair = true;
      }
    }
    if (dist && dE_red.part) {
      Scope s(h, T_RED_DE, 0, 4.0 * (dE_red.nsplit + 1) * dE_red.M * dE_red.N);
      GANMF_LAUNCH(splitk_reduce_kernel, dim3(h->red_elems > 0 ? red_grid(h, dE_red.M, dE_red.N, dE_red.nsplit) : GEMM_RED_GRID, 1), dim3(256), 0, h->st, dE_red);
      HIP_TRY(hipGetLastError());
      dE_red.part = nullptr;
    }
    if (!dist && !wpair) TRY(gemm_gWd());
    if (!wpair) {
      TRY(sparse_rows());
      GemmP g{};
      g.A = h->XF; g.lda = h->ldN; g.B = h->dE; g.ldb = h->lde;
      g.C = h->We.g; g.ldc = h->lde; g.M = N + 1; g.N = e; g.K = 2 * nb; g.epi.kind = EPI_STORE;
      g.b_scale = grad_scale(h, b_global);
      if (fused) {
        g.epi.kind = EPI_ADAM; g.epi.adam_theta = h->We.p; g.epi.adam_m = h->We.m; g.epi.adam_v = h->We.v;
        g.epi.adam_alpha = h->scal + aslot; g.epi.adam_reg = h->cfg.d_reg;
        g.epi.sq_partials = regD ? regWe : nullptr;
      }
      sparse_gWe(g);
      const bool armed = dist && fork_arm(h);
      TRY(run_gemm(h, T_GEMM_GWE, T_RED_GWE, g, true, true, &regn[0], fused ? 24.0 * h->We.count() : 0, 0, wg_tune));
      if (dist) TRY(fork_wait(h, armed));
    }
    if (dist) {
      TRY(dp_update(h, T_ADAM_D, h->We, aslot, h->cfg.d_reg, regD ? regWe : nullptr, 1));
      TRY(dp_mark(h, PEND_WE));
      const bool armed = fork_arm(h);
      TRY(gemm_gWd());
      TRY(fork_wait(h, armed));
      TRY(dp_update(h, T_ADAM_D, h->Wd, aslot, h->cfg.d_reg, regD ? regWd : nullptr, 1));
      TRY(dp_mark(h, PEND_WD));
      (void)regn; (void)parts;
      return 0;
    }
  } else {
    TRY(dp_join(h));
    HIP_TRY(hipMemsetAsync(h->gD, 0, h->gD_elems * sizeof(float), h->st));
    if (dist) {
      const bool regD = h->cfg.d_reg != 0.f;
      TRY(lane_fork(h));
      TRY(dp_update(h, T_ADAM_D, h->We, aslot, h->cfg.d_reg, regD ? regWe : nullptr, 1));
      TRY(dp_mark(h, PEND_WE));
      TRY(dp_update(h, T_ADAM_D, h->Wd, aslot, h->cfg.d_reg, regD ? regWd : nullptr, 1));
      TRY(dp_mark(h, PEND_WD));
    }
  }
  const bool reg = h->cfg.d_reg != 0.f;
  if (!dist && !fused) {
    TRY(adam_dense(h, T_ADAM_D, h->We, h->We.g, aslot, h->cfg.d_reg, reg ? regWe : nullptr));
    TRY(adam_dense(h, T_ADAM_D, h->Wd, h->Wd.g, aslot, h->cfg.d_reg, reg ? regWd : nullptr));
  }
  (void)regn; (void)parts;
  return 0;
}

inline int lazy_tab_slot(const ganmf_handle* h, int p) { return S_TAB + (2 + (p & 1)) * h->tab_cap; }
bool lazy_pass_ok(const ganmf_handle* h, int64_t per_pass, int64_t n) {
  if (!(h->lazy_rows && h->cfg.g_reg == 0.f && per_pass >= 4 && per_pass <= h->tab_cap && n > 0)) return false;
  const GemmPlan pl = gemm_plan(h->B, h->k, h->N, 1, false, h->tune);
  const size_t per_step = (size_t)(std::max(pl.nsplit, 1) + 1) * h->B * h->ldk + 128;
  size_t have = 0;
  for (const auto& ch : h->lazy_chunks) have += ch.second;
  const size_t need = (size_t)per_pass * per_step;
  if (need <= have) return true;
  size_t free_b = 0, total_b = 0;
  if (hipMemGetInfo(&free_b, &total_b) != hipSuccess) return false;
  return (need - have) * sizeof(float) <= free_b / 4;
}
int lazy_block(ganmf_handle* h, size_t elems, float** out) {
  elems = (elems + 63) / 64 * 64;
  while (h->lazy_chunk < h->lazy_chunks.size() && h->lazy_used + elems > h->lazy_chunks[h->lazy_chunk].second) { ++h->lazy_chunk; h->lazy_used = 0; }
  if (h->lazy_chunk == h->lazy_chunks.size()) {
    const size_t want = std::max<size_t>(elems, (size_t)16 << 20);
    if (!lazy_chunk_alloc(h, want)) HIP_TRY(hipErrorOutOfMemory);
    h->lazy_used = 0;
  }
  *out = h->lazy_chunks[h->lazy_chunk].first + h->lazy_used;
  h->lazy_used += elems;
  return 0;
}
void lazy_pass_abort(ganmf_handle* h) {
  h->lazy_pass = false; h->Ub = h->Ub_own; h->gUb = h->gUb_own; h->g_alpha = S_ALPHA_G;
}
int lazy_pass_begin(ganmf_handle* h, int p, int64_t per_pass, int64_t n, bool opened) {
  const size_t need = (size_t)n * h->ldk;
  if (need > h->Ub_sched_elems) {
    HIP_TRY(hipStreamSynchronize(h->st));
    HIP_TRY(hipStreamSynchronize(h->st2));
    hipFree(h->Ub_sched); h->Ub_sched = nullptr; h->Ub_sched_elems = 0;
    TRY(dalloc(&h->Ub_sched, need));
    h->Ub_sched_elems = need;
  }
  const int tab = lazy_tab_slot(h, p);
  if (!opened) {
    GANMF_LAUNCH(open_steps_kernel, dim3(1), dim3(64), 0, h->st, h->scal, 1, tab, (int)per_pass, h->cfg.g_lr);
    HIP_TRY(hipGetLastError());
  }
  {
    Scope s(h, T_ADAM_U, 0, 16.0 * n * h->ldk);
    const long long total = (long long)n * (h->ldk / 4);
    const int grid = (int)std::max<long long>(1, std::min<long long>(8192, (total + 255) / 256));
    GANMF_LAUNCH(adam_rows_advance_kernel, dim3(grid), dim3(256), 0, h->st, h->Ue.p, h->Ue.m, h->Ue.v, h->perm, h->pos_step, (int)n,
                 h->ldk, h->scal, tab, h->cfg.g_reg, h->Ub_sched);
    HIP_TRY(hipGetLastError());
  }
  h->lazy_steps.assign((size_t)per_pass, LazyStep{nullptr, 0, 1, 0, 0});
  h->lazy_chunk = 0; h->lazy_used = 0;
  h->lazy_pass = true;
  return 0;
}
int lazy_pass_end(ganmf_handle* h, int p, int64_t per_pass) {
  const size_t T = (size_t)per_pass;
  if (2 * T > h->lazy_stage_cap) {
    HIP_TRY(hipStreamSynchronize(h->st));
    if (h->lazy_stage) hipHostFree(h->lazy_stage);
    h->lazy_stage = nullptr; h->lazy_stage_cap = 0;
    HIP_TRY(hipHostMalloc((void**)&h->lazy_stage, 2 * (T + 16) * sizeof(LazyStep), hipHostMallocDefault));
    h->lazy_stage_cap = 2 * (T + 16);
  }
  if (2 * T > h->lazy_tab_cap) {
    HIP_TRY(hipStreamSynchronize(h->st));
    hipFree(h->lazy_tab); h->lazy_tab = nullptr; h->lazy_tab_cap = 0;
    HIP_TRY(hipMalloc((void**)&h->lazy_tab, 2 * (T + 16) * sizeof(LazyStep)));
    h->lazy_tab_cap = 2 * (T + 16);
  }
  if (p >= 2) HIP_TRY(hipStreamSynchronize(h->st));
  LazyStep* const host = h->lazy_stage + (size_t)(p & 1) * (h->lazy_stage_cap / 2);
  LazyStep* const dev = h->lazy_tab + (size_t)(p & 1) * (h->lazy_tab_cap / 2);
  std::copy(h->lazy_steps.begin(), h->lazy_steps.end(), host);
  HIP_TRY(hipMemcpyAsync(dev, host, T * sizeof(LazyStep), hipMemcpyHostToDevice, h->st));
  {
    Scope s(h, T_ADAM_U, 0, 24.0 * h->Ue.count());
    const long long total = (long long)h->U * (h->ldk / 4);
    const int grid = (int)std::max<long long>(1, std::min<long long>(8192, (total + 255) / 256));
    GANMF_LAUNCH(adam_rows_flush_kernel, dim3(grid), dim3(256), 0, h->st, h->Ue.p, h->Ue.m, h->Ue.v, h->pos, h->pos_step, dev,
                 (int)per_pass, h->U, h->ldk, h->scal, lazy_tab_slot(h, p), h->cfg.g_reg);
    HIP_TRY(hipGetLastError());
  }
  lazy_pass_abort(h);
  return 0;
}

int gen_update(ganmf_handle* h, int nb, int start, int b_global, int* regn_v, float* reg_u, float* reg_v) {
  const int N = h->N, k = h->k;
  const bool reg = h->cfg.g_reg != 0.f;
  const bool dist = h->has_comm;
  const bool fused = h->fuse_adam && !dist && nb > 0;
  *regn_v = ADAM_GRID;
  const bool lazy = h->lazy_pass;
  h->gub_x3 = (long long)((N + 63) / 64) * ((k + 63) / 64) >= 2 * GEMM_CUS && experiment_int("GANMF_GV_STAGED", 1) != 0;
  SlabRef gub{h->gUb, 1, 0};
  auto gemm_gUb = [&]() -> int {
    GemmP g{};
// ... 210 lines not shown
```

Before: 9488.

## Fold d_coef into dE split-K reduce and add one-piece bf16 A path

Moves the discriminator coefficient computation (loss sums, hinge scalars, scaling of E into Es) out of the dE GEMM launch and into the split-K reduce kernel. The reduced dE output is scaled directly by the per-row coefficients, which removes the extra d_coef blocks and part of a pass over memory. It also adds an optional mode for the weight-gradient GEMM: when the sparse input values are exactly representable in bf16, A is stored as a single bf16 piece for the leading K-tiles, skipping the low-piece MFMAs. That mode is off by default (x_onepiece=0), so the fused-reduce path is the main active change; it adds restructuring and some extra synchronisation inside the reduce.

```diff
diff --git a/ganmf_amd/csrc/d_coef.hpp b/ganmf_amd/csrc/d_coef.hpp
--- /dev/null
+++ b/ganmf_amd/csrc/d_coef.hpp
@@ -0,0 +1,95 @@
+#pragma once
+#include <hip/hip_runtime.h>
+
+namespace ganmf {
+
+enum Scal : int {
+  S_B1P_D = 0, S_B2P_D = 1, S_B1P_G = 2, S_B2P_G = 3,
+  S_ALPHA_D = 4, S_ALPHA_G = 5,
+  S_ALPHA_D_ALT = 6,
+  S_SUM_REAL = 8, S_SUM_FAKE = 9, S_SUM_FM = 10,
+  S_B1P_G_SAVED = 12, S_B2P_G_SAVED = 13,
+  S_COUNT = 16,
+  S_TAB = 16
+};
+
+__device__ inline float wave_sum(float v) {
+#pragma unroll
+  for (int o = 32; o > 0; o >>= 1) v += __shfl_xor(v, o);
+  return v;
+}
+
+struct DCoefP {
+  float* scal;
+  const float* partials;
+  int np, pstride, presummed;
+  float m;
+  int b_local;
+  float inv_bn;
+  const float* E;
+  float* Es;
+  int lde;
+  float* rs;
+  float* loss_parts;
+};
+
+struct DCoefS { float cr, cf, Lr, h; };
+
+__device__ __forceinline__ void d_coef_loads(const DCoefP& p, float& q0, float& q1) {
+  q0 = 0.f; q1 = 0.f;
+  if (p.presummed) { q0 = p.scal[S_SUM_REAL]; q1 = p.scal[S_SUM_FAKE]; }
+  else if (threadIdx.x < 256 && (int)threadIdx.x < p.np) { q0 = p.partials[threadIdx.x]; q1 = p.partials[(size_t)p.pstride + threadIdx.x]; }
+}
+
+__device__ __forceinline__ DCoefS d_coef_scalars(const DCoefP& p, const float q0, const float q1, float* __restrict__ red) {
+  float sum0 = q0, sum1 = q1;
+  if (!p.presummed) {
+    float s0 = 0.f, s1 = 0.f;
+    s0 += q0; s1 += q1;
+    if (threadIdx.x < 256)
+      for (int i = threadIdx.x + 256; i < p.np; i += 256) { s0 += p.partials[i]; s1 += p.partials[(size_t)p.pstride + i]; }
+    s0 = wave_sum(s0);
+    s1 = wave_sum(s1);
+    if (threadIdx.x < 256 && (threadIdx.x & 63) == 0) { red[threadIdx.x >> 6] = s0; red[4 + (threadIdx.x >> 6)] = s1; }
+    __syncthreads();
+    sum0 = (red[0] + red[1]) + (red[2] + red[3]);
+    sum1 = (red[4] + red[5]) + (red[6] + red[7]);
+  }
+  DCoefS s;
+  s.Lr = sum0 * p.inv_bn;
+  const float Lf = sum1 * p.inv_bn;
+  s.h = p.m * s.Lr - Lf;
+  const bool on = s.h > 0.f;
+  s.cr = (on ? 1.f + p.m : 1.f) * (2.f * p.inv_bn);
+  s.cf = (on ? -1.f : 0.f) * (2.f * p.inv_bn);
+  return s;
+}
+
+__device__ __forceinline__ void d_coef_scale(const DCoefP& p, const DCoefS& s, const int bx, const int nbx, const float4* first = nullptr) {
+  const int c4 = p.lde / 4;
+  const long long total = (long long)2 * p.b_local * c4;
+  const long long i0 = (long long)bx * blockDim.x + threadIdx.x;
+  for (long long i = i0; i < total; i += (long long)nbx * blockDim.x) {
+    const int r = (int)(i / c4);
+    const float sc = r < p.b_local ? s.cr : s.cf;
+    float4 v = (first && i == i0) ? *first : reinterpret_cast<const float4*>(p.E)[i];
+    v.x *= sc; v.y *= sc; v.z *= sc; v.w *= sc;
+    reinterpret_cast<float4*>(p.Es)[i] = v;
+  }
+  if (bx == 0) {
+    for (int r = threadIdx.x; r < 2 * p.b_local; r += blockDim.x) p.rs[r] = r < p.b_local ? s.cr : s.cf;
+    if (threadIdx.x == 0) {
+      p.loss_parts[0] = s.Lr + fmaxf(0.f, s.h);
+      p.loss_parts[1] = s.h > 0.f ? 1.f : 0.f;
+    }
+  }
+}
+
+__device__ __forceinline__ void d_coef_body(const DCoefP& p, const int bx, const int nbx, float* __restrict__ red) {
+  float q0, q1;
+  d_coef_loads(p, q0, q1);
+  const DCoefS s = d_coef_scalars(p, q0, q1, red);
+  d_coef_scale(p, s, bx, nbx);
+}
+
+}
diff --git a/ganmf_amd/csrc/gemm_bf16s.hpp b/ganmf_amd/csrc/gemm_bf16s.hpp
--- a/ganmf_amd/csrc/gemm_bf16s.hpp
+++ b/ganmf_amd/csrc/gemm_bf16s.hpp
@@ -130,7 +130,7 @@
   static constexpr int DW = OPER > BM * BN ? OPER : BM * BN;
 };
 
-template <int BM, int BN, int BK, bool AKM, bool BKM, int NPIECE, bool F16 = false, bool GRAM = false, bool ROWSQ = false>
+template <int BM, int BN, int BK, bool AKM, bool BKM, int NPIECE, bool F16 = false, bool GRAM = false, bool ROWSQ = false, bool A1 = false>
 __device__ __forceinline__ void gemm_bf16s_body(const GemmP& p, const int bid, const int nblk, float* __restrict__ smem) {
   static_assert(!F16 || NPIECE == 1, "fp16 pieces only in the single-piece (mixed precision) mode");
   const float sa = (F16 && p.a_scale != 0.f) ? p.a_scale : 1.f, sb = (F16 && p.b_scale != 0.f) ? p.b_scale : 1.f;
@@ -186,16 +186,22 @@
   la.load(ra, p.lda, kleft);
   lb.load(rb, p.ldb, kleft);
   kleft -= BK;
-  la.template store<NPIECE, F16>(planes_a, ra, sa);
-  lb.template store<NPIECE, F16>(planes_b, rb, sb);
-  __syncthreads();
+  static_assert(!A1 || (AKM && BKM && NPIECE == 3 && !F16 && !GRAM && !ROWSQ), "one-piece A: the TN three-way split form");
+  int ne = 0;
+  if constexpr (A1) ne = min(nt, max(p.a_exact_k - kbeg, 0) / BK);
+  if constexpr (!A1) {
+    la.template store<NPIECE, F16>(planes_a, ra, sa);
+    lb.template store<NPIECE, F16>(planes_b, rb, sb);
+    __syncthreads();
+  }
 
   u32x4 pa[2][TM][NPIECE], pb[2][TN][NPIECE];
-  auto load_frags = [&](int set, int c) {
+  auto load_frags = [&](int set, int c, auto a1) {
+    constexpr int NPA = decltype(a1)::value ? 1 : NPIECE;
 #pragma unroll
     for (int a = 0; a < TM; ++a)
 #pragma unroll
-      for (int q = 0; q < NPIECE; ++q) pa[set][a][q] = SA::frag(planes_a + q * SA::PLANE, wr * WM + a * 32, c, li, lh);
+      for (int q = 0; q < NPA; ++q) pa[set][a][q] = SA::frag(planes_a + q * SA::PLANE, wr * WM + a * 32, c, li, lh);
 #pragma unroll
     for (int b = 0; b < TN; ++b)
 #pragma unroll
@@ -210,7 +216,7 @@
 #pragma unroll
         for (int r = 0; r < 16; ++r) accl[a][b][r] = 0.f;
   }
-  auto mfmas = [&](int set) {
+  auto mfmas = [&](int set, auto a1) {
     constexpr int NT = NPIECE == 3 ? 6 : 1;
     constexpr int ta[6] = {1, 0, 2, 1, 0, 0}, tb[6] = {1, 2, 0, 0, 1, 0};
 #pragma unroll
@@ -220,6 +226,7 @@
 #pragma unroll
         for (int b = 0; b < TN; ++b) {
           const int ia = NT == 6 ? ta[t6] : 0, ib = NT == 6 ? tb[t6] : 0;
+          if (decltype(a1)::value && ia != 0) continue;
           if (NT == 6 && t6 < 5)
             accl[a][b] = __builtin_amdgcn_mfma_f32_32x32x16_bf16(__builtin_bit_cast(bf16x8, pa[set][a][ia]),
                                                                  __builtin_bit_cast(bf16x8, pb[set][b][ib]), accl[a][b], 0, 0, 0);
@@ -232,6 +239,7 @@
         }
   };
 
+  if constexpr (!A1)
   for (int it = 0; it < nt; ++it) {
     const bool more = it + 1 < nt;
     if (more) {
@@ -245,14 +253,14 @@
       kleft -= BK;
     }
     if (it < 12) GANMF_S_STAMP(1 + 5 * it);
-    load_frags(0, 0);
+    load_frags(0, 0, std::false_type{});
 #pragma unroll
     for (int c = 0; c < NC; ++c) {
-      if (c + 1 < NC) load_frags((c + 1) & 1, c + 1);
-#ifdef GANMF_PERSIST_DIAG_BUILD
-      if (p.diag & 4) { if (c == 0) mfmas(0); continue; }
-#endif
-      mfmas(c & 1);
+      if (c + 1 < NC) load_frags((c + 1) & 1, c + 1, std::false_type{});
+#ifdef GANMF_PERSIST_DIAG_BUILD
+      if (p.diag & 4) { if (c == 0) mfmas(0, std::false_type{}); continue; }
+#endif
+      mfmas(c & 1, std::false_type{});
     }
     if (it < 12) GANMF_S_STAMP(2 + 5 * it);
     __syncthreads();
@@ -265,6 +273,42 @@
       if (it < 12) GANMF_S_STAMP(5 + 5 * it);
     }
   }
+  auto ktile_a1 = [&](const int it, auto a1) {
+    if constexpr (decltype(a1)::value) la.template store<1, false>(planes_a, ra);
+    else la.template store<NPIECE, F16>(planes_a, ra, sa);
+    lb.template store<NPIECE, F16>(planes_b, rb, sb);
+    if (it > 0 && it <= 12) GANMF_S_STAMP(4 + 5 * (it - 1));
+    __syncthreads();
+    if (it > 0 && it <= 12) GANMF_S_STAMP(5 + 5 * (it - 1));
+    if (it + 1 < nt) {
+#ifdef GANMF_PERSIST_DIAG_BUILD
+      if (!(p.diag & 16))
+#endif
+      {
+      la.load(ra, p.lda, kleft);
+      lb.load(rb, p.ldb, kleft);
+      }
+      kleft -= BK;
+    }
+    if (it < 12) GANMF_S_STAMP(1 + 5 * it);
+    load_frags(0, 0, a1);
+#pragma unroll
+    for (int c = 0; c < NC; ++c) {
+      if (c + 1 < NC) load_frags((c + 1) & 1, c + 1, a1);
+#ifdef GANMF_PERSIST_DIAG_BUILD
+      if (p.diag & 4) { if (c == 0) mfmas(0, a1); continue; }
+#endif
+      mfmas(c & 1, a1);
+    }
+    if (it < 12) GANMF_S_STAMP(2 + 5 * it);
+    __syncthreads();
+    if (it < 12) GANMF_S_STAMP(3 + 5 * it);
+  };
+  if constexpr (A1) {
+    int it = 0;
+    for (; it < ne; ++it) ktile_a1(it, std::true_type{});
+    for (; it < nt; ++it) ktile_a1(it, std::false_type{});
+  }
   GANMF_S_STAMP(62);
   if constexpr (NPIECE == 3) {
 #pragma unroll
diff --git a/ganmf_amd/csrc/gemm_f32.hpp b/ganmf_amd/csrc/gemm_f32.hpp
--- a/ganmf_amd/csrc/gemm_f32.hpp
+++ b/ganmf_amd/csrc/gemm_f32.hpp
@@ -10,6 +10,7 @@
 #include <type_traits>
 
 #include "adam_touch.hpp"
+#include "d_coef.hpp"
 
 namespace ganmf {
 
@@ -259,6 +260,7 @@
   long long a_pstride, b_pstride;
   int n_fastest;
   int adam_touch;
+  int a_exact_k;
 };
 
 #define GANMF_WAIT_VMCNT(N) asm volatile("s_waitcnt vmcnt(%0)" ::"n"(N) : "memory")
@@ -843,13 +845,14 @@
   long long batch_stride;
   EpiD epi;
   int sc1 = 0;
+  DCoefP dc;
 };
 
 __host__ __device__ inline int reduce_groups(long long total4, int nsplit) {
   return (nsplit >= 64 && total4 <= 8192) ? 16 : 1;
 }
 
-template <int NT = 256>
+template <int NT = 256, bool DC = false>
 __device__ __forceinline__ void splitk_reduce_body(const RedP& p, const int bx, const int nbx, const int bz, float* __restrict__ red) {
   const int n4 = (p.N + 3) >> 2;
   const long long total = (long long)p.M * n4;
@@ -859,6 +862,15 @@
   const bool csr0 = e.csr_indptr != nullptr && bz == 0 && e.kind == EPI_SUB_AUX_SQ;
   const float* __restrict__ aux = (e.aux && !csr0) ? e.aux + (size_t)bz * e.aux_batch_stride : nullptr;
   float sq = 0.f;
+  constexpr bool dcon = DC;
+  DCoefS ds{};
+  float dq0 = 0.f, dq1 = 0.f;
+  float4 de0 = make_float4(0.f, 0.f, 0.f, 0.f);
+  if (dcon) {
+    d_coef_loads(p.dc, dq0, dq1);
+    const long long ei = (long long)bx * blockDim.x + threadIdx.x;
+    if (ei < (long long)2 * p.dc.b_local * (p.dc.lde / 4)) de0 = reinterpret_cast<const float4*>(p.dc.E)[ei];
+  }
   auto finish = [&](float4 s, int m, int c, size_t off) {
     if (csr0) {
       const float4 x = csr_quad(e, m, c);
@@ -867,7 +879,7 @@
     float o[4] = {s.x, s.y, s.z, s.w};
     if (c + 3 < p.N) {
 #pragma unroll
-      for (int j = 0; j < 4; ++j) o[j] = epi_apply(e, o[j], m, c + j, p.ld, aux, sq);
+      for (int j = 0; j < 4; ++j) o[j] = dcon ? o[j] * (m < p.dc.b_local ? ds.cr : ds.cf) : epi_apply(e, o[j], m, c + j, p.ld, aux, sq);
       if (p.sc1) {
         typedef unsigned u32x4s __attribute__((ext_vector_type(4)));
         const __amdgpu_buffer_rsrc_t rs = __builtin_amdgcn_make_buffer_rsrc((void*)out, (short)0, 0x7fffffff, 0x00020000);
@@ -879,7 +891,7 @@
       if (e.planes) planes_store4(PlaneRef{e.planes, e.plane_stride}, off, o[0], o[1], o[2], o[3]);
     } else {
       for (int j = 0; j < 4 && c + j < p.N; ++j) {
-        const float r = epi_apply(e, o[j], m, c + j, p.ld, aux, sq);
+        const float r = dcon ? o[j] * (m < p.dc.b_local ? ds.cr : ds.cf) : epi_apply(e, o[j], m, c + j, p.ld, aux, sq);
         if (p.sc1) {
           const __amdgpu_buffer_rsrc_t rs = __builtin_amdgcn_make_buffer_rsrc((void*)out, (short)0, 0x7fffffff, 0x00020000);
           __builtin_amdgcn_raw_buffer_store_b32(__float_as_uint(r), rs, (int)((off + j) * sizeof(float)), 0, 16);
@@ -891,6 +903,7 @@
   };
   const int G = reduce_groups(total, p.nsplit);
   if (G > 1) {
+    if (dcon) { ds = d_coef_scalars(p.dc, dq0, dq1, red); __syncthreads(); }
     float4* const meet = reinterpret_cast<float4*>(red + 4);
     const int epb = NT / G, g = threadIdx.x / epb, el = threadIdx.x % epb;
     for (long long base = (long long)bx * epb; base < total; base += (long long)nbx * epb) {
@@ -918,18 +931,34 @@
       __syncthreads();
     }
   } else {
-    for (long long idx = (long long)bx * NT + threadIdx.x; idx < total; idx += (long long)nbx * NT) {
-      const int m = (int)(idx / n4), c = (int)(idx % n4) * 4;
-      const size_t off = (size_t)m * p.ld + c;
+    auto slab_sum = [&](size_t off) {
       float4 s = *reinterpret_cast<const float4*>(part + off);
 #pragma unroll 8
       for (int k = 1; k < p.nsplit; ++k) {
         const float4 q = *reinterpret_cast<const float4*>(part + (size_t)k * p.split_stride + off);
         s.x += q.x; s.y += q.y; s.z += q.z; s.w += q.w;
       }
-      finish(s, m, c, off);
-    }
-  }
+      return s;
+    };
+    long long idx = (long long)bx * NT + threadIdx.x;
+    if (dcon) {
+      const bool live = idx < total;
+      const int m = live ? (int)(idx / n4) : 0, c = live ? (int)(idx % n4) * 4 : 0;
+      const size_t off = (size_t)m * p.ld + c;
+      float4 s = make_float4(0.f, 0.f, 0.f, 0.f);
+      if (live) s = slab_sum(off);
+      ds = d_coef_scalars(p.dc, dq0, dq1, red);
+      if (e.sq_partials) __syncthreads();
+      if (live) finish(s, m, c, off);
+      idx += (long long)nbx * NT;
+    }
+    for (; idx < total; idx += (long long)nbx * NT) {
+      const int m = (int)(idx / n4), c = (int)(idx % n4) * 4;
+      const size_t off = (size_t)m * p.ld + c;
+      finish(slab_sum(off), m, c, off);
+    }
+  }
+  if (dcon) d_coef_scale(p.dc, ds, bx, nbx, &de0);
   if (e.sq_partials) {
 #pragma unroll
     for (int o = 32; o > 0; o >>= 1) sq += __shfl_xor(sq, o);
@@ -947,6 +976,10 @@
 __global__ __launch_bounds__(256) void splitk_reduce_kernel(const RedP p) {
   __shared__ __attribute__((aligned(16))) float red[4 + 4 * 256];
   splitk_reduce_body(p, (int)blockIdx.x, (int)gridDim.x, (int)blockIdx.y, red);
+}
+__global__ __launch_bounds__(256) void splitk_reduce_dcoef_kernel(const RedP p) {
+  __shared__ __attribute__((aligned(16))) float red[4 + 4 * 256];
+  splitk_reduce_body<256, true>(p, (int)blockIdx.x, (int)gridDim.x, 0, red);
 }
 
 constexpr int GEMM_K_ALIGN = 64;
diff --git a/ganmf_amd/csrc/gemm_multi.hpp b/ganmf_amd/csrc/gemm_multi.hpp
--- a/ganmf_amd/csrc/gemm_multi.hpp
+++ b/ganmf_amd/csrc/gemm_multi.hpp
@@ -37,14 +37,12 @@
   if (nd == 0) {
     d_coef_body(d, (int)blockIdx.x, ng, smem);
     __syncthreads();
-    if constexpr (X3) gemm_bf16k_body<false, false>(g, (int)blockIdx.x, ng, smem);
-    else gemm_f32_body<64, 64, 64, 3, false, false, KG>(g, (int)blockIdx.x, ng, smem);
+  } else if (nd > 0 && (int)blockIdx.x >= ng) {
+    d_coef_body(d, (int)blockIdx.x - ng, nd, smem);
     return;
   }
-  if ((int)blockIdx.x < ng) {
-    if constexpr (X3) gemm_bf16k_body<false, false>(g, (int)blockIdx.x, ng, smem);
-    else gemm_f32_body<64, 64, 64, 3, false, false, KG>(g, (int)blockIdx.x, ng, smem);
-  } else d_coef_body(d, (int)blockIdx.x - ng, nd, smem);
+  if constexpr (X3) gemm_bf16k_body<false, false>(g, (int)blockIdx.x, ng, smem);
+  else gemm_f32_body<64, 64, 64, 3, false, false, KG>(g, (int)blockIdx.x, ng, smem);
 }
 
 template <int KG, int NS>
@@ -85,8 +83,8 @@
   __shared__ __attribute__((aligned(16))) float smem[Bf16sLds<64, 64, 32, 3>::DW];
   const int n0 = g0.tiles_m * g0.tiles_n * g0.nsplit * g0.nbatch;
   const int n1 = g1.tiles_m * g1.tiles_n * g1.nsplit * g1.nbatch;
-  if ((int)blockIdx.x < n0) gemm_bf16s_body<64, 64, 32, true, true, 3>(g0, (int)blockIdx.x, n0, smem);
-  else gemm_bf16s_body<64, 64, 32, true, true, 3>(g1, (int)blockIdx.x - n0, n1, smem);
+  if ((int)blockIdx.x < n0) gemm_bf16s_body<64, 64, 32, true, true, 3, false, false, false, true>(g0, (int)blockIdx.x, n0, smem);
+  else gemm_bf16s_body<64, 64, 32, true, true, 3, false, false, false, true>(g1, (int)blockIdx.x - n0, n1, smem);
 }
 
 __global__ __launch_bounds__(256, 2) void wgrad_seam_kernel(const GemmP g0, const GemmP g1, const RedP r, const int nred, unsigned long long* cnt,
diff --git a/ganmf_amd/csrc/kernels.hpp b/ganmf_amd/csrc/kernels.hpp
--- a/ganmf_amd/csrc/kernels.hpp
+++ b/ganmf_amd/csrc/kernels.hpp
@@ -4,23 +4,6 @@
 #include "gemm_f32.hpp"
 
 namespace ganmf {
-
-enum Scal : int {
-  S_B1P_D = 0, S_B2P_D = 1, S_B1P_G = 2, S_B2P_G = 3,
-  S_ALPHA_D = 4, S_ALPHA_G = 5,
-  S_ALPHA_D_ALT = 6,
-  S_SUM_REAL = 8, S_SUM_FAKE = 9, S_SUM_FM = 10,
-  S_B1P_G_SAVED = 12, S_B2P_G_SAVED = 13,
-  S_COUNT = 16,
-  S_TAB = 16
-};
-
-
-__device__ inline float wave_sum(float v) {
-#pragma unroll
-  for (int o = 32; o > 0; o >>= 1) v += __shfl_xor(v, o);
-  return v;
-}
 
 __device__ inline float block_sum_256(float v, float* red4) {
   v = wave_sum(v);
@@ -318,62 +301,8 @@
   }
 }
 
-struct DCoefP {
-  float* scal;
-  const float* partials;
-  int np, pstride, presummed;
-  float m;
-  int b_local;
-  float inv_bn;
-  const float* E;
-  float* Es;
-  int lde;
-  float* rs;
-  float* loss_parts;
-};
-
-__device__ __forceinline__ void d_coef_body(const DCoefP& p, const int bx, const int nbx, float* __restrict__ red) {
-  float* sums = red + 4;
-  if (!p.presummed) {
-    for (int z = 0; z < 2; ++z) {
-      float s = 0.f;
-      if (threadIdx.x < 256)
-        for (int i = threadIdx.x; i < p.np; i += 256) s += p.partials[(size_t)z * p.pstride + i];
-      s = wave_sum(s);
-      if (threadIdx.x < 256 && (threadIdx.x & 63) == 0) red[threadIdx.x >> 6] = s;
-      __syncthreads();
-      if (threadIdx.x == 0) sums[z] = (red[0] + red[1]) + (red[2] + red[3]);
-      __syncthreads();
-    }
-  } else {
-    if (threadIdx.x == 0) { sums[0] = p.scal[S_SUM_REAL]; sums[1] = p.scal[S_SUM_FAKE]; }
-    __syncthreads();
-  }
-  const float Lr = sums[0] * p.inv_bn, Lf = sums[1] * p.inv_bn;
-  const float h = p.m * Lr - Lf;
-  const bool on = h > 0.f;
-  const float cr = (on ? 1.f + p.m : 1.f) * (2.f * p.inv_bn);
-  const float cf = (on ? -1.f : 0.f) * (2.f * p.inv_bn);
-  const int c4 = p.lde / 4;
-  const long long total = (long long)2 * p.b_local * c4;
-  for (long long i = (long long)bx * blockDim.x + threadIdx.x; i < total; i += (long long)nbx * blockDim.x) {
-    const int r = (int)(i / c4);
-    const float sc = r < p.b_local ? cr : cf;
-    float4 v = reinterpret_cast<const float4*>(p.E)[i];
-    v.x *= sc; v.y *= sc; v.z *= sc; v.w *= sc;
-    reinterpret_cast<float4*>(p.Es)[i] = v;
-  }
-  if (bx == 0) {
-    for (int r = threadIdx.x; r < 2 * p.b_local; r += blockDim.x) p.rs[r] = r < p.b_local ? cr : cf;
-    if (threadIdx.x == 0) {
-      p.loss_parts[0] = Lr + fmaxf(0.f, h);
-      p.loss_parts[1] = on ? 1.f : 0.f;
-    }
-  }
-}
-
 __global__ __launch_bounds__(256) void d_coef_kernel(const DCoefP p) {
-  __shared__ float red[6];
+  __shared__ float red[8];
   d_coef_body(p, (int)blockIdx.x, (int)gridDim.x, red);
 }
 
diff --git a/ganmf_amd/csrc/lib/abi_core.inc b/ganmf_amd/csrc/lib/abi_core.inc
--- a/ganmf_amd/csrc/lib/abi_core.inc
+++ b/ganmf_amd/csrc/lib/abi_core.inc
@@ -97,6 +97,8 @@
   h->g_rows_staged = std::max(0, std::min(2, tune_env_int("g_rows_staged", 1)));
   h->pair_kg = tune_env_int("pair_kg", 4) == 1 ? 1 : 4;
   h->wgrad_seam = tune_env_int("wgrad_seam", 0);
+  h->dcoef_in_red = tune_env_int("dcoef_in_red", 1) != 0;
+  h->x_onepiece = tune_env_int("x_onepiece", 0) != 0;
   h->adam_touch = tune_env_int("adam_touch", 1) != 0 ? 1 : 0;
   h->gram_arith = tune_env_int("gram", 1) == 0 ? 0 : 1;
   HIP_TRY(hipMalloc((void**)&h->seam_cnt, 2 * sizeof(unsigned long long)));
@@ -401,6 +403,13 @@
   }
   h->nnz = nnz;
   h->has_urm = true;
+  h->x_bf16_exact = true;
+  for (int64_t j = 0; j < nnz && h->x_bf16_exact; ++j) {
+    uint32_t bits;
+    memcpy(&bits, &data[j], sizeof bits);
+    const uint32_t ex = (bits >> 23) & 0xffu;
+    if ((bits & 0xffffu) != 0 || ex == 0xffu || (ex == 0 && (bits & 0x7fffffffu) != 0)) h->x_bf16_exact = false;
+  }
   const double density = (double)nnz / ((double)n_rows * (double)n_cols);
   const int force = env_int("GANMF_SPARSE", -1);
   h->sparse_g = h->cfg.model == GANMF_MODEL_GANMF && (force >= 0 ? force != 0 : density < 0.005);
@@ -409,8 +418,8 @@
   h->sparse_d = h->cfg.model == GANMF_MODEL_GANMF && force != 0 &&
                 (force_d >= 0 ? force_d != 0 : (density < 0.005 && flops_saved >= 2.0e9));
   if (h->debug_plan)
-    fprintf(stderr, "[ganmf urm] set_urm_csr %lldx%lld nnz=%lld%s density %.5f -> sparse_g %d sparse_d %d\n", (long long)n_rows,
-            (long long)n_cols, (long long)nnz, canonical ? "" : " (made canonical)", density, (int)h->sparse_g, (int)h->sparse_d);
+    fprintf(stderr, "[ganmf urm] set_urm_csr %lldx%lld nnz=%lld%s density %.5f -> sparse_g %d sparse_d %d x_bf16_exact %d\n", (long long)n_rows,
+            (long long)n_cols, (long long)nnz, canonical ? "" : " (made canonical)", density, (int)h->sparse_g, (int)h->sparse_d, (int)h->x_bf16_exact);
   hipFree(h->csc_colptr); hipFree(h->csc_rowidx); hipFree(h->csc_val);
   h->csc_colptr = nullptr; h->csc_rowidx = nullptr; h->csc_val = nullptr;
   if (h->sparse_d) {
diff --git a/ganmf_amd/csrc/lib/handle.inc b/ganmf_amd/csrc/lib/handle.inc
--- a/ganmf_amd/csrc/lib/handle.inc
+++ b/ganmf_amd/csrc/lib/handle.inc
@@ -221,6 +221,9 @@
   bool wgrad_stream = false;
   int adam_nfast = 3;
   int wgrad_xb = 16;
+  bool dcoef_in_red = true;
+  bool x_onepiece = false;
+  bool x_bf16_exact = false;
   int wgrad_seam = 0;
   int adam_touch = 1;
   unsigned long long* seam_cnt = nullptr;
diff --git a/ganmf_amd/csrc/lib/step_ganmf.inc b/ganmf_amd/csrc/lib/step_ganmf.inc
--- a/ganmf_amd/csrc/lib/step_ganmf.inc
+++ b/ganmf_amd/csrc/lib/step_ganmf.inc
@@ -277,6 +277,19 @@
   bool dcoef_done = false;
   GemmP gde{};
   GemmPlan pde;
+  GemmTune ft;
+  ft.tile = h->fused_tile; ft.ring = 2; ft.nsplit = 1;
+  ft.mode = h->tune.mode != MFMA_AUTO ? h->tune.mode : h->fused_mode;
+  ft.bk = h->fused_bk;
+  auto staged = [](const GemmPlan& pl) { return pl.mode == MFMA_BF16X3 && pl.tile == 64 && pl.bk == 32 && pl.nsplit == 1; };
+  bool dcoef_pending = false;
+  if (nb > 0 && h->dcoef_in_red && !dist && h->fuse_adam && (h->multi & 16) && !h->wd_lane && !(h->wgrad_seam && !h->sparse_d)) {
+    const bool regD = h->cfg.d_reg != 0.f;
+    dcoef_pending = staged(gemm_plan(e + 1, N, 2 * nb, 1, regD, ft, true)) && staged(gemm_plan(N + 1, e, h->sparse_d ? nb : 2 * nb, 1, regD, ft, true));
+#ifdef GANMF_PERSIST_DIAG_BUILD
+    if (h->wgrad_stream && h->pl_XF && ft.mode == MFMA_BF16X3) dcoef_pending = false;
+#endif
+  }
   if (nb > 0 && (h->multi & 4) && (h->multi & 8)) {
     gde.A = h->Dl; gde.lda = h->ldN; gde.B = h->Wd.p; gde.ldb = h->ldN;
     gde.C = h->dE; gde.ldc = h->lde; gde.M = 2 * nb; gde.N = e; gde.K = N; gde.nbatch = 1;
@@ -292,13 +305,22 @@
       fill_plan(q, pde);
       q.C = h->slab; q.c_split_stride = (long long)gde.M * gde.ldc; q.c_batch_stride = (long long)gde.M * gde.ldc;
       const int ng = pde.tiles_m * pde.tiles_n * pde.nsplit;
-      const int nd = h->dcoef_spread ? 0 : (int)std::max<long long>(1, std::min<long long>(32, (dc_total + 4095) / 4096));
-      if (combined_x3(h)) GANMF_LAUNCH((de_dcoef_kernel<4, true>), dim3(ng + nd), dim3(1024), 0, h->st, q, dc, nd);
-      else GANMF_LAUNCH(de_dcoef_kernel<4>, dim3(ng + nd), dim3(1024), 0, h->st, q, dc, nd);
+      if (h->debug_plan) {
+        const long long key = ((long long)T_DE_DCOEF << 48) ^ ((long long)gde.M << 32) ^ ((long long)gde.N << 16) ^ gde.K ^ (dcoef_pending ? 1ll << 62 : 0);
+        if (std::find(h->seen_plans.begin(), h->seen_plans.end(), key) == h->seen_plans.end()) {
+          h->seen_plans.push_back(key);
+          fprintf(stderr, "[ganmf plan] %-28s M=%d N=%d K=%d batch=1 -> tile 64 ring 3 kg 4 nsplit %d (kps %d) mfma %s wgs %d est %.1f us (d_coef in the %s)\n",
+                  kTagName[T_DE_DCOEF], gde.M, gde.N, gde.K, pde.nsplit, pde.kps, combined_x3(h) ? "bf16x3" : "f32", ng, pde.est_us,
+                  dcoef_pending ? "slab sum" : "dE launch");
+        }
+      }
+      const int nd = dcoef_pending ? -1 : h->dcoef_spread ? 0 : (int)std::max<long long>(1, std::min<long long>(32, (dc_total + 4095) / 4096));
+      if (combined_x3(h)) GANMF_LAUNCH((de_dcoef_kernel<4, true>), dim3(ng + std::max(nd, 0)), dim3(1024), 0, h->st, q, dc, nd);
+      else GANMF_LAUNCH(de_dcoef_kernel<4>, dim3(ng + std::max(nd, 0)), dim3(1024), 0, h->st, q, dc, nd);
       HIP_TRY(hipGetLastError());
       dcoef_done = true;
-    }
-  }
+    } else dcoef_pending = false;
+  } else dcoef_pending = false;
   if (!dcoef_done) {
     Scope s(h, T_DCOEF, 0, 8.0 * 2 * nb * e);
     const int grid = (int)std::max<long long>(1, std::min<long long>(128, (dc_total + 1023) / 1024));
@@ -308,10 +330,6 @@
   if (nb > 0) {
     const bool regD = h->cfg.d_reg != 0.f;
     fused = h->fuse_adam && !dist;
-    GemmTune ft;
-    ft.tile = h->fused_tile; ft.ring = 2; ft.nsplit = 1;
-    ft.mode = h->tune.mode != MFMA_AUTO ? h->tune.mode : h->fused_mode;
-    ft.bk = h->fused_bk;
     const GemmTune* wg_tune = &ft;
     const int start = (int)(rows_dev - h->perm);
     auto sparse_gWe = [&](GemmP& g) {
@@ -475,12 +493,18 @@
       g1.epi.adam_alpha = h->scal + aslot; g1.epi.adam_reg = h->cfg.d_reg; g1.epi.sq_partials = regD ? regWe : nullptr;
       sparse_gWe(g1);
       GemmPlan p0 = gemm_plan(g0.M, g0.N, g0.K, 1, regD, ft, true), p1 = gemm_plan(g1.M, g1.N, g1.K, 1, regD, ft, true);
-      auto staged = [](const GemmPlan& pl) { return pl.mode == MFMA_BF16X3 && pl.tile == 64 && pl.bk == 32 && pl.nsplit == 1; };
       const bool seam = h->wgrad_seam && !h->wd_lane && !h->sparse_d;
+      if (h->x_onepiece && h->x_bf16_exact && !h->sparse_d && !seam && h->tune.mode == MFMA_AUTO) g1.a_exact_k = nb;
       if (staged(p0) && staged(p1)) {
         if (!seam) {
-          Scope s(h, T_RED_DE, 0, 4.0 * (dE_red.nsplit + 1) * dE_red.M * dE_red.N);
-          GANMF_LAUNCH(splitk_reduce_kernel, dim3(h->red_elems > 0 ? red_grid(h, dE_red.M, dE_red.N, dE_red.nsplit) : GEMM_RED_GRID, 1), dim3(256), 0, h->st, dE_red);
+          Scope s(h, T_RED_DE, 0, 4.0 * (dE_red.nsplit + 1) * dE_red.M * dE_red.N + (dcoef_pending ? 8.0 * 2 * nb * e : 0.0));
+          const dim3 rgrid(h->red_elems > 0 ? red_grid(h, dE_red.M, dE_red.N, dE_red.nsplit) : GEMM_RED_GRID, 1);
+          if (dcoef_pending) {
+            RedP rr = dE_red;
+            rr.dc = dc;
+            dcoef_pending = false;
+            GANMF_LAUNCH(splitk_reduce_dcoef_kernel, rgrid, dim3(256), 0, h->st, rr);
+          } else GANMF_LAUNCH(splitk_reduce_kernel, rgrid, dim3(256), 0, h->st, dE_red);
           HIP_TRY(hipGetLastError());
         }
         TRY(sparse_rows());
@@ -494,6 +518,14 @@
 #endif
         regn[1] = p0.sq_count; regn[0] = p1.sq_count;
         const int n0 = p0.tiles_m * p0.tiles_n, n1 = p1.tiles_m * p1.tiles_n;
+        if (h->debug_plan) {
+          const long long key = ((long long)T_WPAIR << 48) ^ ((long long)g1.M << 32) ^ ((long long)g1.N << 16) ^ g1.K ^ ((long long)g1.a_exact_k << 40);
+          if (std::find(h->seen_plans.begin(), h->seen_plans.end(), key) == h->seen_plans.end()) {
+            h->seen_plans.push_back(key);
+            fprintf(stderr, "[ganmf plan] %-28s gWd %d + gWe %d wgs, K=%d in K-tiles of 32, gWe: %d K-tiles with A as one bf16 piece (a_exact_k %d)\n",
+                    kTagName[T_WPAIR], n0, n1, g1.K, g1.a_exact_k / 32, g1.a_exact_k);
+          }
+        }
 #ifdef GANMF_PERSIST_DIAG_BUILD
         static unsigned long long* wst = nullptr;
         static int wst_printed = 0;
@@ -570,6 +602,7 @@
         wpair = true;
       }
     }
+    if (dcoef_pending) return fail(-1, "d_step: d_coef was left to a slab sum of dE that did not run");
     if (dist && dE_red.part) {
       Scope s(h, T_RED_DE, 0, 4.0 * (dE_red.nsplit + 1) * dE_red.M * dE_red.N);
       GANMF_LAUNCH(splitk_reduce_kernel, dim3(h->red_elems > 0 ? red_grid(h, dE_red.M, dE_red.N, dE_red.nsplit) : GEMM_RED_GRID, 1), dim3(256), 0, h->st, dE_red);
```

Measured after the change: 9486, median of 3. Within noise of the previous version (-0.0%).
